# Eclectic-Sheep/sheeprl

Hardware: NVIDIA H100
Metric: Dreamer-V3 train-steps/sec (S, bs16 seq64 horizon15, 64x64x3 obs) (higher is better)
Workload: dtype f32

## Files before the change

include/b200rl.h:

```cpp
#ifndef B200RL_H_
#define B200RL_H_

#include <cuda_runtime_api.h>

#ifdef __cplusplus
extern "C" {
#endif

const char* b200rl_last_error(void);
int b200rl_abi_version(void);
const char* b200rl_build_arch(void);
int b200rl_device_check(void);

int b200rl_gemm_f32(const float* A, const float* B, float* C, const float* bias, int M, int N, int K, int lda, int ldb,
                    int ldc, int transA, int transB, int accumulate, cudaStream_t stream);
int b200rl_set_matmul_precision(int tf32_passes);
int b200rl_get_matmul_precision(void);
int b200rl_gemm_tc_supported(const float* A, const float* B, int M, int N, int K, int lda, int ldb, int transA,
                             int transB);
int b200rl_gemm_tc(const float* A, const float* B, float* C, const float* bias, int M, int N, int K, int lda, int ldb,
                   int ldc, int transA, int transB, int accumulate, cudaStream_t stream);
int b200rl_tf32_split(const float* X, float* Xhi, float* Xlo, long long n, cudaStream_t stream);
int b200rl_tf32_split_t(const float* W, float* Thi, float* Tlo, int rows, int cols, long long ldw, long long ldt,
                        cudaStream_t stream);
int b200rl_gemm_tc_presplit_supported(const float* A, const float* Bhi, const float* Blo, int M, int N, int K, int lda,
                                      int ldb);
int b200rl_gemm_tc_presplit(const float* A, const float* Bhi, const float* Blo, float* C, const float* bias, int M, int N,
                            int K, int lda, int ldb, int ldc, int accumulate, cudaStream_t stream);
int b200rl_gemm_ln_supported(const float* A, const float* W, int M, int N, int K, int lda, int ldw, int mode);
int b200rl_gemm_ln(const float* A, const float* W, int M, int N, int K, int lda, int ldw, const float* gamma,
                   const float* beta, float eps, int act, float* pre, long long ldpre, float* out, long long ldout,
                   int mode, const float* h_prev, long long ldh, float* h_out, long long ldho, float* h_out2,
                   long long ldho2, cudaStream_t stream);
int b200rl_gemm_ln_presplit_supported(const float* A, const float* Whi, const float* Wlo, int M, int N, int K, int lda,
                                      int ldw, int mode);
int b200rl_gemm_ln_presplit(const float* A, const float* Whi, const float* Wlo, int M, int N, int K, int lda, int ldw,
                            const float* gamma, const float* beta, float eps, int act, float* pre, long long ldpre,
                            float* out, long long ldout, int mode, const float* h_prev, long long ldh, float* h_out,
                            long long ldho, float* h_out2, long long ldho2, cudaStream_t stream);
int b200rl_ln_act_route(int C, long long ld0, long long ld1, long long ld2, const float* p0, const float* p1,
                        const float* p2, const float* gamma, const float* beta);
int b200rl_ln_act_fwd(const float* X, const float* gamma, const float* beta, float* Y, long long M, int C,
                      long long ldx, long long ldy, float eps, int act, cudaStream_t stream);
int b200rl_ln_act_bwd(const float* X, const float* gamma, const float* beta, const float* dY, float* dX, float* dgamma,
                      float* dbeta, long long M, int C, long long ldx, long long lddy, long long lddx, float eps,
                      int act, int accumulate, cudaStream_t stream);
int b200rl_col_sum(const float* X, float* out, long long M, int C, long long ldx, int accumulate, cudaStream_t stream);

int b200rl_obs_prep(const void* obs_nchw, int is_uint8, float* out_nhwc, long long NB, int C, int HW,
                    cudaStream_t stream);
int b200rl_transpose_batched(const float* X, float* Y, int NB, int a, int b, cudaStream_t stream);
int b200rl_transpose2d(const float* X, float* Y, int rows, int cols, long long ldx, long long ldy, cudaStream_t stream);
int b200rl_conv_down(const float* big, const float* W, float* small_, int NB, int h, int w, int Cs, int Cb,
                     cudaStream_t stream);
int b200rl_conv_up(const float* small_, const float* W, float* big, const float* bias, int NB, int h, int w, int Cs,
                   int Cb, cudaStream_t stream);
int b200rl_conv_wgrad(const float* small_, const float* big, float* dW, int NB, int h, int w, int Cs, int Cb,
                      int accumulate, cudaStream_t stream);
int b200rl_thin_down_supported(int w, int Cs, int Cb);
int b200rl_thin_up_supported(int Cs, int Cb);
int b200rl_thin_wgrad_supported(int Cs, int Cb);
int b200rl_conv_wgrad_tc_supported(int NB, int h, int w, int Cs, int Cb);
long long b200rl_conv_wgrad_tc_workspace(int NB, int h, int w, int Cs, int Cb);
int b200rl_conv_wgrad_tc(const float* small_, const float* big, float* dW, float* workspace, int NB, int h, int w,
                         int Cs, int Cb, int accumulate, cudaStream_t stream);
int b200rl_conv_tc_supported(int mode_up, int NB, int h, int w, int Cs, int Cb);
long long b200rl_conv_pack_floats(int mode_up, int Cs, int Cb);
int b200rl_conv_pack(const float* W, float* Wpacked, int mode_up, int Cs, int Cb, cudaStream_t stream);
int b200rl_conv_down_tc(const float* big, const float* Wpacked, float* small_, int NB, int h, int w, int Cs, int Cb,
                        cudaStream_t stream);
int b200rl_conv_up_tc(const float* small_, const float* Wpacked, float* big, const float* bias, int NB, int h, int w,
                      int Cs, int Cb, cudaStream_t stream);
int b200rl_conv_pack_split(const float* W, float* Whi, float* Wlo, int mode_up, int Cs, int Cb, cudaStream_t stream);
int b200rl_conv_down_tc_presplit(const float* big, const float* Whi, const float* Wlo, float* small_, int NB, int h, int w,
                                 int Cs, int Cb, cudaStream_t stream);
int b200rl_conv_up_tc_presplit(const float* small_, const float* Whi, const float* Wlo, float* big, const float* bias,
                               int NB, int h, int w, int Cs, int Cb, cudaStream_t stream);

int b200rl_gru_gate_fwd(const float* G, const float* Hin, float* Hout, long long M, int R, long long ldg,
                        long long ldhi, long long ldho, cudaStream_t stream);
int b200rl_gru_gate_bwd(const float* G, const float* Hin, const float* dH, float* dG, float* dHin, long long M, int R,
                        long long ldg, long long ldhi, long long lddh, long long lddg, long long lddhi,
                        cudaStream_t stream);
int b200rl_mask_mix(const float* prev, const float* init_row, const float* first, float* out, long long M, int C,
                    long long ldp, long long ldo, cudaStream_t stream);
int b200rl_mask_bwd(const float* dIn, const float* first, float* dPrev, float* dInit, int M, int C, long long ldi,
                    long long ldp, cudaStream_t stream);
int b200rl_cat_sample(const float* raw, const float* noise, float* onehot, float* mix_out, long long M, int groups,
                      int classes, long long ldr, long long ldn, long long ldo, long long ldm, float unimix,
                      cudaStream_t stream);
int b200rl_head_sample_supported(const float* X, const float* W, int Kin, int A, long long ldx, long long ldw);
int b200rl_head_sample(const float* X, const float* W, const float* bias, const float* noise, float* raw, float* onehot,
                       long long M, int Kin, int A, long long ldx, long long ldw, long long ldr, long long ldn,
                       long long ldo, float unimix, cudaStream_t stream);
int b200rl_cat_sample_bwd(const float* raw, const float* dz, const float* dmix, float* draw, long long M, int groups,
                          int classes, long long ldr, long long lddz, long long lddm, long long lddr, float unimix,
                          cudaStream_t stream);
int b200rl_kl_loss_grad(const float* post_mix, const float* prior_mix, float* d_post, float* d_prior, float* rows,
                        long long M, int groups, int classes, long long ldp, long long ldq, long long lddp,
                        long long lddq, float kl_dyn, float kl_rep, float free_nats, float regularizer, float scale,
                        cudaStream_t stream);
typedef struct b200rl_rssm_scan_args {
  int T, B, S, D, R, A, Dx, Dt, Dr, ld_lat, ld_wr1;
  float eps, unimix;
  const float *W_in, *lnx_g, *lnx_b, *W_g, *lng_g, *lng_b, *W_t1, *lnt_g, *lnt_b, *W_t2, *b_t2;
  const float *W_r1, *lnr_g, *lnr_b, *W_r2, *b_r2;
  const float *h0, *z0;
  const float *pe, *actions, *first, *noise;
  float* latent;
  float *z_in, *h_in, *a_in, *x_pre, *x_act, *g_pre, *g_ln, *tr_pre, *tr_act, *rp_pre, *rp_act;
  float *post_raw, *prior_raw, *post_mix, *prior_mix;
  void* workspace;
  long long workspace_bytes;
} b200rl_rssm_scan_args;
typedef struct b200rl_rssm_scan_grads {
  const float *d_latent, *d_post_mix, *d_prior_mix;
  float *d_post_raw, *d_prior_raw, *d_rp_act, *d_rp_pre, *d_tr_act, *d_tr_pre, *d_g_ln, *d_g_pre, *d_x_act, *d_x_pre;
  float* d_h0;
  const float *q_r, *q_g, *q_x;
} b200rl_rssm_scan_grads;
long long b200rl_rssm_scan_workspace_bytes(int T, int B, int S, int D, int Dx, int R, int Dr);
int b200rl_rssm_scan_fwd(const b200rl_rssm_scan_args* args, cudaStream_t stream);
int b200rl_rssm_scan_bwd(const b200rl_rssm_scan_args* args, const b200rl_rssm_scan_grads* grads, cudaStream_t stream);
int b200rl_rssm_scan_check(const b200rl_rssm_scan_args* args, int backward);
int b200rl_rssm_scan_error(const void* workspace, cudaStream_t stream);
int b200rl_rssm_scan_profile(const void* workspace, long long* out64, cudaStream_t stream);
typedef struct b200rl_gru_scan_args {
  int T, B, R, ld_wg, ld_lat, lat_off;
  float eps;
  const float *W_g, *lng_g, *lng_b;
  const float *h0, *first;
  float* g_pre;
  float *g_ln, *h_in, *latent;
  void* workspace;
  long long workspace_bytes;
} b200rl_gru_scan_args;
typedef struct b200rl_gru_scan_grads {
  const float *d_latent, *q_g;
  float *d_g_ln, *d_h0;
} b200rl_gru_scan_grads;
long long b200rl_gru_scan_workspace_bytes(int T, int B, int R);
int b200rl_gru_scan_fwd(const b200rl_gru_scan_args* args, cudaStream_t stream);
int b200rl_gru_scan_bwd(const b200rl_gru_scan_args* args, const b200rl_gru_scan_grads* grads, cudaStream_t stream);
int b200rl_gru_scan_check(const b200rl_gru_scan_args* args, int backward);

int b200rl_mse_loss_grad(const float* pred, const float* target, float* loss_row, float* grad, long long M, int P,
                         float scale, cudaStream_t stream);
int b200rl_twohot_loss_grad(const float* logits, const float* x, const float* weight, float* loss_row, float* dlogits,
                            long long M, int nbins, long long ldl, long long ldd, float low, float high, float scale,
                            int accumulate, cudaStream_t stream);
int b200rl_bce_loss_grad(const float* logit, const float* target, float* loss_row, float* dlogit, long long M,
                         float loss_scale, float scale, cudaStream_t stream);
int b200rl_twohot_mean(const float* logits, float* out, long long M, int nbins, long long ldl, float low, float high,
                       cudaStream_t stream);
int b200rl_lambda_returns(const float* rew, const float* val, const float* cont_logit, const float* true_cont,
                          float* lam, float* discount, int H, int N, float gamma, float lmbda, cudaStream_t stream);
int b200rl_moments_update(const float* x, long long n, float* state_low_high, float* out_offset_invscale, float decay,
                          float max_, float p_low, float p_high, cudaStream_t stream);
int b200rl_actor_loss_grad(const float* raw, const float* actions, const float* lam, const float* val,
                           const float* discount, const float* moments, float* rows, float* draw, long long M,
                           const int* head_dims_host, int n_heads, float unimix, float ent_coef, float scale,
                           cudaStream_t stream);
int b200rl_sum_rows(const float* X, float* out, long long M, int C, long long ldx, float scale, cudaStream_t stream);
int b200rl_weighted_mean(const float* x, const float* w, float* out, long long n, float scale, cudaStream_t stream);

int b200rl_sumsq(const float* x, long long n, double* out, cudaStream_t stream);
int b200rl_adam_step(float* p, const float* g, float* m, float* v, const double* normsq, const int* step_dev,
                     float* norm_out, long long n, float max_norm, float lr, float b1, float b2, float eps,
                     cudaStream_t stream);
int b200rl_adam_step_wd(float* p, const float* g, float* m, float* v, const double* normsq, const int* step_dev,
                        float* norm_out, long long n, float max_norm, float lr, float b1, float b2, float eps,
                        float weight_decay, cudaStream_t stream);
int b200rl_rmsprop_step(float* p, const float* g, float* square_avg, float* momentum_buf, float* grad_avg,
                        const double* normsq, float* norm_out, long long n, float max_norm, float lr, float alpha,
                        float eps, float weight_decay, float momentum, cudaStream_t stream);
int b200rl_ema(float* target, const float* src, long long n, float tau, cudaStream_t stream);
int b200rl_fill_exponential(float* out, long long n, unsigned long long seed, unsigned int stream_id,
                            const int* counter_dev, cudaStream_t stream);
int b200rl_zero(float* x, long long n, cudaStream_t stream);
int b200rl_copy2d(const float* src, float* dst, long long M, int C, long long lds, long long ldd, cudaStream_t stream);
int b200rl_axpy(const float* x, float* y, long long n, float alpha, cudaStream_t stream);
int b200rl_affine(const float* x, float* y, long long n, float alpha, float beta, cudaStream_t stream);
int b200rl_symlog(const float* x, float* y, long long M, int C, long long ldx, long long ldy, cudaStream_t stream);
int b200rl_tanh_fwd(const float* x, float* y, long long n, cudaStream_t stream);
int b200rl_tanh_bwd(const float* y, const float* dy, float* dx, long long n, int accumulate, cudaStream_t stream);
int b200rl_increment(int* p, cudaStream_t stream);

int b200rl_replay_gather(const void* storage, const long long* idx, void* out, int n_samples, int batch, int seq_len,
                         long long row_bytes, cudaStream_t stream);
int b200rl_replay_scatter(const void* src, const long long* dst_rows, void* storage, long long n_rows,
                          long long row_bytes, cudaStream_t stream);
int b200rl_gae(const float* rewards, const float* values, const float* dones, const float* next_value, float* returns,
// ... 89 lines not shown
```

sheeprl_b200/algos/p2e_dv3/engine.py:

```python
from __future__ import annotations

from collections import OrderedDict
from typing import Dict, Optional, Sequence

import torch

from sheeprl_b200.engine import TWOHOT_HIGH, TWOHOT_LOW, DV3Engine, _MLP, dv3_param_shapes
from sheeprl_b200.params import FlatGroup


def ensemble_param_shapes(cfg, actions_dim: Sequence[int], members: Sequence[int]) -> "OrderedDict[str, tuple]":
    a, w = cfg.algo, cfg.algo.world_model
    Z = w.stochastic_size * w.discrete_size
    d_in = Z + w.recurrent_model.recurrent_state_size + int(sum(actions_dim))
    hid, nh = a.ensembles.dense_units, a.ensembles.mlp_layers
    out = OrderedDict()
    for i in members:
        for k in range(nh):
            out[f"{i}._model.{3 * k}.weight"] = (hid, d_in if k == 0 else hid)
            out[f"{i}._model.{3 * k + 1}.weight"] = (hid,)
            out[f"{i}._model.{3 * k + 1}.bias"] = (hid,)
        out[f"{i}._model.{3 * nh}.weight"] = (Z, hid)
        out[f"{i}._model.{3 * nh}.bias"] = (Z,)
    return out


class P2EDV3Engine(DV3Engine):
    METRIC_NAMES_P2E = ("Loss/ensemble_loss", "Loss/policy_loss_exploration")

    def __init__(self, cfg, actions_dim: Sequence[int], in_channels: int = 3, device="cuda", ops=None,
                 is_continuous: bool = False, mlp_dims=None, cnn_dims=None):
        if cfg.algo.world_model.decoupled_rssm:
            raise NotImplementedError(
                "Plan2Explore cannot run with decoupled_rssm: the reference's exploration train() calls the five-argument "
                "RSSM.dynamic (p2e_dv3_exploration.py:136), which DecoupledRSSM does not have")
        super().__init__(cfg, actions_dim, in_channels, device, ops, is_continuous=is_continuous, mlp_dims=mlp_dims,
                         cnn_dims=cnn_dims)
        a = cfg.algo
        N, H, L, A, Z = self.N, self.H, self.L, self.A, self.Z
        M1, M0 = (H + 1) * N, H * N
        b = self._buf
        _, ac_s, cr_s, _ = dv3_param_shapes(cfg, self.actions_dim, in_channels, self.is_continuous,
                                            dict(zip(self.vec_keys, self.vec_dims)), self.cnn_dims)
        self.actor_expl = FlatGroup(ac_s, device)
        self.actor_expl_mlp = _MLP(self, self.actor_expl, "model._model.", L, self.du, self.nh, None, M1, self.eps,
                                   "actor_expl", True)
        self.critics_expl: "OrderedDict[str, dict]" = OrderedDict()
        for k, v in a.critics_exploration.items():
            if v.weight > 0:
                grp, tgt = FlatGroup(cr_s, device), FlatGroup(cr_s, device, with_optimizer=False)
                self.critics_expl[k] = dict(
                    weight=float(v.weight), reward_type=str(v.reward_type), group=grp, target=tgt,
                    mlp=_MLP(self, grp, "_model.", L, self.du, self.nh, self.bins_c, M1, self.eps, f"critic_expl_{k}", True),
                    target_mlp=_MLP(self, tgt, "_model.", L, self.du, self.nh, self.bins_c, M0, self.eps, f"target_expl_{k}", False),
                    moments_state=b(f"moments_state_{k}", 2), moments_out=b(f"moments_out_{k}", 2),
                    values=b(f"values_{k}", H + 1, N), lam=b(f"lam_{k}", H, N), reward_mean=b(f"reward_mean_{k}", 1),
                    values_mean=b(f"values_mean_{k}", 1), lam_mean=b(f"lam_mean_{k}", 1), value_loss=b(f"value_loss_{k}", 1),
                    policy_rows=b(f"policy_rows_{k}", M0) if self.is_continuous else None)
        if not any(c["reward_type"] == "intrinsic" for c in self.critics_expl.values()):
            raise RuntimeError("You must specify at least one intrinsic critic (`reward_type='intrinsic'`)")
        self.n_ens = int(a.ensembles.n)
        rest = list(range(self.n_ens - 1))
        self.ens_rest = FlatGroup(ensemble_param_shapes(cfg, self.actions_dim, rest), device) if rest else None
        self.ens_last = FlatGroup(ensemble_param_shapes(cfg, self.actions_dim, [self.n_ens - 1]), device)
        eh, el = a.ensembles.dense_units, a.ensembles.mlp_layers
        self.ens_mlps = [_MLP(self, self.ens_last if i == self.n_ens - 1 else self.ens_rest, f"{i}._model.", L + A, eh, el, Z,
                              M1, self.eps, f"ens{i}", True) for i in range(self.n_ens)]
        self.ens_in = b("ens_in", M1, L + A)
        self.z_next = b("z_next", N, Z)
        self.ens_rows = b("ens_rows", M1)
        self.d_ens_out = b("d_ens_out", N, Z)
        self.ens_mean = b("ens_mean", M1, Z)
        self.ens_scratch = b("ens_scratch", M1, Z)
        self.intr_reward = b("intr_reward", H + 1, N)
        self.d_actor_raw_k = b("d_actor_raw_k", M0, self.AW)
        self.policy_rows_k = b("policy_rows_k", M0)
        self.p2e_metrics = b("p2e_metrics", 4)
        self.unit_moments = b("unit_moments", 2)
        self.unit_moments[1] = 1.0
        self.norms = b("norms_p2e", 6 + len(self.critics_expl))
        for name in ["ens_rest", "ens_last", "actor_expl"] + [f"critic_expl_{k}" for k in self.critics_expl]:
            self.normsq[name] = self._buf(f"normsq_{name}", (), dtype=torch.float64)
        self.noise_img_state_expl = b("noise_img_state_expl", H, N, Z)
        self.noise_img_action_expl = b("noise_img_action_expl", H + 1, N, A)

    def extra_groups(self):
        d = {"actor_expl": self.actor_expl, "ens_last": self.ens_last}
        if self.ens_rest is not None:
            d["ens_rest"] = self.ens_rest
        for k, c in self.critics_expl.items():
            d[f"critic_expl_{k}"] = c["group"]
        return d

    def optimizer_groups(self):
        return super().optimizer_groups() + list(self.extra_groups().values())

    def groups(self) -> "OrderedDict[str, FlatGroup]":
        out = OrderedDict(wm=self.wm, actor_task=self.actor, critic_task=self.critic, target_task=self.target,
                          actor_expl=self.actor_expl)
        for k, c in self.critics_expl.items():
            out[f"critic_expl_{k}"], out[f"target_expl_{k}"] = c["group"], c["target"]
        return out

    def load_ensembles(self, state: Dict[str, torch.Tensor]):
        last = f"{self.n_ens - 1}."
        if self.ens_rest is not None:
            self.ens_rest.load({k: v for k, v in state.items() if not k.startswith(last)})
        self.ens_last.load({k: v for k, v in state.items() if k.startswith(last)})

    def ensembles_state_dict(self) -> "OrderedDict[str, torch.Tensor]":
        out = OrderedDict()
        if self.ens_rest is not None:
            out.update(self.ens_rest.state_dict())
        out.update(self.ens_last.state_dict())
        return out

    def train_step(self, data: Dict[str, torch.Tensor], noise: Optional[Dict[str, torch.Tensor]] = None):
        ops = self.ops
        N, H, Z = self.N, self.H, self.Z
        if noise is None:
            self._draw_noise(None)
            ops.fill_exponential(self.noise_img_state_expl.view(-1), self.rng_seed, 3, self.rng_t)
            fill = ops.fill_normal if self.is_continuous else ops.fill_exponential
            fill(self.noise_img_action_expl.view(-1), self.rng_seed, 4, self.rng_t)
        else:
            self._draw_noise({"post": noise["post"], "img_state": noise["img_state_task"], "img_action": noise["img_action_task"]})
            self.noise_img_state_expl.copy_(noise["img_state_expl"].reshape(H, N, Z))
            self.noise_img_action_expl.copy_(torch.cat([x for x in noise["img_action_expl"]], -1))
        self._world_model_phase(data, heads_detached=True)
        self._ensemble_learning(data)
        task_noise = (self.noise_img_state, self.noise_img_action)
        self.noise_img_state, self.noise_img_action = self.noise_img_state_expl, self.noise_img_action_expl
        try:
            self._imagine(self.actor_expl, self.actor_expl_mlp)
            self._exploration_losses()
        finally:
            self.noise_img_state, self.noise_img_action = task_noise
        self._imagine()
        self._behaviour_losses()
        return self.metrics

    def _ensemble_learning(self, data: Dict[str, torch.Tensor]):
        ops, N, B, L, A, Z = self.ops, self.N, self.B, self.L, self.A, self.Z
        a = self.cfg.algo
        M = N - B
        x = self.ens_in[:N]
        ops.copy(self.latent, x[:, :L])
        ops.copy(data["actions"].reshape(N, A), x[:, L:])
        ops.copy(self.latent[B:, :Z], self.z_next[:M])
        ops.zero(self.ens_last.grad)
        if self.ens_rest is not None:
            ops.zero(self.ens_rest.grad)
        ops.zero(self.p2e_metrics[0:1])
        x = x[:M]
        for m in self.ens_mlps:
            out = m.forward(x, M=M)
            ops.mse_loss_grad(out, self.z_next[:M], 1.0 / M, self.ens_rows[:M], self.d_ens_out[:M])
            ops.sum_rows(self.ens_rows[:M].view(M, 1), self.p2e_metrics[2:3], 1.0 / M)
            ops.axpy(self.p2e_metrics[2:3], self.p2e_metrics[0:1])
            m.backward(x, self.d_ens_out[:M], None, False, M=M)
        o = a.ensembles.optimizer
        if self.ens_rest is not None:
            self._optimizer_step("ens_rest", self.ens_rest, 0.0, o, self.norms.numel() - 1)
        self._optimizer_step("ens_last", self.ens_last, float(a.ensembles.clip_gradients or 0.0), o, 3)

    def _intrinsic_reward(self):
        ops, N, H, L, Z = self.ops, self.N, self.H, self.L, self.Z
        M1 = (H + 1) * N
        n = self.n_ens
        x = self.ens_in
        ops.copy(self.traj.view(M1, L), x[:, :L])
        ops.copy(self.actions.view(M1, self.A), x[:, L:])
        outs = [m.forward(x) for m in self.ens_mlps]
        ops.zero(self.ens_mean)
        for o in outs:
            ops.axpy(o, self.ens_mean, 1.0 / n)
        ops.zero(self.intr_reward)
        scale = float(self.cfg.algo.intrinsic_reward_multiplier) / (Z * max(n - 1, 1))
        for o in outs:
            ops.mse_loss_grad(o, self.ens_mean, 0.0, self.ens_rows, self.ens_scratch)
            ops.axpy(self.ens_rows, self.intr_reward.view(-1), scale)

    def _exploration_losses(self):
        ops, N, H, L = self.ops, self.N, self.H, self.L
        a = self.cfg.algo
        M1, M0 = (H + 1) * N, H * N
        traj2 = self.traj.view(M1, L)
        c_logit = self.cont_img.forward(traj2)
        mo = a.actor.moments
        weights_sum = sum(c["weight"] for c in self.critics_expl.values())
        v_logits, r_logits = {}, None
        for k, c in self.critics_expl.items():
            v_logits[k] = c["mlp"].forward(traj2)
            ops.twohot_mean(v_logits[k], TWOHOT_LOW, TWOHOT_HIGH, c["values"].view(-1))
            if c["reward_type"] == "intrinsic":
                self._intrinsic_reward()
                rew = self.intr_reward
            else:
                r_logits = self.rew_img.forward(traj2)
                ops.twohot_mean(r_logits, TWOHOT_LOW, TWOHOT_HIGH, self.rew_pred.view(-1))
                rew = self.rew_pred
            ops.sum_rows(rew.view(M1, 1), c["reward_mean"], 1.0 / M1)
            ops.lambda_returns(rew, c["values"], c_logit.view(H + 1, N), self.true_cont, float(a.gamma), float(a.lmbda),
                               c["lam"], self.discount)
            lam_all = c["lam"] if self.allgather is None else self.allgather(c["lam"])
            ops.moments_update(lam_all.view(-1), c["moments_state"], float(mo.decay), float(mo.max),
                               float(mo.percentile.low), float(mo.percentile.high), c["moments_out"])
            ops.sum_rows(c["values"].view(M1, 1), c["values_mean"], 1.0 / M1)
            ops.sum_rows(c["lam"].view(M0, 1), c["lam_mean"], 1.0 / M0)
        ops.zero(self.p2e_metrics[1:2])
        if self.is_continuous:
            self._continuous_policy_gradient(c_logit, [
                (c["mlp"], v_logits[k], c["values"], c["lam"], c["moments_out"], c["weight"] / weights_sum,
                 None if c["reward_type"] == "intrinsic" else r_logits, c["policy_rows"])
                for k, c in self.critics_expl.items()])
            for c in self.critics_expl.values():
                ops.sum_rows(c["policy_rows"].view(M0, 1), self.p2e_metrics[2:3], -c["weight"] / weights_sum / M0)
                ops.axpy(self.p2e_metrics[2:3], self.p2e_metrics[1:2])
        else:
            for j, (k, c) in enumerate(self.critics_expl.items()):
                share = c["weight"] / weights_sum
                rows, draw = (self.policy_rows, self.d_actor_raw) if j == 0 else (self.policy_rows_k, self.d_actor_raw_k)
                ops.actor_loss_grad(self.actor_raw[:M0], self.actions.view(M1, self.A)[:M0], c["lam"].view(-1),
                                    c["values"].view(-1)[:M0], self.discount.view(-1)[:M0], c["moments_out"],
                                    self.actions_dim, self.unimix, float(a.actor.ent_coef) / share if j == 0 else 0.0,
                                    share / M0, rows, draw)
                ops.sum_rows(rows.view(M0, 1), self.p2e_metrics[2:3], -share / M0)
                ops.axpy(self.p2e_metrics[2:3], self.p2e_metrics[1:2])
                if j > 0:
                    ops.axpy(self.d_actor_raw_k, self.d_actor_raw)
        self._actor_update(self.actor_expl, self.actor_expl_mlp, "actor_expl", 4)
        for j, (k, c) in enumerate(self.critics_expl.items()):
            self._critic_update(c["group"], c["mlp"], c["target_mlp"], v_logits[k], c["lam"], c["value_loss"],
                                f"critic_expl_{k}", 5 + j)

    def metrics_dict(self) -> Dict[str, torch.Tensor]:
        d = {n: self.metrics[i] for i, n in enumerate(self.METRIC_NAMES[:8])}
        d["Loss/policy_loss_task"], d["Loss/value_loss_task"] = self.metrics[8], self.metrics[9]
        d["Loss/ensemble_loss"], d["Loss/policy_loss_exploration"] = self.p2e_metrics[0], self.p2e_metrics[1]
        d["Grads/world_model"], d["Grads/actor_task"], d["Grads/critic_task"] = self.norms[0], self.norms[1], self.norms[2]
        d["Grads/ensemble"], d["Grads/actor_exploration"] = self.norms[3], self.norms[4]
        for j, (k, c) in enumerate(self.critics_expl.items()):
            d[f"Loss/value_loss_exploration_{k}"] = c["value_loss"][0]
            d[f"Grads/critic_exploration_{k}"] = self.norms[5 + j]
            d[f"Values_exploration/predicted_values_{k}"] = c["values_mean"][0]
            d[f"Values_exploration/lambda_values_{k}"] = c["lam_mean"][0]
            if c["reward_type"] == "intrinsic":
                d[f"Rewards/intrinsic_{k}"] = c["reward_mean"][0]
        return d

    def update_targets(self, tau: float):
        self.update_target(tau)
        for c in self.critics_expl.values():
            if tau >= 1.0:
                self.ops.copy(c["group"].flat, c["target"].flat)
            else:
                self.ops.ema(c["target"].flat, c["group"].flat, float(tau))
```

sheeprl_b200/csrc/gemm_tc.cu:

```cuda
#include <cuda.h>
#include <cudaTypedefs.h>

#include <mutex>
#include <unordered_map>

#include "common.cuh"

namespace {

constexpr int BM = 128, BK = 32;
constexpr int NTHREADS = 384;
constexpr int NSPLIT_THREADS = 96;
constexpr int NCONS_WARPS = 8;
constexpr int PRODUCER_REGS = 56, CONSUMER_REGS = 224;
template <int PASSES, bool PRESPLIT> __host__ __device__ constexpr int b_buffers() { return PRESPLIT ? (PASSES == 3 ? 2 : 1) : 3; }
template <int BN, int PASSES, bool PRESPLIT> constexpr int stages_for() {
  return (227 * 1024 - 1024 - 256) / ((BM + b_buffers<PASSES, PRESPLIT>() * BN) * BK * (int)sizeof(float));
}

__device__ __forceinline__ uint32_t smem_u32(const void* p) { return (uint32_t)__cvta_generic_to_shared(p); }

__device__ __forceinline__ void mbar_init(uint64_t* bar, uint32_t count) {
  asm volatile("mbarrier.init.shared::cta.b64 [%0], %1;" ::"r"(smem_u32(bar)), "r"(count) : "memory");
}
__device__ __forceinline__ void mbar_expect_tx(uint64_t* bar, uint32_t bytes) {
  asm volatile("mbarrier.arrive.expect_tx.shared::cta.b64 _, [%0], %1;" ::"r"(smem_u32(bar)), "r"(bytes) : "memory");
}
__device__ __forceinline__ void mbar_arrive(uint64_t* bar) {
  asm volatile("mbarrier.arrive.shared::cta.b64 _, [%0];" ::"r"(smem_u32(bar)) : "memory");
}
__device__ __forceinline__ bool mbar_try_wait(uint64_t* bar, uint32_t parity) {
  uint32_t ok;
  asm volatile(
      "{\n\t"
      ".reg .pred p;\n\t"
      "mbarrier.try_wait.parity.shared::cta.b64 p, [%1], %2;\n\t"
      "selp.u32 %0, 1, 0, p;\n\t"
      "}"
      : "=r"(ok)
      : "r"(smem_u32(bar)), "r"(parity)
      : "memory");
  return ok != 0;
}
__device__ __forceinline__ void mbar_wait(uint64_t* bar, uint32_t parity) {
  if (mbar_try_wait(bar, parity)) return;
  const long long t0 = clock64();
  while (!mbar_try_wait(bar, parity)) {
    if (clock64() - t0 > 2000000000LL) asm volatile("trap;");
  }
}
__device__ __forceinline__ bool elect_one() {
  uint32_t pred;
  asm volatile(
      "{\n\t"
      ".reg .pred p;\n\t"
      "elect.sync _|p, 0xffffffff;\n\t"
      "selp.u32 %0, 1, 0, p;\n\t"
      "}"
      : "=r"(pred));
  return pred != 0;
}
__device__ __forceinline__ void tma_load_2d(void* smem_dst, const CUtensorMap* map, uint64_t* bar, int c0, int c1) {
  asm volatile(
      "cp.async.bulk.tensor.2d.shared::cluster.global.mbarrier::complete_tx::bytes [%0], [%1, {%3, %4}], [%2];" ::"r"(
          smem_u32(smem_dst)),
      "l"(map), "r"(smem_u32(bar)), "r"(c0), "r"(c1)
      : "memory");
}
__device__ __forceinline__ void tma_load_4d(void* smem_dst, const CUtensorMap* map, uint64_t* bar, int c0, int c1, int c2,
                                            int c3) {
  asm volatile(
      "cp.async.bulk.tensor.4d.shared::cluster.global.mbarrier::complete_tx::bytes [%0], [%1, {%3, %4, %5, %6}], [%2];" ::"r"(
          smem_u32(smem_dst)),
      "l"(map), "r"(smem_u32(bar)), "r"(c0), "r"(c1), "r"(c2), "r"(c3)
      : "memory");
}

__device__ __forceinline__ void wgmma_tf32(float (&d)[32], const uint32_t (&a)[4], uint64_t desc_b, int scale_d) {
  asm volatile(
      "{\n\t.reg .pred p;\n\tsetp.ne.b32 p, %37, 0;\n\twgmma.mma_async.sync.aligned.m64n64k8.f32.tf32.tf32 {%0, %1, %2, %3, %4, %5, %6, %7, %8, %9, %10, %11, %12, %13, %14, %15, %16, %17, %18, %19, %20, %21, %22, %23, %24, %25, %26, %27, %28, %29, %30, %31}, {%32, %33, %34, %35}, %36, p, 1, 1;\n\t}"
      : "+f"(d[0]), "+f"(d[1]), "+f"(d[2]), "+f"(d[3]), "+f"(d[4]), "+f"(d[5]), "+f"(d[6]), "+f"(d[7]), "+f"(d[8]), "+f"(d[9]), "+f"(d[10]), "+f"(d[11]), "+f"(d[12]), "+f"(d[13]), "+f"(d[14]), "+f"(d[15]), "+f"(d[16]), "+f"(d[17]), "+f"(d[18]), "+f"(d[19]), "+f"(d[20]), "+f"(d[21]), "+f"(d[22]), "+f"(d[23]), "+f"(d[24]), "+f"(d[25]), "+f"(d[26]), "+f"(d[27]), "+f"(d[28]), "+f"(d[29]), "+f"(d[30]), "+f"(d[31])
      : "r"(a[0]), "r"(a[1]), "r"(a[2]), "r"(a[3]), "l"(desc_b), "r"(scale_d));
}
__device__ __forceinline__ void wgmma_tf32(float (&d)[64], const uint32_t (&a)[4], uint64_t desc_b, int scale_d) {
  asm volatile(
      "{\n\t.reg .pred p;\n\tsetp.ne.b32 p, %69, 0;\n\twgmma.mma_async.sync.aligned.m64n128k8.f32.tf32.tf32 {%0, %1, %2, %3, %4, %5, %6, %7, %8, %9, %10, %11, %12, %13, %14, %15, %16, %17, %18, %19, %20, %21, %22, %23, %24, %25, %26, %27, %28, %29, %30, %31, %32, %33, %34, %35, %36, %37, %38, %39, %40, %41, %42, %43, %44, %45, %46, %47, %48, %49, %50, %51, %52, %53, %54, %55, %56, %57, %58, %59, %60, %61, %62, %63}, {%64, %65, %66, %67}, %68, p, 1, 1;\n\t}"
      : "+f"(d[0]), "+f"(d[1]), "+f"(d[2]), "+f"(d[3]), "+f"(d[4]), "+f"(d[5]), "+f"(d[6]), "+f"(d[7]), "+f"(d[8]), "+f"(d[9]), "+f"(d[10]), "+f"(d[11]), "+f"(d[12]), "+f"(d[13]), "+f"(d[14]), "+f"(d[15]), "+f"(d[16]), "+f"(d[17]), "+f"(d[18]), "+f"(d[19]), "+f"(d[20]), "+f"(d[21]), "+f"(d[22]), "+f"(d[23]), "+f"(d[24]), "+f"(d[25]), "+f"(d[26]), "+f"(d[27]), "+f"(d[28]), "+f"(d[29]), "+f"(d[30]), "+f"(d[31]), "+f"(d[32]), "+f"(d[33]), "+f"(d[34]), "+f"(d[35]), "+f"(d[36]), "+f"(d[37]), "+f"(d[38]), "+f"(d[39]), "+f"(d[40]), "+f"(d[41]), "+f"(d[42]), "+f"(d[43]), "+f"(d[44]), "+f"(d[45]), "+f"(d[46]), "+f"(d[47]), "+f"(d[48]), "+f"(d[49]), "+f"(d[50]), "+f"(d[51]), "+f"(d[52]), "+f"(d[53]), "+f"(d[54]), "+f"(d[55]), "+f"(d[56]), "+f"(d[57]), "+f"(d[58]), "+f"(d[59]), "+f"(d[60]), "+f"(d[61]), "+f"(d[62]), "+f"(d[63])
      : "r"(a[0]), "r"(a[1]), "r"(a[2]), "r"(a[3]), "l"(desc_b), "r"(scale_d));
}
__device__ __forceinline__ void wgmma_fence() { asm volatile("wgmma.fence.sync.aligned;" ::: "memory"); }
__device__ __forceinline__ void wgmma_commit() { asm volatile("wgmma.commit_group.sync.aligned;" ::: "memory"); }
__device__ __forceinline__ void wgmma_wait_all() { asm volatile("wgmma.wait_group.sync.aligned 0;" ::: "memory"); }
template <int N>
__device__ __forceinline__ void fence_regs(float (&r)[N]) {
#pragma unroll
  for (int i = 0; i < N; ++i) asm volatile("" : "+f"(r[i])::"memory");
}
template <int N, int W>
__device__ __forceinline__ void fence_regs(uint32_t (&r)[N][W]) {
#pragma unroll
  for (int i = 0; i < N; ++i)
#pragma unroll
    for (int j = 0; j < W; ++j) asm volatile("" : "+r"(r[i][j])::"memory");
}

__device__ __forceinline__ uint64_t make_desc(uint32_t smem_addr) {
  uint64_t d = 0;
  d |= (uint64_t)((smem_addr & 0x3FFFF) >> 4);
  d |= (uint64_t)1 << 16;
  d |= (uint64_t)(1024 >> 4) << 32;
  d |= (uint64_t)1 << 62;
  return d;
}

__device__ __forceinline__ uint32_t kmajor_off(int r, int k) {
  return (uint32_t)(r * 128 + ((((k >> 2) ^ r) & 7) << 4) + (k & 3) * 4);
}
__device__ __forceinline__ uint32_t mnmajor_off(int r, int k) {
  return (uint32_t)((r >> 5) * 4096 + k * 128 + (((((r & 31) >> 2) ^ k) & 7) << 4) + (r & 3) * 4);
}

template <int BN, int PASSES, bool PRESPLIT>
struct Smem;
template <int BN, int PASSES>
struct Smem<BN, PASSES, false> {
  static constexpr int STAGES = stages_for<BN, PASSES, false>();
  float a[STAGES][BM * BK];
  float b[STAGES][BN * BK];
  float b_hi[STAGES][BN * BK];
  float b_lo[STAGES][BN * BK];
  uint64_t full[STAGES], split[STAGES], empty[STAGES];
};
template <int BN, int PASSES>
struct Smem<BN, PASSES, true> {
  static constexpr int STAGES = stages_for<BN, PASSES, true>();
  float a[STAGES][BM * BK];
  float b_hi[STAGES][BN * BK];
  float b_lo[PASSES == 3 ? STAGES : 1][PASSES == 3 ? BN * BK : 256];
  uint64_t full[STAGES], empty[STAGES];
};

constexpr int CH = 4;

constexpr int MODE_GEMM = 0, MODE_DOWN = 1, MODE_UP = 2;
constexpr int MODE_UP4 = 3;
constexpr int GROUP_M = 16;
struct TileGeo {
  int mode;
  int h, w, NB;
  int bw, bh, bn;
  int tiles_x, tiles_y;
  int chunks;
  int Cout;
  int ksplits;
  float* part;
  int mpad, ldw;
  int force_part;
  int passes;
  int a_mn, b_mn;
// ... 630 lines not shown
extern "C" int b200rl_tf32_split_t(const float* W, float* Thi, float* Tlo, int rows, int cols, long long ldw, long long ldt,
                                   cudaStream_t st) {
  RL_CHECK_ARG(W && Thi && Tlo, "null pointer");
  RL_CHECK_ARG(rows > 0 && cols > 0 && ldw >= cols && ldt >= rows, "bad transposed-split geometry");
  dim3 grid(ceil_div(cols, 32), ceil_div(ldt, 32));
  tf32_split_t_kernel<<<grid, dim3(32, 8), 0, st>>>(W, Thi, Tlo, rows, cols, ldw, ldt);
  RL_CHECK_LAUNCH();
  return B200RL_OK;
}

extern "C" int b200rl_gemm_tc_supported(const float* A, const float* B, int M, int N, int K, int lda, int ldb,
                                        int transA, int transB) {
  (void)transA; (void)transB;
  if (M < 32 || N < 48 || K < 32) return 0;
  if ((lda & 3) || (ldb & 3)) return 0;
  if ((reinterpret_cast<uintptr_t>(A) & 15) || (reinterpret_cast<uintptr_t>(B) & 15)) return 0;
  return 1;
}

namespace {
struct FusedTail { float* part; int ks, mpad, ldw; };

int gemm_tc_impl(const float* A, const float* B, const float* Blo, float* C, const float* bias, int M, int N, int K,
                 int lda, int ldb, int ldc, int transA, int transB, int accumulate, cudaStream_t st, FusedTail* fused) {
  RL_CHECK_ARG(A && B && (C || fused), "null pointer");
  RL_CHECK_ARG(b200rl_gemm_tc_supported(A, B, M, N, K, lda, ldb, transA, transB), "shape not eligible for the tensor-core path");
  RL_CHECK_ARG(!Blo || (transB && !(reinterpret_cast<uintptr_t>(Blo) & 15)), "pre-split B must be 16-byte aligned [N][K] planes");
  const int BN = (N <= 64) ? 64 : 128;
  CUtensorMap ma, mb, mb2;
  if (!transA) { if (int rc = get_map(A, M, K, lda, BM, &ma)) return rc; }
  else         { if (int rc = get_map(A, K, M, lda, 32, &ma)) return rc; }
  if (transB)  { if (int rc = get_map(B, N, K, ldb, BN, &mb)) return rc; }
  else         { if (int rc = get_map(B, K, N, ldb, 32, &mb)) return rc; }
  mb2 = mb;
  if (Blo && g_passes == 3) { if (int rc = get_map(Blo, N, K, ldb, BN, &mb2)) return rc; }
  dim3 grid((N + BN - 1) / BN, (M + BM - 1) / BM);
  TileGeo g = {};
  g.mode = MODE_GEMM;
  g.a_mn = transA ? 1 : 0;
  g.b_mn = transB ? 0 : 1;
  g.ksplits = 1;
  g.passes = g_passes;
  const int tiles = grid.x * grid.y, nkb = (K + BK - 1) / BK;
  if (tiles < 2 * kNumSMs && nkb >= 8) {
    int best = 1;
    float best_t = 1e30f;
    const int max_sp = nkb / 4 < 32 ? nkb / 4 : 32;
    for (int sp = 1; sp <= (max_sp < 1 ? 1 : max_sp); ++sp) {
      const int per = (nkb + sp - 1) / sp, real = (nkb + per - 1) / per;
      const int waves = (tiles * real + kNumSMs - 1) / kNumSMs;
      const float t = waves * (per * 0.8f + 4.0f) + (real > 1 ? 3.0f + 0.3f * real : 0.0f);
      if (t < best_t - 1e-3f) { best_t = t; best = real; }
    }
    g.ksplits = best;
  }
  if (g.ksplits > 1 || fused) {
    grid.z = g.ksplits;
    g.mpad = (int)grid.y * BM;
    g.ldw = (int)grid.x * BN;
    if (int rc = split_workspace((size_t)g.ksplits * g.mpad * g.ldw, st, &g.part)) return rc;
    if (fused) { g.force_part = 1; *fused = FusedTail{g.part, g.ksplits, g.mpad, g.ldw}; }
  }
  g.mtiles = (int)grid.y;
  g.ntiles = (int)grid.x;
  grid.x = 1;
  grid.y = persistent_grid_y(g.mtiles * g.ntiles, grid.z);
  DISPATCH_GEMM_TC(BN, g.passes, Blo != nullptr, grid, st, ma, mb, mb2, C, bias, M, N, K, ldc, accumulate, g);
  RL_CHECK_LAUNCH();
  if (g.ksplits > 1 && !fused) {
    splitk_reduce_kernel<<<ceil_div((long long)M * ((N + 3) / 4), 256), 256, 0, st>>>(g.part, C, bias, M, N, ldc, g.ksplits, g.mpad,
                                                                                      g.ldw, accumulate);
    RL_CHECK_LAUNCH();
  }
  return B200RL_OK;
}

template <int NV>
__global__ void __launch_bounds__(256)
splitk_ln_kernel(const float* __restrict__ part, int ks, int mpad, int ldw, int M, int N, const float* __restrict__ gamma,
                 const float* __restrict__ beta, float eps, int act, float* __restrict__ pre, long long ldpre,
                 float* __restrict__ ln_out, long long ldln, int mode, const float* __restrict__ h_prev, long long ldh,
                 float* __restrict__ h_out, long long ldho, float* __restrict__ h_out2, long long ldho2) {
  const int lane = threadIdx.x & 31;
  const long long row = ((long long)blockIdx.x * blockDim.x + threadIdx.x) >> 5;
  if (row >= M) return;
  const int n4 = N >> 2;
  float4 v[NV];
#pragma unroll
  for (int i = 0; i < NV; ++i) v[i] = make_float4(0.f, 0.f, 0.f, 0.f);
#pragma unroll 4
  for (int z = 0; z < ks; ++z) {
    const float4* p = reinterpret_cast<const float4*>(part + ((size_t)z * mpad + row) * ldw);
#pragma unroll
    for (int i = 0; i < NV; ++i) {
      const int c = lane + 32 * i;
      if (c < n4) { const float4 t = __ldcg(p + c); v[i].x += t.x; v[i].y += t.y; v[i].z += t.z; v[i].w += t.w; }
    }
  }
  float s = 0.f;
#pragma unroll
  for (int i = 0; i < NV; ++i) {
    const int c = lane + 32 * i;
    if (c < n4) {
      if (pre) reinterpret_cast<float4*>(pre + row * ldpre)[c] = v[i];
      s += (v[i].x + v[i].y) + (v[i].z + v[i].w);
    }
  }
  const float mu = warp_sum(s) / (float)N;
  float q = 0.f;
#pragma unroll
  for (int i = 0; i < NV; ++i) {
    const int c = lane + 32 * i;
    if (c < n4) {
      const float dx = v[i].x - mu, dy = v[i].y - mu, dz = v[i].z - mu, dw = v[i].w - mu;
      q += (dx * dx + dy * dy) + (dz * dz + dw * dw);
    }
  }
  const float rstd = rsqrtf(warp_sum(q) / (float)N + eps);
#pragma unroll
  for (int i = 0; i < NV; ++i) {
    const int c = lane + 32 * i;
    if (c < n4) {
      const float4 g = reinterpret_cast<const float4*>(gamma)[c], b = reinterpret_cast<const float4*>(beta)[c];
      v[i].x = (v[i].x - mu) * rstd * g.x + b.x; v[i].y = (v[i].y - mu) * rstd * g.y + b.y;
      v[i].z = (v[i].z - mu) * rstd * g.z + b.z; v[i].w = (v[i].w - mu) * rstd * g.w + b.w;
      if (mode == 0 && act == 1) {
        v[i].x = v[i].x / (1.f + expf(-v[i].x)); v[i].y = v[i].y / (1.f + expf(-v[i].y));
        v[i].z = v[i].z / (1.f + expf(-v[i].z)); v[i].w = v[i].w / (1.f + expf(-v[i].w));
      }
      if (ln_out) reinterpret_cast<float4*>(ln_out + row * ldln)[c] = v[i];
    }
  }
  if (mode == 1) {
    constexpr int NR = NV / 3;
#pragma unroll
    for (int i = 0; i < NR; ++i) {
      const int c = lane + 32 * i;
      const float4 hp = reinterpret_cast<const float4*>(h_prev + row * ldh)[c];
      const float4 gr = v[i], gc = v[i + NR], gu = v[i + 2 * NR];
      float4 h;
      auto gate = [](float r_, float c_, float u_, float hprev) {
        const float r = 1.f / (1.f + expf(-r_));
        const float cand = tanhf(r * c_);
        const float u = 1.f / (1.f + expf(-(u_ - 1.f)));
        return u * cand + (1.f - u) * hprev;
      };
      h.x = gate(gr.x, gc.x, gu.x, hp.x); h.y = gate(gr.y, gc.y, gu.y, hp.y);
      h.z = gate(gr.z, gc.z, gu.z, hp.z); h.w = gate(gr.w, gc.w, gu.w, hp.w);
      reinterpret_cast<float4*>(h_out + row * ldho)[c] = h;
      if (h_out2) reinterpret_cast<float4*>(h_out2 + row * ldho2)[c] = h;
    }
  }
}
}

extern "C" int b200rl_gemm_tc(const float* A, const float* B, float* C, const float* bias, int M, int N, int K, int lda,
                              int ldb, int ldc, int transA, int transB, int accumulate, cudaStream_t st) {
  return gemm_tc_impl(A, B, nullptr, C, bias, M, N, K, lda, ldb, ldc, transA, transB, accumulate, st, nullptr);
}

extern "C" int b200rl_gemm_tc_presplit_supported(const float* A, const float* Bhi, const float* Blo, int M, int N, int K,
                                                 int lda, int ldb) {
  return b200rl_gemm_tc_supported(A, Bhi, M, N, K, lda, ldb, 0, 1) && !(reinterpret_cast<uintptr_t>(Blo) & 15);
}
extern "C" int b200rl_gemm_tc_presplit(const float* A, const float* Bhi, const float* Blo, float* C, const float* bias, int M,
                                       int N, int K, int lda, int ldb, int ldc, int accumulate, cudaStream_t st) {
  RL_CHECK_ARG(Blo, "null pointer");
  return gemm_tc_impl(A, Bhi, Blo, C, bias, M, N, K, lda, ldb, ldc, 0, 1, accumulate, st, nullptr);
}

extern "C" int b200rl_gemm_ln_supported(const float* A, const float* B, int M, int N, int K, int lda, int ldb, int mode) {
  if (!b200rl_gemm_tc_supported(A, B, M, N, K, lda, ldb, 0, 1)) return 0;
  if (N % 4 || N > 1536) return 0;
  if (mode == 1 && (N % 384 != 0)) return 0;
  return 1;
}

namespace {
int gemm_ln_impl(const float* A, const float* W, const float* Wlo, int M, int N, int K, int lda, int ldw_, const float* gamma,
                 const float* beta, float eps, int act, float* pre, long long ldpre, float* out, long long ldout, int mode,
                 const float* h_prev, long long ldh, float* h_out, long long ldho, float* h_out2, long long ldho2,
                 cudaStream_t st) {
  RL_CHECK_ARG(A && W && gamma && beta, "null pointer");
  RL_CHECK_ARG(b200rl_gemm_ln_supported(A, W, M, N, K, lda, ldw_, mode), "shape not eligible for the fused product + LayerNorm");
  RL_CHECK_ARG(mode == 0 ? out != nullptr : (h_prev && h_out), "missing output");
  RL_CHECK_ARG(((reinterpret_cast<uintptr_t>(gamma) | reinterpret_cast<uintptr_t>(beta) | reinterpret_cast<uintptr_t>(pre) |
                 reinterpret_cast<uintptr_t>(out) | reinterpret_cast<uintptr_t>(h_prev) | reinterpret_cast<uintptr_t>(h_out) |
                 reinterpret_cast<uintptr_t>(h_out2)) & 15) == 0 &&
                   ((ldpre | ldout | ldh | ldho | ldho2) & 3) == 0,
               "fused product + LayerNorm needs 16-byte aligned rows");
  FusedTail ft;
  if (int rc = gemm_tc_impl(A, W, Wlo, nullptr, nullptr, M, N, K, lda, ldw_, N, 0, 1, 0, st, &ft)) return rc;
  const int blocks = ceil_div((long long)M * 32, 256);
#define LAUNCH_SPLITK_LN(NV_)                                                                                              \
  splitk_ln_kernel<NV_><<<blocks, 256, 0, st>>>(ft.part, ft.ks, ft.mpad, ft.ldw, M, N, gamma, beta, eps, act, pre, ldpre, out, \
                                                ldout, mode, h_prev, ldh, h_out, ldho, h_out2, ldho2)
  if (mode == 1) {
    if (N == 384) LAUNCH_SPLITK_LN(3); else if (N == 768) LAUNCH_SPLITK_LN(6); else if (N == 1152) LAUNCH_SPLITK_LN(9);
    else LAUNCH_SPLITK_LN(12);
  } else if (N <= 128) LAUNCH_SPLITK_LN(1);
  else if (N <= 256) LAUNCH_SPLITK_LN(2);
  else if (N <= 512) LAUNCH_SPLITK_LN(4);
  else if (N <= 1024) LAUNCH_SPLITK_LN(8);
  else LAUNCH_SPLITK_LN(12);
#undef LAUNCH_SPLITK_LN
  RL_CHECK_LAUNCH();
  return B200RL_OK;
}
}

extern "C" int b200rl_gemm_ln(const float* A, const float* W, int M, int N, int K, int lda, int ldw_, const float* gamma,
                              const float* beta, float eps, int act, float* pre, long long ldpre, float* out, long long ldout,
                              int mode, const float* h_prev, long long ldh, float* h_out, long long ldho, float* h_out2,
                              long long ldho2, cudaStream_t st) {
  return gemm_ln_impl(A, W, nullptr, M, N, K, lda, ldw_, gamma, beta, eps, act, pre, ldpre, out, ldout, mode, h_prev, ldh,
                      h_out, ldho, h_out2, ldho2, st);
}
extern "C" int b200rl_gemm_ln_presplit_supported(const float* A, const float* Whi, const float* Wlo, int M, int N, int K,
                                                 int lda, int ldw, int mode) {
  return b200rl_gemm_ln_supported(A, Whi, M, N, K, lda, ldw, mode) && !(reinterpret_cast<uintptr_t>(Wlo) & 15);
}
extern "C" int b200rl_gemm_ln_presplit(const float* A, const float* Whi, const float* Wlo, int M, int N, int K, int lda,
                                       int ldw, const float* gamma, const float* beta, float eps, int act, float* pre,
                                       long long ldpre, float* out, long long ldout, int mode, const float* h_prev,
                                       long long ldh, float* h_out, long long ldho, float* h_out2, long long ldho2,
                                       cudaStream_t st) {
  RL_CHECK_ARG(Wlo, "null pointer");
  return gemm_ln_impl(A, Whi, Wlo, M, N, K, lda, ldw, gamma, beta, eps, act, pre, ldpre, out, ldout, mode, h_prev, ldh,
                      h_out, ldho, h_out2, ldho2, st);
}

extern "C" int b200rl_conv_wgrad_mn_supported(int NB, int h, int w, int Cs, int Cb) {
  if (w <= 0 || h <= 0 || (w & (w - 1)) || (h & (h - 1))) return 0;
  const long long P = (long long)NB * h * w;
  if (Cb % 32 || Cs < 48 || Cs % 4 || P % 32 || P < 1024 || P > 2000000000LL) return 0;
  const int bw = w < 32 ? w : 32, bh = (32 / bw) < h ? (32 / bw) : h, bn = 32 / (bw * bh);
  return (bw * bh * bn == 32) && (NB % bn == 0);
}

extern "C" int b200rl_conv_wgrad_mn(const float* small_, const float* big, float* G, int NB, int h, int w, int Cs, int Cb,
                                    cudaStream_t st) {
  RL_CHECK_ARG(small_ && big && G, "null pointer");
  RL_CHECK_ARG(b200rl_conv_wgrad_mn_supported(NB, h, w, Cs, Cb), "shape not eligible for the in-place wgrad path");
  const int P = NB * h * w, M = 16 * Cb, N = Cs;
  TileGeo g = {};
  g.mode = MODE_GEMM; g.a_mn = 1; g.b_mn = 1; g.wg = 1; g.passes = g_passes;
  g.h = h; g.w = w; g.NB = NB; g.Cout = Cb;
  g.bw = w < 32 ? w : 32; g.bh = (32 / g.bw) < h ? (32 / g.bw) : h; g.bn = 32 / (g.bw * g.bh);
  CUtensorMap ma, mb;
  if (int rc = get_map4(big, Cb, 2 * w, 2 * h, NB, g.bw, g.bh, g.bn, 2, &ma)) return rc;
  if (int rc = get_map(small_, P, Cs, Cs, 32, &mb)) return rc;
  const int BN = (N <= 64) ? 64 : 128;
  dim3 grid((N + BN - 1) / BN, M / BM);
  const int tiles = grid.x * grid.y, nkb = P / BK;
  int sp = (2 * kNumSMs + tiles - 1) / tiles;
  if (sp > nkb / 8) sp = nkb / 8;
  if (sp < 1) sp = 1;
  const int per = (nkb + sp - 1) / sp;
  g.ksplits = (nkb + per - 1) / per;
  grid.z = g.ksplits;
  g.mtiles = (int)grid.y;
  g.ntiles = (int)grid.x;
  if (g.ksplits > 1) {
    g.mpad = (int)grid.y * BM;
    g.ldw = (int)grid.x * BN;
    if (int rc = split_workspace((size_t)g.ksplits * g.mpad * g.ldw, st, &g.part)) return rc;
  }
  grid.x = 1;
  grid.y = (unsigned)(g.mtiles * g.ntiles);
  DISPATCH_GEMM_TC(BN, g.passes, false, grid, st, ma, mb, mb, G, nullptr, M, N, P, N, 0, g);
  RL_CHECK_LAUNCH();
  if (g.ksplits > 1) {
    splitk_reduce_kernel<<<ceil_div((long long)M * ((N + 3) / 4), 256), 256, 0, st>>>(g.part, G, nullptr, M, N, N, g.ksplits, g.mpad,
                                                                                      g.ldw, 0);
    RL_CHECK_LAUNCH();
  }
  return B200RL_OK;
}
```

sheeprl_b200/csrc/rssm.cu:

```cuda
#include "common.cuh"

namespace {

__global__ void gru_gate_fwd_kernel(const float* __restrict__ G, const float* __restrict__ Hin, float* __restrict__ Hout,
                                    long long M, int R, long long ldg, long long ldhi, long long ldho) {
  const long long idx = (long long)blockIdx.x * blockDim.x + threadIdx.x;
  if (idx >= M * R) return;
  const long long m = idx / R;
  const int j = (int)(idx - m * R);
  const float* g = G + m * ldg;
  const float r = sigmoidf_(g[j]);
  const float c = tanhf(r * g[R + j]);
  const float u = sigmoidf_(g[2 * R + j] - 1.f);
  const float h = Hin[m * ldhi + j];
  Hout[m * ldho + j] = u * c + (1.f - u) * h;
}

__global__ void gru_gate_bwd_kernel(const float* __restrict__ G, const float* __restrict__ Hin,
                                    const float* __restrict__ dH, float* __restrict__ dG, float* __restrict__ dHin,
                                    long long M, int R, long long ldg, long long ldhi, long long lddh,
                                    long long lddg, long long lddhi) {
  const long long idx = (long long)blockIdx.x * blockDim.x + threadIdx.x;
  if (idx >= M * R) return;
  const long long m = idx / R;
  const int j = (int)(idx - m * R);
  const float* g = G + m * ldg;
  const float gc = g[R + j];
  const float r = sigmoidf_(g[j]);
  const float c = tanhf(r * gc);
  const float u = sigmoidf_(g[2 * R + j] - 1.f);
  const float h = Hin[m * ldhi + j];
  const float dh = dH[m * lddh + j];
  const float du = dh * (c - h);
  const float drc = dh * u * (1.f - c * c);
  float* dg = dG + m * lddg;
  dg[j] = drc * gc * r * (1.f - r);
  dg[R + j] = drc * r;
  dg[2 * R + j] = du * u * (1.f - u);
  dHin[m * lddhi + j] = dh * (1.f - u);
}

__global__ void mask_mix_kernel(const float* __restrict__ prev, const float* __restrict__ init,
                                const float* __restrict__ first, float* __restrict__ out, long long M, int C,
                                long long ldp, long long ldo) {
  const long long idx = (long long)blockIdx.x * blockDim.x + threadIdx.x;
  if (idx >= M * C) return;
  const long long m = idx / C;
  const int c = (int)(idx - m * C);
  const float f = first[m];
  float v = (1.f - f) * prev[m * ldp + c];
  if (init) v += f * init[c];
  out[m * ldo + c] = v;
}

__global__ void mask_bwd_kernel(const float* __restrict__ dIn, const float* __restrict__ first,
                                float* __restrict__ dPrev, float* __restrict__ dInit, int M, int C, long long ldi,
                                long long ldp) {
  const int c = blockIdx.x * blockDim.x + threadIdx.x;
  if (c >= C) return;
  float s = 0.f;
  for (int m = 0; m < M; ++m) {
    const float f = first[m];
    const float d = dIn[m * ldi + c];
    dPrev[m * ldp + c] = (1.f - f) * d;
    s = fmaf(f, d, s);
  }
  if (dInit) dInit[c] += s;
}

struct GroupStats {
  float raw_max, raw_sum;
  float lse;
};

__device__ __forceinline__ float unimix_logprob(float s, float unimix, float invK, float& pm) {
  pm = (1.f - unimix) * s + unimix * invK;
  return logf(fminf(fmaxf(pm, kFp32Eps), 1.f - kFp32Eps));
}

__device__ __forceinline__ GroupStats group_stats(const float* x, int K, float unimix, int lane) {
  GroupStats st;
  float mx = -INFINITY;
  for (int c = lane; c < K; c += 32) mx = fmaxf(mx, x[c]);
  mx = warp_max(mx);
  float sm = 0.f;
  for (int c = lane; c < K; c += 32) sm += expf(x[c] - mx);
  sm = warp_sum(sm);
  st.raw_max = mx;
  st.raw_sum = sm;
  const float invK = 1.f / (float)K;
  float lmx = -INFINITY;
  for (int c = lane; c < K; c += 32) {
    float l = x[c];
    if (unimix > 0.f) { float pm; l = unimix_logprob(expf(x[c] - mx) / sm, unimix, invK, pm); }
    lmx = fmaxf(lmx, l);
  }
  lmx = warp_max(lmx);
  float ls = 0.f;
  for (int c = lane; c < K; c += 32) {
    float l = x[c];
    if (unimix > 0.f) { float pm; l = unimix_logprob(expf(x[c] - mx) / sm, unimix, invK, pm); }
    ls += expf(l - lmx);
  }
  ls = warp_sum(ls);
  st.lse = lmx + logf(ls);
  return st;
}

__global__ void __launch_bounds__(256)
cat_sample_kernel(const float* __restrict__ raw, const float* __restrict__ noise, float* __restrict__ onehot,
                  float* __restrict__ mix_out, long long M, int groups, int K, long long ldr, long long ldn,
                  long long ldo, long long ldm, float unimix) {
  const int lane = threadIdx.x & 31;
  const long long warp = ((long long)blockIdx.x * blockDim.x + threadIdx.x) >> 5;
  if (warp >= M * groups) return;
  const long long m = warp / groups;
  const int g = (int)(warp - m * groups);
  const float* x = raw + m * ldr + (long long)g * K;
  const GroupStats st = group_stats(x, K, unimix, lane);
  const float invK = 1.f / (float)K;
  float lgmax = -INFINITY;
  for (int c = lane; c < K; c += 32) {
    float l = x[c];
    if (unimix > 0.f) { float pm; l = unimix_logprob(expf(x[c] - st.raw_max) / st.raw_sum, unimix, invK, pm); }
    if (mix_out) mix_out[m * ldm + (long long)g * K + c] = l;
    lgmax = fmaxf(lgmax, l - st.lse);
  }
  lgmax = warp_max(lgmax);
  float psum = 0.f;
  for (int c = lane; c < K; c += 32) {
    float l = x[c];
    if (unimix > 0.f) { float pm; l = unimix_logprob(expf(x[c] - st.raw_max) / st.raw_sum, unimix, invK, pm); }
    psum += expf(l - st.lse - lgmax);
  }
  psum = warp_sum(psum);
  if (!onehot) return;
  float best = -INFINITY;
  int besti = 0x7fffffff;
  for (int c = lane; c < K; c += 32) {
    float l = x[c];
    if (unimix > 0.f) { float pm; l = unimix_logprob(expf(x[c] - st.raw_max) / st.raw_sum, unimix, invK, pm); }
    float p = expf(l - st.lse - lgmax) / psum;
    if (noise) p = p / noise[m * ldn + (long long)g * K + c];
    if (p > best) { best = p; besti = c; }
  }
#pragma unroll
  for (int o = 16; o > 0; o >>= 1) {
    const float ob = __shfl_xor_sync(0xffffffffu, best, o);
    const int oi = __shfl_xor_sync(0xffffffffu, besti, o);
    if (ob > best || (ob == best && oi < besti)) { best = ob; besti = oi; }
  }
  for (int c = lane; c < K; c += 32) onehot[m * ldo + (long long)g * K + c] = (c == besti) ? 1.f : 0.f;
}

__device__ __forceinline__ void cat_sample_lane(float xv, bool on, int K, int lane, float unimix,
                                                const float* __restrict__ noise_row, float* __restrict__ onehot_row,
                                                float* __restrict__ mix_row) {
  const float mx = warp_max(xv);
  const float sm = warp_sum(on ? expf(xv - mx) : 0.f);
  const float invK = 1.f / (float)K;
  float l = xv;
  if (unimix > 0.f && on) { float pm; l = unimix_logprob(expf(xv - mx) / sm, unimix, invK, pm); }
  const float lmx = warp_max(on ? l : -INFINITY);
  const float ls = warp_sum(on ? expf(l - lmx) : 0.f);
  const float lse = lmx + logf(ls);
  if (mix_row && on) mix_row[lane] = l;
  const float lgmax = warp_max(on ? l - lse : -INFINITY);
  const float e = on ? expf(l - lse - lgmax) : 0.f;
  const float psum = warp_sum(e);
  if (!onehot_row) return;
  float best = -INFINITY;
  int besti = 0x7fffffff;
  if (on) {
    float p = e / psum;
    if (noise_row) p = p / noise_row[lane];
    if (p > best) { best = p; besti = lane; }
  }
#pragma unroll
  for (int o = 16; o > 0; o >>= 1) {
    const float ob = __shfl_xor_sync(0xffffffffu, best, o);
    const int oi = __shfl_xor_sync(0xffffffffu, besti, o);
    if (ob > best || (ob == best && oi < besti)) { best = ob; besti = oi; }
  }
  if (on) onehot_row[lane] = (lane == besti) ? 1.f : 0.f;
}

__global__ void __launch_bounds__(256)
cat_sample_small_kernel(const float* __restrict__ raw, const float* __restrict__ noise, float* __restrict__ onehot,
                        float* __restrict__ mix_out, long long M, int groups, int K, long long ldr, long long ldn,
                        long long ldo, long long ldm, float unimix) {
  const int lane = threadIdx.x & 31;
  const long long warp = ((long long)blockIdx.x * blockDim.x + threadIdx.x) >> 5;
  if (warp >= M * groups) return;
  const long long m = warp / groups;
  const int g = (int)(warp - m * groups);
  const bool on = lane < K;
  const float xv = on ? raw[m * ldr + (long long)g * K + lane] : -INFINITY;
  cat_sample_lane(xv, on, K, lane, unimix, noise ? noise + m * ldn + (long long)g * K : nullptr,
                  onehot ? onehot + m * ldo + (long long)g * K : nullptr, mix_out ? mix_out + m * ldm + (long long)g * K : nullptr);
}

__global__ void __launch_bounds__(256)
head_sample_kernel(const float* __restrict__ X, const float* __restrict__ W, const float* __restrict__ bias,
                   const float* __restrict__ noise, float* __restrict__ raw, float* __restrict__ onehot, long long M, int Kin,
                   int A, long long ldx, long long ldw, long long ldr, long long ldn, long long ldo, float unimix) {
  const int lane = threadIdx.x & 31;
  const long long m = ((long long)blockIdx.x * blockDim.x + threadIdx.x) >> 5;
  if (m >= M) return;
  const int k4 = Kin >> 2;
  float4 x[8];
#pragma unroll
  for (int i = 0; i < 8; ++i) {
    const int c = lane + 32 * i;
    x[i] = c < k4 ? reinterpret_cast<const float4*>(X + m * ldx)[c] : make_float4(0.f, 0.f, 0.f, 0.f);
  }
  float mine = -INFINITY;
  for (int a = 0; a < A; ++a) {
    const float4* w = reinterpret_cast<const float4*>(W + (long long)a * ldw);
    float acc = 0.f;
#pragma unroll
    for (int i = 0; i < 8; ++i) {
      const int c = lane + 32 * i;
      if (c < k4) {
        const float4 t = __ldg(w + c);
        acc = fmaf(x[i].x, t.x, acc); acc = fmaf(x[i].y, t.y, acc); acc = fmaf(x[i].z, t.z, acc); acc = fmaf(x[i].w, t.w, acc);
      }
    }
    acc = warp_sum(acc);
    if (lane == a) mine = acc + (bias ? bias[a] : 0.f);
  }
  const bool on = lane < A;
  if (on) raw[m * ldr + lane] = mine;
  cat_sample_lane(mine, on, A, lane, unimix, noise ? noise + m * ldn : nullptr, onehot + m * ldo, nullptr);
}

__global__ void __launch_bounds__(256)
cat_sample_bwd_kernel(const float* __restrict__ raw, const float* __restrict__ dz, const float* __restrict__ dmix,
                      float* __restrict__ draw, long long M, int groups, int K, long long ldr, long long lddz,
                      long long lddm, long long lddr, float unimix) {
  const int lane = threadIdx.x & 31;
  const long long warp = ((long long)blockIdx.x * blockDim.x + threadIdx.x) >> 5;
  if (warp >= M * groups) return;
  const long long m = warp / groups;
  const int g = (int)(warp - m * groups);
  const long long go = (long long)g * K;
  const float* x = raw + m * ldr + go;
  const GroupStats st = group_stats(x, K, unimix, lane);
  const float invK = 1.f / (float)K;
  float pdz = 0.f;
  if (dz) {
    for (int c = lane; c < K; c += 32) {
      float l = x[c];
      if (unimix > 0.f) { float pm; l = unimix_logprob(expf(x[c] - st.raw_max) / st.raw_sum, unimix, invK, pm); }
      pdz = fmaf(expf(l - st.lse), dz[m * lddz + go + c], pdz);
    }
    pdz = warp_sum(pdz);
  }
  float sds = 0.f;
  for (int c = lane; c < K; c += 32) {
    const float s = expf(x[c] - st.raw_max) / st.raw_sum;
    float pm = 0.f, l = x[c];
    if (unimix > 0.f) l = unimix_logprob(s, unimix, invK, pm);
    float gg = dmix ? dmix[m * lddm + go + c] : 0.f;
    if (dz) gg += expf(l - st.lse) * (dz[m * lddz + go + c] - pdz);
    if (unimix > 0.f) {
      const bool inside = pm >= kFp32Eps && pm <= 1.f - kFp32Eps;
      const float ds = inside ? gg * (1.f - unimix) / pm : 0.f;
      sds = fmaf(s, ds, sds);
    }
  }
  sds = warp_sum(sds);
  for (int c = lane; c < K; c += 32) {
    const float s = expf(x[c] - st.raw_max) / st.raw_sum;
    float pm = 0.f, l = x[c];
    if (unimix > 0.f) l = unimix_logprob(s, unimix, invK, pm);
    float gg = dmix ? dmix[m * lddm + go + c] : 0.f;
    if (dz) gg += expf(l - st.lse) * (dz[m * lddz + go + c] - pdz);
    if (unimix > 0.f) {
      const bool inside = pm >= kFp32Eps && pm <= 1.f - kFp32Eps;
      const float ds = inside ? gg * (1.f - unimix) / pm : 0.f;
      gg = s * (ds - sds);
    }
    draw[m * lddr + go + c] = gg;
  }
}

__global__ void __launch_bounds__(256)
kl_loss_grad_kernel(const float* __restrict__ post, const float* __restrict__ prior, float* __restrict__ d_post,
                    float* __restrict__ d_prior, float* __restrict__ rows, int groups, int K, long long ldp,
                    long long ldq, long long lddp, long long lddq, float kl_dyn, float kl_rep, float free_nats,
                    float coef ) {
  __shared__ float red[32];
  const long long m = blockIdx.x;
  const int lane = threadIdx.x & 31, wid = threadIdx.x >> 5, nw = blockDim.x >> 5;
  const float* lp0 = post + m * ldp;
  const float* lq0 = prior + m * ldq;
  float kl = 0.f, hp = 0.f, hq = 0.f;
  for (int g = wid; g < groups; g += nw) {
    const float* a = lp0 + (long long)g * K;
    const float* b = lq0 + (long long)g * K;
    float ma = -INFINITY, mb = -INFINITY;
    for (int c = lane; c < K; c += 32) { ma = fmaxf(ma, a[c]); mb = fmaxf(mb, b[c]); }
    ma = warp_max(ma); mb = warp_max(mb);
    float sa = 0.f, sb = 0.f;
    for (int c = lane; c < K; c += 32) { sa += expf(a[c] - ma); sb += expf(b[c] - mb); }
    const float lsea = ma + logf(warp_sum(sa)), lseb = mb + logf(warp_sum(sb));
    float t = 0.f, ea = 0.f, eb = 0.f;
    for (int c = lane; c < K; c += 32) {
      const float lpa = a[c] - lsea, lqb = b[c] - lseb;
      const float pa = expf(lpa), pb = expf(lqb);
      t = fmaf(pa, lpa - lqb, t);
      ea = fmaf(-pa, lpa, ea);
      eb = fmaf(-pb, lqb, eb);
    }
    kl += t; hp += ea; hq += eb;
  }
  kl = block_sum(kl, red);
  hp = block_sum(hp, red);
  hq = block_sum(hq, red);
  if (threadIdx.x == 0) {
    rows[m * 4 + 0] = kl;
    rows[m * 4 + 1] = (kl_dyn + kl_rep) * fmaxf(kl, free_nats);
    rows[m * 4 + 2] = hp;
    rows[m * 4 + 3] = hq;
  }
  const float live = (kl > free_nats) ? coef : 0.f;
  for (int g = wid; g < groups; g += nw) {
    const float* a = lp0 + (long long)g * K;
    const float* b = lq0 + (long long)g * K;
    float ma = -INFINITY, mb = -INFINITY;
    for (int c = lane; c < K; c += 32) { ma = fmaxf(ma, a[c]); mb = fmaxf(mb, b[c]); }
    ma = warp_max(ma); mb = warp_max(mb);
    float sa = 0.f, sb = 0.f;
    for (int c = lane; c < K; c += 32) { sa += expf(a[c] - ma); sb += expf(b[c] - mb); }
    const float lsea = ma + logf(warp_sum(sa)), lseb = mb + logf(warp_sum(sb));
    float t = 0.f;
    for (int c = lane; c < K; c += 32) {
// ... 212 lines not shown
```

sheeprl_b200/engine.py:

```python
from __future__ import annotations

import math
from typing import Dict, Mapping, Optional, Sequence

import torch

from sheeprl_b200.params import FlatGroup

ACT_NONE, ACT_SILU = 0, 1
TWOHOT_LOW, TWOHOT_HIGH = -20.0, 20.0


def decoder_channels(cfg, in_channels: int, cnn_dims: Optional[Mapping[str, int]] = None) -> int:
    a = cfg.algo
    dec = list(a.cnn_keys.decoder or [])
    if dec == list(a.cnn_keys.encoder or []):
        return in_channels
    missing = [k for k in dec if k not in (cnn_dims or {})]
    if missing:
        raise ValueError(f"the channel count of the decoded image key(s) {missing} is not known (pass cnn_dims)")
    return sum(int(cnn_dims[k]) for k in dec)


def check_decoder_keys(cfg) -> None:
    a = cfg.algo
    for kind in ("cnn_keys", "mlp_keys"):
        enc, dec = list(a[kind].encoder or []), list(a[kind].decoder or [])
        for k in dec:
            if k not in enc:
                raise ValueError(f"{kind}.decoder: key '{k}' is not in {kind}.encoder {enc}: the decoder can only "
                                 f"reconstruct encoded keys")
        if len(set(dec)) != len(dec):
            raise ValueError(f"{kind}.decoder names a key twice: {dec}")
    if not a.cnn_keys.decoder and not a.mlp_keys.decoder:
        raise ValueError("There must be at least one decoder: cnn_keys.decoder and mlp_keys.decoder are both empty")


def dv3_param_shapes(cfg, actions_dim: Sequence[int], in_channels: int, is_continuous: bool = False,
                     mlp_dims: Optional[Mapping[str, int]] = None, cnn_dims: Optional[Mapping[str, int]] = None):
    a, w = cfg.algo, cfg.algo.world_model
    S, D = w.stochastic_size, w.discrete_size
    Z, R = S * D, w.recurrent_model.recurrent_state_size
    L = Z + R
    du, nh = a.dense_units, a.mlp_layers
    mult = w.encoder.cnn_channels_multiplier
    stages = int(round(math.log2(cfg.env.screen_size) - 2))
    A = int(sum(actions_dim))
    wm, actor, critic = {}, {}, {}

    def mlp(d, prefix, i, hidden, n_hidden, o):
        for k in range(n_hidden):
            d[f"{prefix}{3 * k}.weight"] = (hidden, i if k == 0 else hidden)
            d[f"{prefix}{3 * k + 1}.weight"] = (hidden,)
            d[f"{prefix}{3 * k + 1}.bias"] = (hidden,)
        if o is not None:
            d[f"{prefix}{3 * n_hidden}.weight"] = (o, hidden)
            d[f"{prefix}{3 * n_hidden}.bias"] = (o,)

    has_cnn = len(a.cnn_keys.encoder) > 0
    vkeys, vdims = list(a.mlp_keys.encoder), dict(mlp_dims or {})
    chans = [in_channels] + [mult * 2 ** i for i in range(stages)]
    for i in range(stages if has_cnn else 0):
        p = f"encoder.cnn_encoder.model.0._model.{3 * i}"
        wm[p + ".weight"] = (chans[i + 1], chans[i], 4, 4)
        wm[f"encoder.cnn_encoder.model.0._model.{3 * i + 1}.weight"] = (chans[i + 1],)
        wm[f"encoder.cnn_encoder.model.0._model.{3 * i + 1}.bias"] = (chans[i + 1],)
    E = chans[-1] * 16 if has_cnn else 0
    Ev = w.encoder.dense_units if vkeys else 0
    if vkeys:
        mlp(wm, "encoder.mlp_encoder.model._model.", sum(vdims[k] for k in vkeys), w.encoder.dense_units,
            w.encoder.mlp_layers, None)
    dx = w.recurrent_model.dense_units
    wm["rssm.initial_recurrent_state"] = (R,)
    wm["rssm.recurrent_model.mlp._model.0.weight"] = (dx, Z + A)
    wm["rssm.recurrent_model.mlp._model.1.weight"] = (dx,)
    wm["rssm.recurrent_model.mlp._model.1.bias"] = (dx,)
    wm["rssm.recurrent_model.rnn.linear.weight"] = (3 * R, R + dx)
    wm["rssm.recurrent_model.rnn.layer_norm.weight"] = (3 * R,)
    wm["rssm.recurrent_model.rnn.layer_norm.bias"] = (3 * R,)
    mlp(wm, "rssm.representation_model._model.", (0 if w.decoupled_rssm else R) + E + Ev,
        w.representation_model.hidden_size, 1, Z)
    mlp(wm, "rssm.transition_model._model.", R, w.transition_model.hidden_size, 1, Z)
    has_cnn_dec = len(a.cnn_keys.decoder or []) > 0
    if has_cnn_dec:
        wm["observation_model.cnn_decoder.model.0.weight"] = (E, L)
        wm["observation_model.cnn_decoder.model.0.bias"] = (E,)
    dch = [chans[-1]] + [mult * 2 ** i for i in reversed(range(stages - 1))] + [
        decoder_channels(cfg, in_channels, cnn_dims) if has_cnn_dec else in_channels]
    for i in range(stages if has_cnn_dec else 0):
        p = f"observation_model.cnn_decoder.model.2._model.{3 * i}"
        wm[p + ".weight"] = (dch[i], dch[i + 1], 4, 4)
        if i == stages - 1:
            wm[p + ".bias"] = (dch[i + 1],)
        else:
            wm[f"observation_model.cnn_decoder.model.2._model.{3 * i + 1}.weight"] = (dch[i + 1],)
            wm[f"observation_model.cnn_decoder.model.2._model.{3 * i + 1}.bias"] = (dch[i + 1],)
    if a.mlp_keys.decoder:
        om = w.observation_model
        mlp(wm, "observation_model.mlp_decoder.model._model.", L, om.dense_units, om.mlp_layers, None)
        for i, k in enumerate(a.mlp_keys.decoder):
            wm[f"observation_model.mlp_decoder.heads.{i}.weight"] = (vdims[k], om.dense_units)
            wm[f"observation_model.mlp_decoder.heads.{i}.bias"] = (vdims[k],)
    mlp(wm, "reward_model._model.", L, du, nh, w.reward_model.bins)
    mlp(wm, "continue_model._model.", L, du, nh, 1)
    mlp(actor, "model._model.", L, du, nh, None)
    if is_continuous:
        actor["mlp_heads.0.weight"] = (2 * A, du)
        actor["mlp_heads.0.bias"] = (2 * A,)
    else:
        for i, ad in enumerate(actions_dim):
            actor[f"mlp_heads.{i}.weight"] = (ad, du)
            actor[f"mlp_heads.{i}.bias"] = (ad,)
    mlp(critic, "_model.", L, du, nh, a.critic.bins)
    return wm, actor, critic, dict(chans=chans, dch=dch, E=E, Ev=Ev, stages=stages)


def _check_supported_modules(cfg) -> None:
    a, w = cfg.algo, cfg.algo.world_model
    blocks = {"algo": a, "encoder": w.encoder, "observation_model": w.observation_model, "reward_model": w.reward_model,
              "discount_model": w.discount_model, "transition_model": w.transition_model,
              "representation_model": w.representation_model, "recurrent_model": w.recurrent_model, "actor": a.actor,
              "critic": a.critic}
    for name, blk in blocks.items():
        for key in ("dense_act", "cnn_act"):
            v = blk.get(key, None)
            if v is not None and not str(v).endswith("SiLU"):
                raise NotImplementedError(f"{name}.{key} = {v}: only torch.nn.SiLU is built")
        for key in ("layer_norm", "mlp_layer_norm", "cnn_layer_norm"):
            v = blk.get(key, None)
            if v is not None and "LayerNorm" not in str(v.get("cls", "LayerNorm")):
                raise NotImplementedError(f"{name}.{key}.cls = {v.get('cls')}: only the LayerNorm variants are built")
    for name in ("reward_model", "discount_model"):
        blk = blocks[name]
        if int(blk.get("dense_units", a.dense_units)) != int(a.dense_units) or int(blk.get("mlp_layers", a.mlp_layers)) != int(a.mlp_layers):
            raise NotImplementedError(f"world_model.{name}: dense_units / mlp_layers must equal algo.dense_units / algo.mlp_layers")
    if int(w.observation_model.get("cnn_channels_multiplier", w.encoder.cnn_channels_multiplier)) != int(w.encoder.cnn_channels_multiplier):
        raise NotImplementedError("observation_model.cnn_channels_multiplier must equal encoder.cnn_channels_multiplier")
    for name in ("actor", "critic"):
        blk = blocks[name]
        if int(blk.get("dense_units", a.dense_units)) != int(a.dense_units) or int(blk.get("mlp_layers", a.mlp_layers)) != int(a.mlp_layers):
            raise NotImplementedError(f"algo.{name}: dense_units / mlp_layers must equal algo.dense_units / algo.mlp_layers")


FUSED_DENSE_MAX_ROWS = 4096


def dense_ln_act(ops, x, W, gamma, beta, eps, act, out, pre=None, scratch=None):
    if x.shape[0] <= FUSED_DENSE_MAX_ROWS and ops.gemm_ln_supported(x, W):
        ops.gemm_ln_act(x, W, gamma, beta, eps, act, out, pre)
        return
    tmp = pre if pre is not None else scratch
    ops.gemm(x, W, tmp, False, True)
    ops.ln_act_fwd(tmp, gamma, beta, eps, act, out)


class _MLP:

    def __init__(self, eng, group: FlatGroup, prefix: str, in_dim: int, hidden: int, n_hidden: int,
                 out_dim: Optional[int], rows: int, eps: float, tag: str, train: bool):
        self.eng, self.g, self.prefix = eng, group, prefix
        self.in_dim, self.hidden, self.n_hidden, self.out_dim, self.eps = in_dim, hidden, n_hidden, out_dim, eps
        self.rows = rows
        new = eng._buf
        self.pre = [new(f"{tag}.pre{i}", rows, hidden) for i in range(n_hidden)]
        self.act = [new(f"{tag}.act{i}", rows, hidden) for i in range(n_hidden)]
        self.out = new(f"{tag}.out", rows, out_dim) if out_dim is not None else None
        if train:
            self.dact = new(f"{tag}.dact", rows, hidden)
            self.dpre = new(f"{tag}.dpre", rows, hidden)

    def W(self, i):
        return self.g.views[f"{self.prefix}{3 * i}.weight"]

    def forward(self, x: torch.Tensor, group: Optional[FlatGroup] = None, M: Optional[int] = None):
        ops = self.eng.ops
        g = group or self.g
        M = x.shape[0] if M is None else M
        cur = x
        for i in range(self.n_hidden):
            dense_ln_act(ops, cur, g.views[f"{self.prefix}{3 * i}.weight"], g.views[f"{self.prefix}{3 * i + 1}.weight"],
                         g.views[f"{self.prefix}{3 * i + 1}.bias"], self.eps, ACT_SILU, self.act[i][:M], self.pre[i][:M])
            cur = self.act[i][:M]
        if self.out_dim is None:
            return cur
        j = 3 * self.n_hidden
        ops.gemm(cur, g.views[f"{self.prefix}{j}.weight"], self.out[:M], False, True,
                 bias=g.views[f"{self.prefix}{j}.bias"])
        return self.out[:M]

    def backward(self, x: torch.Tensor, dout: torch.Tensor, dx: Optional[torch.Tensor], accumulate_dx: bool,
                 M: Optional[int] = None, data_only: bool = False, group: Optional[FlatGroup] = None):
        ops, g = self.eng.ops, group or self.g
        M = x.shape[0] if M is None else M
        if self.out_dim is not None:
            j = 3 * self.n_hidden
            last = self.act[-1][:M]
            if not data_only:
                ops.gemm(dout, last, g.gviews[f"{self.prefix}{j}.weight"], True, False)
                ops.col_sum(dout, g.gviews[f"{self.prefix}{j}.bias"])
            ops.gemm(dout, g.views[f"{self.prefix}{j}.weight"], self.dact[:M], False, False)
            d = self.dact[:M]
        else:
            d = dout
        for i in reversed(range(self.n_hidden)):
            ops.ln_act_bwd(self.pre[i][:M], g.views[f"{self.prefix}{3 * i + 1}.weight"],
                           g.views[f"{self.prefix}{3 * i + 1}.bias"], self.eps, ACT_SILU, d, self.dpre[:M],
                           None if data_only else g.gviews[f"{self.prefix}{3 * i + 1}.weight"],
                           None if data_only else g.gviews[f"{self.prefix}{3 * i + 1}.bias"])
            inp = x if i == 0 else self.act[i - 1][:M]
            if not data_only:
                ops.gemm(self.dpre[:M], inp, g.gviews[f"{self.prefix}{3 * i}.weight"], True, False)
            if i > 0:
                ops.gemm(self.dpre[:M], g.views[f"{self.prefix}{3 * i}.weight"], self.dact[:M], False, False)
                d = self.dact[:M]
            elif dx is not None:
                ops.gemm(self.dpre[:M], g.views[f"{self.prefix}0.weight"], dx, False, False, accumulate=accumulate_dx)


class DV3Engine:
    def __init__(self, cfg, actions_dim: Sequence[int], in_channels: int = 3, device="cuda", ops=None,
                 is_continuous: bool = False, groups=None, mlp_dims: Optional[Mapping[str, int]] = None,
                 cnn_dims: Optional[Mapping[str, int]] = None):
        a, w = cfg.algo, cfg.algo.world_model
        self.is_continuous = bool(is_continuous)
        if self.is_continuous and str(cfg.distribution.get("type", "auto")).lower() not in ("auto", "scaled_normal"):
            raise NotImplementedError(
                "continuous actions: distribution.type must be auto / scaled_normal — the reference's own train() fails "
                "with tanh_normal (entropy fallback shape, dreamer_v3.py:294-297) and normal (negative scale)")
        self.decoupled = bool(w.decoupled_rssm)
        _check_supported_modules(cfg)
        if not a.cnn_keys.encoder and not a.mlp_keys.encoder:
            raise ValueError("There must be at least one encoder, both cnn and mlp encoders are None")
        check_decoder_keys(cfg)
        actor_cls = str(a.actor.get("cls", "Actor"))
        if actor_cls.endswith("MinedojoActor"):
            raise NotImplementedError(f"algo.actor.cls = {actor_cls}: the action masks of the MineDojo actor are not built")
        self.cnn_keys = list(a.cnn_keys.encoder)
        self.has_cnn = len(self.cnn_keys) > 0
        self.vec_keys = list(a.mlp_keys.encoder)
        vd = dict(mlp_dims if mlp_dims is not None else (cfg.env.get("mlp_dims", None) or {}))
        self.vec_dims = [int(vd[k]) for k in self.vec_keys]
        self.Dv = sum(self.vec_dims)
        self.dec_cnn_keys = list(a.cnn_keys.decoder or [])
        self.has_cnn_dec = len(self.dec_cnn_keys) > 0
        self.cnn_dec_same = self.dec_cnn_keys == self.cnn_keys
        self.dec_vec_keys = list(a.mlp_keys.decoder or [])
        self.dec_vec_dims = [int(vd[k]) for k in self.dec_vec_keys]
        self.has_vec_dec = len(self.dec_vec_keys) > 0
        self.vec_dec_same = self.dec_vec_keys == self.vec_keys
        self.Dvd = sum(self.dec_vec_dims)
        self.cnn_dims = dict(cnn_dims if cnn_dims is not None else (cfg.env.get("cnn_channels", None) or {}))
        if ops is None:
            from sheeprl_b200.lib import CudaOps

            ops = CudaOps(device)
        self.ops = ops
        self.cfg = cfg
        self.device = torch.device(device)
        self.actions_dim = tuple(int(x) for x in actions_dim)
        self.Cin = in_channels
        self.T, self.B = a.per_rank_sequence_length, a.per_rank_batch_size
        self.N = self.T * self.B
        self.H = a.horizon
        self.S, self.D = w.stochastic_size, w.discrete_size
        self.Z, self.R = self.S * self.D, w.recurrent_model.recurrent_state_size
        self.L = self.Z + self.R
        self.Rh = 0 if self.decoupled else self.R
        self.A = int(sum(self.actions_dim))
        self.du, self.nh = a.dense_units, a.mlp_layers
        self.Dx = w.recurrent_model.dense_units
        self.Dt, self.Dr = w.transition_model.hidden_size, w.representation_model.hidden_size
        self.eps = float(a.mlp_layer_norm.kw.eps)
        self.ceps = float(a.cnn_layer_norm.kw.eps)
        self.unimix = float(a.unimix)
        self.img = cfg.env.screen_size
        self.key = a.cnn_keys.encoder[0] if self.has_cnn else None
        self.bins_r, self.bins_c = w.reward_model.bins, a.critic.bins
        self.Cdec = decoder_channels(cfg, in_channels, self.cnn_dims) if self.has_cnn_dec else 0
        wm_s, ac_s, cr_s, meta = dv3_param_shapes(cfg, self.actions_dim, in_channels, self.is_continuous,
                                                  dict(zip(self.vec_keys, self.vec_dims)), self.cnn_dims)
        self.Ev = meta["Ev"]
        self.AW = 2 * self.A if self.is_continuous else self.A
        self.chans, self.dch, self.E, self.stages = meta["chans"], meta["dch"], meta["E"], meta["stages"]
        if groups is not None:
            self.wm, self.actor, self.critic, self.target = groups
        else:
            self.wm = FlatGroup(wm_s, device)
            self.actor = FlatGroup(ac_s, device)
            self.critic = FlatGroup(cr_s, device)
            self.target = FlatGroup(cr_s, device, with_optimizer=False)
        self.moments_state = torch.zeros(2, dtype=torch.float32, device=device)
        self.world_size = 1
        self.allreduce = None
        self.allgather = None
        self.allreduce_async = None
        self.allreduce_join = None
        self._bufs: Dict[str, torch.Tensor] = {}
        self._alloc()

    def _buf(self, name: str, *shape, dtype=torch.float32) -> torch.Tensor:
        assert name not in self._bufs, name
        t = torch.zeros(*shape, dtype=dtype, device=self.device)
        self._bufs[name] = t
        return t

    def _buf_ld4(self, name: str, rows: int, cols: int) -> torch.Tensor:
        return self._buf(name, rows, (cols + 3) // 4 * 4)[:, :cols]

    def _alloc(self):
        N, T, B, H, Z, R, L, A, E = self.N, self.T, self.B, self.H, self.Z, self.R, self.L, self.A, self.E
        b = self._buf
        img = self.img
        n_st = self.stages if self.has_cnn else 0
        self.x0 = b("x0", N, img, img, self.Cin) if self.has_cnn else None
        self.enc_y, self.enc_a = [], []
        s = img
        for i in range(n_st):
            s //= 2
            self.enc_y.append(b(f"enc_y{i}", N, s, s, self.chans[i + 1]))
            self.enc_a.append(b(f"enc_a{i}", N, s, s, self.chans[i + 1]))
        self.emb = b("emb", N, E) if self.has_cnn else None
        self.pe = b("pe", N, self.Dr)
        we, wo = self.cfg.algo.world_model.encoder, self.cfg.algo.world_model.observation_model
        if self.vec_keys:
            self.vx = b("vx", N, self.Dv)
            self.venc = _MLP(self, self.wm, "encoder.mlp_encoder.model._model.", self.Dv, we.dense_units, we.mlp_layers, None,
                             N, float(we.mlp_layer_norm.kw.eps), "venc", True)
            self.d_emb_vec = b("d_emb_vec", N, self.Ev)
        if self.has_vec_dec:
            self.vdec = _MLP(self, self.wm, "observation_model.mlp_decoder.model._model.", L, wo.dense_units, wo.mlp_layers,
                             None, N, float(wo.mlp_layer_norm.kw.eps), "vdec", True)
            self.vrecon, self.vec_rows = b("vrecon", N, self.Dvd), b("vec_rows", N)
            self.d_vdec_hidden = b("d_vdec_hidden", N, wo.dense_units)
            self.vtgt = self.vx if self.vec_dec_same else b("vtgt", N, self.Dvd)
        self.traj = b("traj", H + 1, N, L)
        self.latent = self.traj[0]
        self.z_in, self.h_in, self.a_in = b("z_in", N, Z), b("h_in", N, R), b("a_in", N, A)
        self.x_pre, self.x_act = b("x_pre", N, self.Dx), b("x_act", N, self.Dx)
        self.g_pre, self.g_ln = b("g_pre", N, 3 * R), b("g_ln", N, 3 * R)
        self.tr_pre, self.tr_act = b("tr_pre", N, self.Dt), b("tr_act", N, self.Dt)
        self.rp_pre, self.rp_act = b("rp_pre", N, self.Dr), b("rp_act", N, self.Dr)
        self.post_raw, self.prior_raw = b("post_raw", N, Z), b("prior_raw", N, Z)
        self.post_mix, self.prior_mix = b("post_mix", N, Z), b("prior_mix", N, Z)
        self.h0, self.z0 = b("h0", 1, R), b("z0", 1, Z)
        self.init_tr_pre, self.init_tr_act = b("init_tr_pre", 1, self.Dt), b("init_tr_act", 1, self.Dt)
        self.init_raw = b("init_raw", 1, Z)
        self.zero_h, self.zero_z = b("zero_h", B, R), b("zero_z", B, Z)
        self.shift_actions = b("shift_actions", N, A)
        self.d_latent = b("d_latent", N, L)
        self.d_post_mix, self.d_prior_mix = b("d_post_mix", N, Z), b("d_prior_mix", N, Z)
        self.d_post_raw, self.d_prior_raw = b("d_post_raw", N, Z), b("d_prior_raw", N, Z)
        self.d_rp_act, self.d_rp_pre = b("d_rp_act", N, self.Dr), b("d_rp_pre", N, self.Dr)
        self.d_tr_act, self.d_tr_pre = b("d_tr_act", N, self.Dt), b("d_tr_pre", N, self.Dt)
        self.d_g_ln, self.d_g_pre = b("d_g_ln", N, 3 * R), b("d_g_pre", N, 3 * R)
        self.d_x_act, self.d_x_pre = b("d_x_act", N, self.Dx), b("d_x_pre", N, self.Dx)
        self.dz_carry, self.dh_carry = b("dz_carry", B, Z), b("dh_carry", B, R)
        self.dz_tot, self.dh_tot = b("dz_tot", B, Z), b("dh_tot", B, R)
        self.dh_in, self.dz_in = b("dh_in", B, R), b("dz_in", B, Z)
        self.d_h0 = b("d_h0", R)
        self.kl_rows = b("kl_rows", N, 4)
        self.dec_y, self.dec_a, self.d_dec_a, self.d_enc_a = [], [], [], []
        if self.has_cnn:
            self.d_emb = b("d_emb", N, E)
        if self.has_cnn_dec:
            self.dec_lin = b("dec_lin", N, E)
            C0 = self.dch[0]
            self.dec_in = b("dec_in", N, 4, 4, C0)
            s = 4
            for i in range(self.stages - 1):
                s *= 2
                self.dec_y.append(b(f"dec_y{i}", N, s, s, self.dch[i + 1]))
                self.dec_a.append(b(f"dec_a{i}", N, s, s, self.dch[i + 1]))
            self.recon = b("recon", N, img, img, self.Cdec)
            self.d_dec_in = b("d_dec_in", N, 4, 4, C0)
            self.d_dec_lin = b("d_dec_lin", N, E)
            self.d_dec_a = [b(f"d_dec_a{i}", *self.dec_a[i].shape) for i in range(self.stages - 1)]
            self.x_dec = self.x0 if self.cnn_dec_same else b("x_dec", N, img, img, self.Cdec)
        if self.has_cnn:
            self.d_enc_a = [b(f"d_enc_a{i}", *self.enc_a[i].shape) for i in range(self.stages)]
        self.obs_rows, self.rew_rows, self.cont_rows = b("obs_rows", N), b("rew_rows", N), b("cont_rows", N)
        self.metrics = b("metrics", 16)
        self.normsq = {k: self._buf(f"normsq_{k}", (), dtype=torch.float64) for k in ("wm", "actor", "critic")}
        self.norms = b("norms", 3)
        self.reward_wm = _MLP(self, self.wm, "reward_model._model.", L, self.du, self.nh, self.bins_r, N, self.eps,
                              "rew", True)
        self.cont_wm = _MLP(self, self.wm, "continue_model._model.", L, self.du, self.nh, 1, N, self.eps, "cont", True)
        self.d_rew_logits, self.d_cont_logit = self._buf_ld4("d_rew_logits", N, self.bins_r), b("d_cont_logit", N, 1)
        M1 = (H + 1) * N
        self.actions = b("img_actions", H + 1, N, A)
        self.actor_mlp = _MLP(self, self.actor, "model._model.", L, self.du, self.nh, None, M1, self.eps, "actor", True)
        self.actor_raw = b("actor_raw", M1, self.AW)
        self.d_actor_raw = b("d_actor_raw", H * N, self.AW)
        self.d_actor_hidden = b("d_actor_hidden", H * N, self.du)
        self.critic_mlp = _MLP(self, self.critic, "_model.", L, self.du, self.nh, self.bins_c, M1, self.eps,
                               "critic", True)
        self.target_mlp = _MLP(self, self.target, "_model.", L, self.du, self.nh, self.bins_c, H * N, self.eps,
                               "target", False)
        self.rew_img = _MLP(self, self.wm, "reward_model._model.", L, self.du, self.nh, self.bins_r, M1, self.eps,
                            "rew_img", self.is_continuous)
        self.cont_img = _MLP(self, self.wm, "continue_model._model.", L, self.du, self.nh, 1, M1, self.eps,
                             "cont_img", False)
        self.values, self.rew_pred = b("values", H + 1, N), b("rew_pred", H + 1, N)
        self.target_values = b("target_values", H * N)
        self.true_cont = b("true_cont", N)
        self.lam, self.discount = b("lam", H, N), b("discount", H + 1, N)
        self.moments_out = b("moments_out", 2)
        self.policy_rows = b("policy_rows", H * N)
        self.value_rows = b("value_rows", H * N)
        self.d_critic_logits = self._buf_ld4("d_critic_logits", H * N, self.bins_c)
        self.i_x_pre = b("i_x_pre", N, self.Dx)
        self.i_hx = b("i_hx", N, self.R + self.Dx)
        self.i_x_act = self.i_hx[:, self.R:]
        self.i_g_pre, self.i_g_ln = b("i_g_pre", N, 3 * R), b("i_g_ln", N, 3 * R)
        self.i_tr_pre, self.i_tr_act = b("i_tr_pre", N, self.Dt), b("i_tr_act", N, self.Dt)
        self.i_raw = b("i_raw", N, Z)
        if self.is_continuous:
            self.c_x_pre, self.c_hx = b("c_x_pre", H, N, self.Dx), b("c_hx", H, N, self.R + self.Dx)
            self.c_g_pre, self.c_g_ln = b("c_g_pre", H, N, 3 * R), b("c_g_ln", H, N, 3 * R)
            self.c_tr_pre, self.c_tr_act = b("c_tr_pre", H, N, self.Dt), b("c_tr_act", H, N, self.Dt)
            self.c_raw = b("c_raw", H, N, Z)
            self.act_ent = b("act_ent", M1)
            self.d_values, self.d_rew = b("d_values", H + 1, N), b("d_rew", H + 1, N)
            self.d_v_logits = self._buf_ld4("d_v_logits", M1, self.bins_c)
            self.d_r_logits = self._buf_ld4("d_r_logits", M1, self.bins_r)
            self.d_traj = b("d_traj", H + 1, N, L)
            self.cd_raw = b("cd_raw", N, Z)
            self.cd_tr_act, self.cd_tr_pre = b("cd_tr_act", N, self.Dt), b("cd_tr_pre", N, self.Dt)
            self.cd_g_ln, self.cd_g_pre = b("cd_g_ln", N, 3 * R), b("cd_g_pre", N, 3 * R)
            self.cd_x_act, self.cd_x_pre = b("cd_x_act", N, self.Dx), b("cd_x_pre", N, self.Dx)
            self.cd_dz, self.cd_dh = b("cd_dz", N, Z), b("cd_dh", N, R)
            self.cd_dz_carry, self.cd_dh_carry = b("cd_dz_carry", N, Z), b("cd_dh_carry", N, R)
            self.cd_a = b("cd_a", N, A)
        self.noise_post = b("noise_post", T, B, Z)
        self.noise_img_state = b("noise_img_state", H, N, Z)
        self.noise_img_action = b("noise_img_action", H + 1, N, A)
        self.rng_seed = int(self.cfg.get("seed", 0) or 0)
        self.rng_t = torch.zeros(1, dtype=torch.int32, device=self.device)
        self.cuda_graph = bool(self.cfg.algo.get("cuda_graph", True))
        prec = self.cfg.get("float32_matmul_precision", None)
        if prec is not None and hasattr(self.ops, "set_matmul_precision"):
            self.ops.set_matmul_precision(str(prec))
        self._graph = None
        if self.decoupled:
            has_scan, dims = hasattr(self.ops, "gru_scan_fwd"), self._gru_scan_dims()
            self.fused_scan = has_scan and self.ops.gru_scan_supported(dims, backward=False)
            self.fused_scan_bwd = has_scan and self.ops.gru_scan_supported(dims, backward=True)
        else:
            has_scan, dims = hasattr(self.ops, "rssm_scan_fwd"), self._scan_dims()
            self.fused_scan = has_scan and self.ops.rssm_scan_supported(dims, backward=False)
            self.fused_scan_bwd = has_scan and self.ops.rssm_scan_supported(dims, backward=True)
        self._scan_ws = None
        self._scan_q = None

    def optimizer_groups(self):
        return [self.wm, self.actor, self.critic]

    def use_cuda_graph(self) -> bool:
        return self.cuda_graph and self.device.type == "cuda" and type(self.ops).__name__ == "CudaOps"

    def graph_key(self) -> tuple:
        prec = self.ops.matmul_precision() if hasattr(self.ops, "matmul_precision") else "highest"
        return tuple((float(g.optimizer.lr), g.adam_kwargs().get("weight_decay", 0.0))
                     if getattr(g, "optimizer", None) is not None else -1.0 for g in self.optimizer_groups()) + (prec,)

    def step_graph(self):
        if self._graph is None:
            from sheeprl_b200.graph import StepGraph

            groups = self.optimizer_groups()

            def bump():
                for g in groups:
                    g.step += 1

            self._graph = StepGraph(self.device, warmup=2, on_replay=bump,
                                    host_state=(lambda: [g.step for g in groups],
                                                lambda s: [setattr(g, "step", v) for g, v in zip(groups, s)]))
        return self._graph

    def rng_state(self) -> Dict[str, torch.Tensor]:
        return {"rng_t": self.rng_t.detach().clone().cpu(), "rng_seed": torch.tensor(self.rng_seed)}

    def load_rng_state(self, st) -> None:
        self.rng_t.copy_(st["rng_t"].to(self.rng_t.device))
        self.rng_seed = int(st["rng_seed"])

    def bytes_allocated(self) -> int:
        tot = sum(t.numel() * t.element_size() for t in self._bufs.values())
        for g in (self.wm, self.actor, self.critic):
            tot += 4 * g.numel * 4
        return tot + self.target.numel * 4

    def _w(self, name):
        return self.wm.views[name]

    def _gw(self, name):
        return self.wm.gviews[name]

    def train_step(self, data: Dict[str, torch.Tensor], noise: Optional[Dict[str, torch.Tensor]] = None):
        self._draw_noise(noise)
        self._world_model_phase(data)
        self._imagine()
        self._behaviour_losses()
        return self.metrics

    def _draw_noise(self, noise: Optional[Dict[str, torch.Tensor]]):
        ops = self.ops
        T, B, N, H, Z = self.T, self.B, self.N, self.H, self.Z
        if noise is None:
            ops.increment(self.rng_t)
            ops.fill_exponential(self.noise_post.view(-1), self.rng_seed, 0, self.rng_t)
            ops.fill_exponential(self.noise_img_state.view(-1), self.rng_seed, 1, self.rng_t)
            if self.is_continuous:
                ops.fill_normal(self.noise_img_action.view(-1), self.rng_seed, 2, self.rng_t)
            else:
                ops.fill_exponential(self.noise_img_action.view(-1), self.rng_seed, 2, self.rng_t)
        else:
            self.noise_post.copy_(noise["post"].reshape(T, B, Z))
            self.noise_img_state.copy_(noise["img_state"].reshape(H, N, Z))
            self.noise_img_action.copy_(torch.cat([x for x in noise["img_action"]], -1))

    def _world_model_phase(self, data: Dict[str, torch.Tensor], heads_detached: bool = False):
        ops = self.ops
        B, N, R, A = self.B, self.N, self.R, self.A
        w = self.cfg.algo.world_model
        if self.has_cnn:
            ops.obs_prep(self.image_batch(data, N), self.x0)
        off = 0
        for k, d in zip(self.vec_keys, self.vec_dims):
            ops.symlog(data[k].reshape(N, d), self.vx[:, off:off + d])
            off += d
        if self.has_cnn_dec and not self.cnn_dec_same:
            ops.obs_prep(self.image_batch(data, N, self.dec_cnn_keys), self.x_dec)
        if self.has_vec_dec and not self.vec_dec_same:
            off = 0
            for k, d in zip(self.dec_vec_keys, self.dec_vec_dims):
                ops.symlog(data[k].reshape(N, d), self.vtgt[:, off:off + d])
                off += d
        data["is_first"][0].fill_(1.0)
        first = data["is_first"].reshape(N)
        ops.zero(self.shift_actions[:B])
        ops.copy(data["actions"].reshape(N, A)[: N - B], self.shift_actions[B:])
        rewards = data["rewards"].reshape(N)
        ops.affine(data["terminated"].reshape(N), self.true_cont, -1.0, 1.0)

        self._encoder_forward()
        self._project_embedding(self.rp_pre if self.decoupled else self.pe)
        self._scan_forward(first)
        self._decoder_forward()
        rew_logits = self.reward_wm.forward(self.latent)
        cont_logit = self.cont_wm.forward(self.latent)

        inv = 1.0 / N
        if self.has_cnn_dec:
            P = self.img * self.img * self.Cdec
            ops.mse_loss_grad(self.recon.view(N, P), self.x_dec.view(N, P), inv, self.obs_rows, self.recon.view(N, P))
        if self.has_vec_dec:
            rows = self.vec_rows if self.has_cnn_dec else self.obs_rows
            ops.mse_loss_grad(self.vrecon, self.vtgt, inv, rows, self.vrecon)
            if self.has_cnn_dec:
                ops.axpy(self.vec_rows, self.obs_rows)
        ops.twohot_loss_grad(rew_logits, rewards, None, inv, TWOHOT_LOW, TWOHOT_HIGH, self.rew_rows, self.d_rew_logits)
        ops.bce_loss_grad(cont_logit, self.true_cont, float(w.continue_scale_factor), inv, self.cont_rows,
                          self.d_cont_logit)
        ops.kl_loss_grad(self.post_mix, self.prior_mix, self.S, self.D, float(w.kl_dynamic),
                         float(w.kl_representation), float(w.kl_free_nats), float(w.kl_regularizer), inv,
                         self.d_post_mix, self.d_prior_mix, self.kl_rows)
        ops.sum_rows(self.obs_rows.view(N, 1), self.metrics[1:2], inv)
        ops.sum_rows(self.rew_rows.view(N, 1), self.metrics[2:3], inv)
        ops.sum_rows(self.cont_rows.view(N, 1), self.metrics[4:5], inv)
        ops.sum_rows(self.kl_rows[:, 1:2], self.metrics[3:4], inv)
        ops.sum_rows(self.kl_rows[:, 0:1], self.metrics[5:6], inv)
        ops.sum_rows(self.kl_rows[:, 2:4], self.metrics[6:8], inv)
        ops.zero(self.metrics[0:1])
        ops.axpy(self.metrics[1:2], self.metrics[0:1])
        ops.axpy(self.metrics[2:3], self.metrics[0:1])
        ops.axpy(self.metrics[3:4], self.metrics[0:1], float(w.kl_regularizer))
        ops.axpy(self.metrics[4:5], self.metrics[0:1])

        ops.zero(self.wm.grad)
        self._decoder_backward()
        self.reward_wm.backward(self.latent, self.d_rew_logits, None if heads_detached else self.d_latent, True)
        self.cont_wm.backward(self.latent, self.d_cont_logit, None if heads_detached else self.d_latent, True)
        b_enc, b_tail = self._wm_buckets()
        overlap = self.allreduce_async is not None and bool(self.cfg.algo.get("overlap_allreduce", not self.fused_scan))
        if overlap:
            self.allreduce_async(self.wm.grad[b_tail:])
        self._scan_backward(first)
        if overlap:
            self.allreduce_async(self.wm.grad[b_enc:b_tail])
        self._encoder_backward()
        if overlap:
            self.allreduce_async(self.wm.grad[:b_enc])
            self.allreduce_join()
        self._optimizer_step("wm", self.wm, float(w.clip_gradients or 0.0), w.optimizer, 0, reduced=overlap)

    def _enc_names(self, i):
        p = "encoder.cnn_encoder.model.0._model."
        return f"{p}{3 * i}.weight", f"{p}{3 * i + 1}.weight", f"{p}{3 * i + 1}.bias"

    def _dec_names(self, i):
        p = "observation_model.cnn_decoder.model.2._model."
        return f"{p}{3 * i}.weight", f"{p}{3 * i + 1}.weight", f"{p}{3 * i + 1}.bias"

    def image_batch(self, obs: Dict[str, torch.Tensor], rows: int, keys: Optional[Sequence[str]] = None) -> torch.Tensor:
        keys = self.cnn_keys if keys is None else keys
        C = self.Cin if keys is self.cnn_keys else self.Cdec
        imgs = [obs[k].reshape(rows, -1, self.img, self.img) for k in keys]
        if len(imgs) == 1:
            return imgs[0]
        if any(t.dtype != imgs[0].dtype for t in imgs):
            imgs = [t.float() for t in imgs]
        out = torch.cat(imgs, 1)
        assert out.shape[1] == C, f"image keys {keys} carry {out.shape[1]} channels, the network was built for {C}"
        return out

    def _project_embedding(self, out: torch.Tensor):
        ops, R, E = self.ops, self.Rh, self.E
        Wr1 = self._w("rssm.representation_model._model.0.weight")
        if self.has_cnn:
            ops.gemm(self.emb, Wr1[:, R:R + E], out, False, True)
        if self.vec_keys:
            ops.gemm(self.venc.act[-1], Wr1[:, R + E:], out, False, True, accumulate=self.has_cnn)

    def _encoder_forward(self):
        ops = self.ops
        if self.vec_keys:
            self.venc.forward(self.vx)
        if not self.has_cnn:
            return
        cur = self.x0
        for i in range(self.stages):
            wn, gn, bn = self._enc_names(i)
            ops.conv_down(cur, self._w(wn), self.enc_y[i])
            C = self.chans[i + 1]
            ops.ln_act_fwd(self.enc_y[i].view(-1, C), self._w(gn), self._w(bn), self.ceps, ACT_SILU,
                           self.enc_a[i].view(-1, C))
            cur = self.enc_a[i]
        C = self.chans[-1]
        ops.transpose_batched(cur.view(self.N, 16, C), self.emb.view(self.N, C, 16))

    def _encoder_backward(self):
        ops = self.ops
        if self.vec_keys:
            self.venc.backward(self.vx, self.d_emb_vec, None, False)
        if not self.has_cnn:
            return
        C = self.chans[-1]
        ops.transpose_batched(self.d_emb.view(self.N, C, 16), self.d_enc_a[-1].view(self.N, 16, C))
        for i in reversed(range(self.stages)):
            wn, gn, bn = self._enc_names(i)
            C = self.chans[i + 1]
            d = self.d_enc_a[i].view(-1, C)
            ops.ln_act_bwd(self.enc_y[i].view(-1, C), self._w(gn), self._w(bn), self.ceps, ACT_SILU, d, d,
                           self._gw(gn), self._gw(bn))
            inp = self.x0 if i == 0 else self.enc_a[i - 1]
            ops.conv_wgrad(self.d_enc_a[i], inp, self._gw(wn))
            if i > 0:
                ops.conv_up(self.d_enc_a[i], self._w(wn), self.d_enc_a[i - 1])

    def _vec_heads(self):
        out, off = [], 0
        for i, d in enumerate(self.dec_vec_dims):
            out.append((f"observation_model.mlp_decoder.heads.{i}", off, d))
            off += d
        return out

    def _decoder_forward(self):
        ops = self.ops
        if self.has_vec_dec:
            hid = self.vdec.forward(self.latent)
            for name, off, d in self._vec_heads():
                ops.gemm(hid, self._w(name + ".weight"), self.vrecon[:, off:off + d], False, True, bias=self._w(name + ".bias"))
        if not self.has_cnn_dec:
            return
        p = "observation_model.cnn_decoder.model."
        ops.gemm(self.latent, self._w(p + "0.weight"), self.dec_lin, False, True, bias=self._w(p + "0.bias"))
        C0 = self.dch[0]
        ops.transpose_batched(self.dec_lin.view(self.N, C0, 16), self.dec_in.view(self.N, 16, C0))
        cur = self.dec_in
        for i in range(self.stages - 1):
            wn, gn, bn = self._dec_names(i)
            C = self.dch[i + 1]
            ops.conv_up(cur, self._w(wn), self.dec_y[i])
            ops.ln_act_fwd(self.dec_y[i].view(-1, C), self._w(gn), self._w(bn), self.ceps, ACT_SILU,
                           self.dec_a[i].view(-1, C))
            cur = self.dec_a[i]
        wn = self._dec_names(self.stages - 1)[0]
        ops.conv_up(cur, self._w(wn), self.recon, bias=self._w(wn.replace(".weight", ".bias")))

    def _decoder_backward(self):
        ops = self.ops
        if self.has_cnn_dec:
            self._cnn_decoder_backward()
        if self.has_vec_dec:
            hid = self.vdec.act[-1]
            ops.zero(self.d_vdec_hidden)
            for name, off, d in self._vec_heads():
                dv = self.vrecon[:, off:off + d]
                ops.gemm(dv, hid, self._gw(name + ".weight"), True, False)
                ops.col_sum(dv, self._gw(name + ".bias"))
                ops.gemm(dv, self._w(name + ".weight"), self.d_vdec_hidden, False, False, accumulate=True)
            self.vdec.backward(self.latent, self.d_vdec_hidden, self.d_latent, self.has_cnn_dec)

    def _cnn_decoder_backward(self):
        ops = self.ops
        st = self.stages
        wn = self._dec_names(st - 1)[0]
        d_big = self.recon
        ops.col_sum(d_big.view(-1, self.Cdec), self._gw(wn.replace(".weight", ".bias")))
        for i in reversed(range(st)):
            wn, gn, bn = self._dec_names(i)
            inp = self.dec_in if i == 0 else self.dec_a[i - 1]
            d_inp = self.d_dec_in if i == 0 else self.d_dec_a[i - 1]
            ops.conv_wgrad(inp, d_big, self._gw(wn))
            ops.conv_down(d_big, self._w(wn), d_inp)
            if i > 0:
                gn_p, bn_p = self._dec_names(i - 1)[1:]
                C = self.dch[i]
                d = d_inp.view(-1, C)
                ops.ln_act_bwd(self.dec_y[i - 1].view(-1, C), self._w(gn_p), self._w(bn_p), self.ceps, ACT_SILU, d, d,
                               self._gw(gn_p), self._gw(bn_p))
            d_big = d_inp
        C0 = self.dch[0]
        ops.transpose_batched(self.d_dec_in.view(self.N, 16, C0), self.d_dec_lin.view(self.N, C0, 16))
        p = "observation_model.cnn_decoder.model."
        ops.gemm(self.d_dec_lin, self.latent, self._gw(p + "0.weight"), True, False)
        ops.col_sum(self.d_dec_lin, self._gw(p + "0.bias"))
        ops.gemm(self.d_dec_lin, self._w(p + "0.weight"), self.d_latent, False, False)

    def _recurrent_forward(self, z, act, h_prev, x_pre, x_act, g_pre, g_ln, h_out, win_t=None, hx=None, h_next=None,
                           keep: bool = True):
        self._recurrent_input(z, act, x_pre, x_act, win_t, keep)
        return self._gru_forward(h_prev, x_act, g_pre, g_ln, h_out, hx, h_next, keep)

    def _recurrent_input(self, z, act, x_pre, x_act, win_t=None, keep: bool = True):
        ops, Z = self.ops, self.Z
        p = "rssm.recurrent_model."
        Win = self._w(p + "mlp._model.0.weight")
        fused_x = win_t is not None and ops.onehot_linear_ln_supported(win_t, x_act, x_pre if keep else None)
        if fused_x:
            ops.onehot_linear_ln(z, act, win_t, self._w(p + "mlp._model.1.weight"), self._w(p + "mlp._model.1.bias"),
                                 self.eps, x_act, self.S, self.D, pre=x_pre if keep else None)
        elif win_t is not None:
            ops.onehot_linear(z, act, win_t, x_pre, self.S, self.D)
        else:
            ops.gemm(z, Win[:, :Z], x_pre, False, True)
            ops.gemm(act, Win[:, Z:], x_pre, False, True, accumulate=True)
        if not fused_x:
            ops.ln_act_fwd(x_pre, self._w(p + "mlp._model.1.weight"), self._w(p + "mlp._model.1.bias"), self.eps,
                           ACT_SILU, x_act)

    def _gru_forward(self, h_prev, x_act, g_pre, g_ln, h_out, hx=None, h_next=None, keep: bool = True):
        ops, R = self.ops, self.R
        p = "rssm.recurrent_model."
        Wg = self._w(p + "rnn.linear.weight")
        if hx is not None and hx.shape[0] <= FUSED_DENSE_MAX_ROWS and ops.gemm_ln_supported(hx, Wg, 1):
            ops.gemm_ln_gru(hx, Wg, self._w(p + "rnn.layer_norm.weight"), self._w(p + "rnn.layer_norm.bias"), self.eps,
                            h_prev, h_out, h_next, g_pre if keep else None, g_ln if keep else None)
            return True
        if hx is not None:
            ops.gemm(hx, Wg, g_pre, False, True)
        else:
            ops.gemm(h_prev, Wg[:, :R], g_pre, False, True, accumulate=x_act is None)
            if x_act is not None:
                ops.gemm(x_act, Wg[:, R:], g_pre, False, True, accumulate=True)
        ops.ln_act_fwd(g_pre, self._w(p + "rnn.layer_norm.weight"), self._w(p + "rnn.layer_norm.bias"), self.eps,
                       ACT_NONE, g_ln)
        ops.gru_gate_fwd(g_ln, h_prev, h_out)
        return False

    def _recurrent_backward(self, g_ln, h_prev, g_pre, x_pre, dh, d_g_ln, d_g_pre, d_x_act, d_x_pre, dh_prev, dz,
                            da=None):
        ops, Z, R = self.ops, self.Z, self.R
        p = "rssm.recurrent_model."
        Win, Wg = self._w(p + "mlp._model.0.weight"), self._w(p + "rnn.linear.weight")
        self._gru_backward(g_ln, h_prev, g_pre, dh, d_g_ln, d_g_pre, dh_prev)
        ops.gemm(d_g_pre, Wg[:, R:], d_x_act, False, False)
        ops.ln_act_bwd(x_pre, self._w(p + "mlp._model.1.weight"), self._w(p + "mlp._model.1.bias"), self.eps, ACT_SILU,
                       d_x_act, d_x_pre, None, None)
        ops.gemm(d_x_pre, Win[:, :Z], dz, False, False)
        if da is not None:
            ops.gemm(d_x_pre, Win[:, Z:], da, False, False)

    def _gru_backward(self, g_ln, h_prev, g_pre, dh, d_g_ln, d_g_pre, dh_prev):
        ops = self.ops
        p = "rssm.recurrent_model.rnn."
        ops.gru_gate_bwd(g_ln, h_prev, dh, d_g_ln, dh_prev)
        ops.ln_act_bwd(g_pre, self._w(p + "layer_norm.weight"), self._w(p + "layer_norm.bias"), self.eps, ACT_NONE,
                       d_g_ln, d_g_pre, None, None)
        ops.gemm(d_g_pre, self._w(p + "linear.weight")[:, :self.R], dh_prev, False, False, accumulate=True)

    def _transition_forward(self, h, tr_pre, tr_act, raw, keep: bool = True):
        ops = self.ops
        p = "rssm.transition_model._model."
        dense_ln_act(ops, h, self._w(p + "0.weight"), self._w(p + "1.weight"), self._w(p + "1.bias"), self.eps, ACT_SILU,
                     tr_act, tr_pre if keep else None, scratch=tr_pre)
        ops.gemm(tr_act, self._w(p + "3.weight"), raw, False, True, bias=self._w(p + "3.bias"))

    def _transition_backward(self, raw, tr_pre, dz, dmix, d_raw, d_tr_act, d_tr_pre, dh, ln_grads: bool = False):
        ops = self.ops
        p = "rssm.transition_model._model."
        ops.cat_sample_bwd(raw, dz, dmix, self.unimix, self.S, self.D, d_raw)
        ops.gemm(d_raw, self._w(p + "3.weight"), d_tr_act, False, False)
        ops.ln_act_bwd(tr_pre, self._w(p + "1.weight"), self._w(p + "1.bias"), self.eps, ACT_SILU, d_tr_act, d_tr_pre,
                       self._gw(p + "1.weight") if ln_grads else None, self._gw(p + "1.bias") if ln_grads else None)
        ops.gemm(d_tr_pre, self._w(p + "0.weight"), dh, False, False, accumulate=True)

    def _posterior_forward(self, h, rp_pre, rp_act, raw, noise, z_out, mix_out=None):
        ops, R = self.ops, self.R
        pr = "rssm.representation_model._model."
        if h is not None:
            ops.gemm(h, self._w(pr + "0.weight")[:, :R], rp_pre, False, True, accumulate=True)
        ops.ln_act_fwd(rp_pre, self._w(pr + "1.weight"), self._w(pr + "1.bias"), self.eps, ACT_SILU, rp_act)
        ops.gemm(rp_act, self._w(pr + "3.weight"), raw, False, True, bias=self._w(pr + "3.bias"))
        ops.cat_sample(raw, noise, self.unimix, self.S, self.D, z_out, mix_out)

    def _scan_forward(self, first: torch.Tensor):
        ops, B, Z, R = self.ops, self.B, self.Z, self.R
        ops.tanh_fwd(self._w("rssm.initial_recurrent_state").view(1, R), self.h0)
        self._transition_forward(self.h0, self.init_tr_pre, self.init_tr_act, self.init_raw)
        ops.cat_sample(self.init_raw, None, self.unimix, self.S, self.D, self.z0)
        if self.decoupled:
            self._scan_forward_decoupled(first)
        elif self.fused_scan:
            self._scan_forward_fused(first)
        for t in (() if self.fused_scan or self.decoupled else range(self.T)):
            s = slice(t * B, (t + 1) * B)
            f = first[s]
            if t == 0:
                zp, hp = self.zero_z, self.zero_h
            else:
                sp = slice((t - 1) * B, t * B)
                zp, hp = self.latent[sp, :Z], self.latent[sp, Z:]
            ops.mask_rows(self.shift_actions[s], f, self.a_in[s])
            ops.mask_mix(hp, self.h0, f, self.h_in[s])
            ops.mask_mix(zp, self.z0, f, self.z_in[s])
            h = self.latent[s, Z:]
            self._recurrent_forward(self.z_in[s], self.a_in[s], self.h_in[s], self.x_pre[s], self.x_act[s],
                                    self.g_pre[s], self.g_ln[s], h)
            ops.copy(self.pe[s], self.rp_pre[s])
            self._posterior_forward(h, self.rp_pre[s], self.rp_act[s], self.post_raw[s], self.noise_post[t],
                                    self.latent[s, :Z], self.post_mix[s])
        self._prior_forward()

    def _scan_forward_decoupled(self, first: torch.Tensor):
        ops, B, N, Z, R = self.ops, self.B, self.N, self.Z, self.R
        self._posterior_forward(None, self.rp_pre, self.rp_act, self.post_raw, self.noise_post.view(N, Z),
                                self.latent[:, :Z], self.post_mix)
        ops.mask_mix(self.zero_z, self.z0, first[:B], self.z_in[:B])
        if N > B:
            ops.mask_mix(self.latent[:N - B, :Z], self.z0, first[B:], self.z_in[B:])
        ops.mask_rows(self.shift_actions, first, self.a_in)
        self._recurrent_input(self.z_in, self.a_in, self.x_pre, self.x_act)
        ops.gemm(self.x_act, self._w("rssm.recurrent_model.rnn.linear.weight")[:, R:], self.g_pre, False, True)
        if self.fused_scan:
            if self._scan_ws is None:
                self._scan_ws = ops.gru_scan_workspace(self.T, B, R)
            ops.gru_scan_fwd(self._gru_scan_dims(), self.eps, self._gru_scan_tensors(first), self._scan_ws)
            return
        for t in range(self.T):
            s = slice(t * B, (t + 1) * B)
            hp = self.zero_h if t == 0 else self.latent[(t - 1) * B:t * B, Z:]
            ops.mask_mix(hp, self.h0, first[s], self.h_in[s])
            self._gru_forward(self.h_in[s], None, self.g_pre[s], self.g_ln[s], self.latent[s, Z:])

    def _gru_scan_dims(self):
        return dict(T=self.T, B=self.B, R=self.R, ld_wg=self.R + self.Dx, ld_lat=self.L, lat_off=self.Z)

    def _gru_scan_tensors(self, first: torch.Tensor):
        p = "rssm.recurrent_model.rnn."
        return dict(W_g=self._w(p + "linear.weight"), lng_g=self._w(p + "layer_norm.weight"),
                    lng_b=self._w(p + "layer_norm.bias"), h0=self.h0, first=first, g_pre=self.g_pre, g_ln=self.g_ln,
                    h_in=self.h_in, latent=self.latent)

    def _prior_forward(self):
        Z = self.Z
        self._transition_forward(self.latent[:, Z:], self.tr_pre, self.tr_act, self.prior_raw)
        self.ops.cat_sample(self.prior_raw, None, self.unimix, self.S, self.D, None, self.prior_mix)

    def _scan_forward_fused(self, first: torch.Tensor):
        if self._scan_ws is None:
            self._scan_ws = self.ops.rssm_scan_workspace(self.T, self.B, self.S, self.D, self.Dx, self.R, self.Dr)
        self.ops.rssm_scan_fwd(self._scan_dims(), self.eps, self.unimix, self._scan_tensors(first), self._scan_ws)

    def _scan_dims(self):
        return dict(T=self.T, B=self.B, S=self.S, D=self.D, R=self.R, A=self.A, Dx=self.Dx, Dt=self.Dt, Dr=self.Dr,
                    ld_lat=self.L, ld_wr1=self.Rh + self.E + self.Ev)

    def _scan_tensors(self, first: torch.Tensor):
        p = "rssm.recurrent_model."
        pt, pr = "rssm.transition_model._model.", "rssm.representation_model._model."
        w = self._w
        return dict(
            W_in=w(p + "mlp._model.0.weight"), lnx_g=w(p + "mlp._model.1.weight"), lnx_b=w(p + "mlp._model.1.bias"),
            W_g=w(p + "rnn.linear.weight"), lng_g=w(p + "rnn.layer_norm.weight"), lng_b=w(p + "rnn.layer_norm.bias"),
            W_t1=w(pt + "0.weight"), lnt_g=w(pt + "1.weight"), lnt_b=w(pt + "1.bias"), W_t2=w(pt + "3.weight"),
            b_t2=w(pt + "3.bias"), W_r1=w(pr + "0.weight"), lnr_g=w(pr + "1.weight"), lnr_b=w(pr + "1.bias"),
            W_r2=w(pr + "3.weight"), b_r2=w(pr + "3.bias"), h0=self.h0, z0=self.z0, pe=self.pe,
            actions=self.shift_actions, first=first, noise=self.noise_post, latent=self.latent, z_in=self.z_in,
            h_in=self.h_in, a_in=self.a_in, x_pre=self.x_pre, x_act=self.x_act, g_pre=self.g_pre, g_ln=self.g_ln,
            tr_pre=self.tr_pre, tr_act=self.tr_act, rp_pre=self.rp_pre, rp_act=self.rp_act, post_raw=self.post_raw,
            prior_raw=self.prior_raw, post_mix=self.post_mix, prior_mix=self.prior_mix)

    def _prior_backward(self):
        self._transition_backward(self.prior_raw, self.tr_pre, None, self.d_prior_mix, self.d_prior_raw, self.d_tr_act,
                                  self.d_tr_pre, self.d_latent[:, self.Z:], ln_grads=True)

    def _scan_backward_fused(self, first: torch.Tensor):
        ops, Z, R = self.ops, self.Z, self.R
        if self._scan_q is None:
            new = lambda *shape: torch.zeros(*shape, dtype=torch.float32, device=self.device)
            self._scan_q = (new(self.N, R), new(self.N, R + self.Dx), new(self.N, Z))
        q_r, q_g, q_x = self._scan_q
        grads = dict(d_latent=self.d_latent, d_post_mix=self.d_post_mix, d_prior_mix=self.d_prior_mix,
                     d_post_raw=self.d_post_raw, d_prior_raw=self.d_prior_raw, d_rp_act=self.d_rp_act,
                     d_rp_pre=self.d_rp_pre, d_tr_act=self.d_tr_act, d_tr_pre=self.d_tr_pre, d_g_ln=self.d_g_ln,
                     d_g_pre=self.d_g_pre, d_x_act=self.d_x_act, d_x_pre=self.d_x_pre, d_h0=self.d_h0,
                     q_r=q_r, q_g=q_g, q_x=q_x)
        p, pr = "rssm.recurrent_model.", "rssm.representation_model._model."
        ops.gemm(self.rp_pre, self._w(pr + "0.weight")[:, :R], q_r, False, False)
        ops.gemm(self.g_pre, self._w(p + "rnn.linear.weight"), q_g, False, False)
        ops.gemm(self.x_pre, self._w(p + "mlp._model.0.weight")[:, :Z], q_x, False, False)
        ops.rssm_scan_bwd(self._scan_dims(), self.eps, self.unimix, self._scan_tensors(first), grads, self._scan_ws)

    def _scan_backward(self, first: torch.Tensor):
        ops, B, Z, R = self.ops, self.B, self.Z, self.R
        pt, pr = "rssm.transition_model._model.", "rssm.representation_model._model."
        Wr1 = self._w(pr + "0.weight")
        ops.zero(self.dz_carry)
        ops.zero(self.dh_carry)
        ops.zero(self.d_h0)
        self._prior_backward()
        fused = self.fused_scan and self.fused_scan_bwd
        if self.decoupled:
            self._scan_backward_decoupled(first, fused)
        elif fused:
            self._scan_backward_fused(first)
        for t in (() if fused or self.decoupled else reversed(range(self.T))):
            s = slice(t * B, (t + 1) * B)
            f = first[s]
            ops.copy(self.d_latent[s, :Z], self.dz_tot)
            ops.axpy(self.dz_carry, self.dz_tot)
            ops.copy(self.d_latent[s, Z:], self.dh_tot)
            ops.axpy(self.dh_carry, self.dh_tot)
            ops.cat_sample_bwd(self.post_raw[s], self.dz_tot, self.d_post_mix[s], self.unimix, self.S, self.D,
                               self.d_post_raw[s])
            ops.gemm(self.d_post_raw[s], self._w(pr + "3.weight"), self.d_rp_act[s], False, False)
            ops.ln_act_bwd(self.rp_pre[s], self._w(pr + "1.weight"), self._w(pr + "1.bias"), self.eps, ACT_SILU,
                           self.d_rp_act[s], self.d_rp_pre[s], None, None)
            ops.gemm(self.d_rp_pre[s], Wr1[:, :R], self.dh_tot, False, False, accumulate=True)
            self._recurrent_backward(self.g_ln[s], self.h_in[s], self.g_pre[s], self.x_pre[s], self.dh_tot,
                                     self.d_g_ln[s], self.d_g_pre[s], self.d_x_act[s], self.d_x_pre[s], self.dh_in,
                                     self.dz_in)
            ops.mask_bwd(self.dz_in, f, self.dz_carry, None)
            ops.mask_bwd(self.dh_in, f, self.dh_carry, self.d_h0)
        self._representation_param_grads()
        gW, h_all = self._gw, self.latent[:, Z:]
        ops.gemm(self.d_prior_raw, self.tr_act, gW(pt + "3.weight"), True, False)
        ops.col_sum(self.d_prior_raw, gW(pt + "3.bias"))
        ops.gemm(self.d_tr_pre, h_all, gW(pt + "0.weight"), True, False)
        if not self.decoupled:
            self._recurrent_param_grads()
        if self.cfg.algo.world_model.get("learnable_initial_recurrent_state", True):
            ops.tanh_bwd(self.h0.view(R), self.d_h0, gW("rssm.initial_recurrent_state"))

    def _representation_param_grads(self):
        ops, R, E, Z, gW = self.ops, self.Rh, self.E, self.Z, self._gw
        pr = "rssm.representation_model._model."
        Wr1 = self._w(pr + "0.weight")
        ops.gemm(self.d_post_raw, self.rp_act, gW(pr + "3.weight"), True, False)
        ops.col_sum(self.d_post_raw, gW(pr + "3.bias"))
        ops.ln_act_bwd(self.rp_pre, self._w(pr + "1.weight"), self._w(pr + "1.bias"), self.eps, ACT_SILU,
                       self.d_rp_act, self.d_rp_pre, gW(pr + "1.weight"), gW(pr + "1.bias"))
        gWr1 = gW(pr + "0.weight")
        if R:
            ops.gemm(self.d_rp_pre, self.latent[:, Z:], gWr1[:, :R], True, False)
        if self.has_cnn:
            ops.gemm(self.d_rp_pre, self.emb, gWr1[:, R:R + E], True, False)
            ops.gemm(self.d_rp_pre, Wr1[:, R:R + E], self.d_emb, False, False)
        if self.vec_keys:
            ops.gemm(self.d_rp_pre, self.venc.act[-1], gWr1[:, R + E:], True, False)
            ops.gemm(self.d_rp_pre, Wr1[:, R + E:], self.d_emb_vec, False, False)

    def _recurrent_param_grads(self, x_data_grad: bool = False):
        ops, Z, R, gW = self.ops, self.Z, self.R, self._gw
        p = "rssm.recurrent_model."
        ops.ln_act_bwd(self.g_pre, self._w(p + "rnn.layer_norm.weight"), self._w(p + "rnn.layer_norm.bias"),
                       self.eps, ACT_NONE, self.d_g_ln, self.d_g_pre, gW(p + "rnn.layer_norm.weight"),
                       gW(p + "rnn.layer_norm.bias"))
        gWg = gW(p + "rnn.linear.weight")
        ops.gemm(self.d_g_pre, self.h_in, gWg[:, :R], True, False)
        ops.gemm(self.d_g_pre, self.x_act, gWg[:, R:], True, False)
        if x_data_grad:
            ops.gemm(self.d_g_pre, self._w(p + "rnn.linear.weight")[:, R:], self.d_x_act, False, False)
        ops.ln_act_bwd(self.x_pre, self._w(p + "mlp._model.1.weight"), self._w(p + "mlp._model.1.bias"), self.eps,
                       ACT_SILU, self.d_x_act, self.d_x_pre, gW(p + "mlp._model.1.weight"),
                       gW(p + "mlp._model.1.bias"))
        gWin = gW(p + "mlp._model.0.weight")
        ops.gemm(self.d_x_pre, self.z_in, gWin[:, :Z], True, False)
        ops.gemm(self.d_x_pre, self.a_in, gWin[:, Z:], True, False)

    def _scan_backward_decoupled(self, first: torch.Tensor, fused: bool):
        ops, B, N, Z, R = self.ops, self.B, self.N, self.Z, self.R
        p, pr = "rssm.recurrent_model.", "rssm.representation_model._model."
        if fused:
            if self._scan_q is None:
                self._scan_q = torch.zeros(N, R, dtype=torch.float32, device=self.device)
            ops.gemm(self.g_pre, self._w(p + "rnn.linear.weight")[:, :R], self._scan_q, False, False)
            ops.gru_scan_bwd(self._gru_scan_dims(), self.eps, self._gru_scan_tensors(first),
                             dict(d_latent=self.d_latent, d_g_ln=self.d_g_ln, d_h0=self.d_h0, q_g=self._scan_q),
                             self._scan_ws)
        for t in (() if fused else reversed(range(self.T))):
            s = slice(t * B, (t + 1) * B)
            ops.copy(self.d_latent[s, Z:], self.dh_tot)
            ops.axpy(self.dh_carry, self.dh_tot)
            self._gru_backward(self.g_ln[s], self.h_in[s], self.g_pre[s], self.dh_tot, self.d_g_ln[s], self.d_g_pre[s],
                               self.dh_in)
            ops.mask_bwd(self.dh_in, first[s], self.dh_carry, self.d_h0)
        self._recurrent_param_grads(x_data_grad=True)
        if N > B:
            ops.mask_rows(self.d_x_pre, first, self.d_x_act)
            ops.gemm(self.d_x_act[B:], self._w(p + "mlp._model.0.weight")[:, :Z], self.d_latent[:N - B, :Z], False, False,
                     accumulate=True)
        ops.cat_sample_bwd(self.post_raw, self.d_latent[:, :Z], self.d_post_mix, self.unimix, self.S, self.D,
                           self.d_post_raw)
        ops.gemm(self.d_post_raw, self._w(pr + "3.weight"), self.d_rp_act, False, False)

    def _wm_buckets(self):
        off = self.wm.offsets
        b_enc = off["rssm.initial_recurrent_state"]
        tail = [v for k, v in off.items() if not (k.startswith("encoder.") or k.startswith("rssm."))]
        return b_enc, min(tail)

    def _optimizer_step(self, name: str, g: FlatGroup, max_norm: float, ocfg, slot: int, reduced: bool = False):
        ops = self.ops
        if self.allreduce is not None and not reduced:
            self.allreduce(g.grad, name)
        ops.sumsq(g.grad, self.normsq[name])
        g.step += 1
        ops.increment(g.step_t)
        b1, b2 = ocfg.betas
        opt = getattr(g, "optimizer", None)
        lr = opt.lr if opt is not None else float(ocfg.lr)
        ops.adam_step(g.flat, g.grad, g.exp_avg, g.exp_avg_sq, self.normsq[name], max_norm, lr,
                      float(b1), float(b2), float(ocfg.eps), g.step_t, self.norms[slot: slot + 1],
                      **g.adam_kwargs(ocfg.get("weight_decay", 0.0)))

    def _actor_heads(self, hidden: torch.Tensor, raw_out: torch.Tensor, actor: Optional[FlatGroup] = None):
        actor = actor or self.actor
        if self.is_continuous:
            self.ops.gemm(hidden, actor.views["mlp_heads.0.weight"], raw_out, False, True,
                          bias=actor.views["mlp_heads.0.bias"])
            return
        off = 0
        for i, ad in enumerate(self.actions_dim):
            self.ops.gemm(hidden, actor.views[f"mlp_heads.{i}.weight"], raw_out[:, off:off + ad], False, True,
                          bias=actor.views[f"mlp_heads.{i}.bias"])
            off += ad

    def _imagine(self, actor: Optional[FlatGroup] = None, actor_mlp: Optional["_MLP"] = None):
        ops, N, Z, R, H = self.ops, self.N, self.Z, self.R, self.H
        actor = actor or self.actor
        am = actor_mlp or self.actor_mlp
        Win = self._w("rssm.recurrent_model.mlp._model.0.weight")
        gather = ops.onehot_linear_supported(self.S, self.D, self.A, Win.shape[0])
        if gather:
            if getattr(self, "_win_t", None) is None:
                self._win_t = torch.empty(Win.shape[1], Win.shape[0], dtype=torch.float32, device=self.device)
            ops.transpose2d(Win, self._win_t)
        h_staged = False
        for i in range(H + 1):
            rows = slice(i * N, (i + 1) * N)
            if i > 0:
                prev, cur = self.traj[i - 1], self.traj[i]
                if self.is_continuous:
                    j = i - 1
                    x_pre, hx, g_pre, g_ln = self.c_x_pre[j], self.c_hx[j], self.c_g_pre[j], self.c_g_ln[j]
                    tr_pre, tr_act, raw = self.c_tr_pre[j], self.c_tr_act[j], self.c_raw[j]
                else:
                    x_pre, hx, g_pre, g_ln = self.i_x_pre, self.i_hx, self.i_g_pre, self.i_g_ln
                    tr_pre, tr_act, raw = self.i_tr_pre, self.i_tr_act, self.i_raw
                if not h_staged:
                    ops.copy(prev[:, Z:], hx[:, :R])
                keep = self.is_continuous
                h_next = None
                if i < H:
                    h_next = (self.c_hx[i] if self.is_continuous else hx)[:, :R]
                h_staged = self._recurrent_forward(prev[:, :Z], self.actions[i - 1], prev[:, Z:], x_pre, hx[:, R:], g_pre,
                                                   g_ln, cur[:, Z:], win_t=self._win_t if gather else None, hx=hx,
                                                   h_next=h_next, keep=keep) and h_next is not None
                self._transition_forward(cur[:, Z:], tr_pre, tr_act, raw, keep=keep)
                ops.cat_sample(raw, self.noise_img_state[i - 1], self.unimix, self.S, self.D, cur[:, :Z])
            x = self.traj[i]
            cur_in = x
            for l in range(am.n_hidden):
                dense_ln_act(ops, cur_in, am.W(l), actor.views[f"model._model.{3 * l + 1}.weight"],
                             actor.views[f"model._model.{3 * l + 1}.bias"], self.eps, ACT_SILU, am.act[l][rows],
                             am.pre[l][rows])
                cur_in = am.act[l][rows]
            if not self.is_continuous:
                off, done = 0, True
                for k, ad in enumerate(self.actions_dim):
                    Wh = actor.views[f"mlp_heads.{k}.weight"]
                    done = done and ops.head_sample_supported(cur_in, Wh)
                if done:
                    for k, ad in enumerate(self.actions_dim):
                        ops.head_sample(cur_in, actor.views[f"mlp_heads.{k}.weight"], actor.views[f"mlp_heads.{k}.bias"],
                                        self.noise_img_action[i, :, off:off + ad], self.unimix,
                                        self.actor_raw[rows, off:off + ad], self.actions[i, :, off:off + ad])
                        off += ad
                    continue
            self._actor_heads(cur_in, self.actor_raw[rows], actor)
            if self.is_continuous:
                ac = self.cfg.algo.actor
                ops.cont_action_fwd(self.actor_raw[rows], self.noise_img_action[i], self.actions[i], self.act_ent[rows],
                                    float(ac.min_std), float(ac.max_std), float(ac.init_std), float(ac.action_clip))
                continue
            off = 0
            for k, ad in enumerate(self.actions_dim):
                ops.cat_sample(self.actor_raw[rows, off:off + ad], self.noise_img_action[i, :, off:off + ad],
                               self.unimix, 1, ad, self.actions[i, :, off:off + ad])
                off += ad


    def _continuous_policy_gradient(self, c_logit, critics):
        ops, N, H, Z, R, L = self.ops, self.N, self.H, self.Z, self.R, self.L
        a = self.cfg.algo
        ac = a.actor
        M1, M0 = (H + 1) * N, H * N
        traj2, d_traj2 = self.traj.view(M1, L), self.d_traj.view(M1, L)
        for j, (mlp, v_logits, values, lam, moments, share, r_logits, rows) in enumerate(critics):
            ops.lambda_returns_bwd(c_logit.view(H + 1, N), self.discount, moments, lam, values, self.act_ent,
                                   float(a.gamma), float(a.lmbda), float(ac.ent_coef) / share if j == 0 else 0.0,
                                   share / M0, self.d_values, self.d_rew, rows.view(H, N))
            ops.twohot_mean_bwd(v_logits, self.d_values.view(-1), TWOHOT_LOW, TWOHOT_HIGH, self.d_v_logits)
            if r_logits is not None:
                ops.twohot_mean_bwd(r_logits, self.d_rew.view(-1), TWOHOT_LOW, TWOHOT_HIGH, self.d_r_logits)
            mlp.backward(traj2, self.d_v_logits, d_traj2, j > 0, data_only=True)
            if r_logits is not None:
                self.rew_img.backward(traj2, self.d_r_logits, d_traj2, True, data_only=True)
        args = (float(ac.min_std), float(ac.max_std), float(ac.init_std), float(ac.action_clip))
        ops.zero(self.cd_dz_carry)
        ops.zero(self.cd_dh_carry)
        for i in range(H, 0, -1):
            j = i - 1
            ops.copy(self.d_traj[i][:, :Z], self.cd_dz)
            ops.axpy(self.cd_dz_carry, self.cd_dz)
            ops.copy(self.d_traj[i][:, Z:], self.cd_dh)
            ops.axpy(self.cd_dh_carry, self.cd_dh)
            self._transition_backward(self.c_raw[j], self.c_tr_pre[j], self.cd_dz, None, self.cd_raw, self.cd_tr_act,
                                      self.cd_tr_pre, self.cd_dh)
            self._recurrent_backward(self.c_g_ln[j], self.c_hx[j][:, :R], self.c_g_pre[j], self.c_x_pre[j], self.cd_dh,
                                     self.cd_g_ln, self.cd_g_pre, self.cd_x_act, self.cd_x_pre, self.cd_dh_carry,
                                     self.cd_dz_carry, da=self.cd_a)
            rows = slice(j * N, (j + 1) * N)
            ops.cont_action_bwd(self.actor_raw[rows], self.noise_img_action[j], self.cd_a, self.discount[j],
                                self.d_actor_raw[rows], *args, -float(ac.ent_coef) / M0)

    def _behaviour_losses(self):
        ops, N, H, L = self.ops, self.N, self.H, self.L
        a = self.cfg.algo
        M1, M0 = (H + 1) * N, H * N
        traj2 = self.traj.view(M1, L)
        v_logits = self.critic_mlp.forward(traj2)
        ops.twohot_mean(v_logits, TWOHOT_LOW, TWOHOT_HIGH, self.values.view(-1))
        r_logits = self.rew_img.forward(traj2)
        ops.twohot_mean(r_logits, TWOHOT_LOW, TWOHOT_HIGH, self.rew_pred.view(-1))
        c_logit = self.cont_img.forward(traj2)
        ops.lambda_returns(self.rew_pred, self.values, c_logit.view(H + 1, N), self.true_cont, float(a.gamma),
                           float(a.lmbda), self.lam, self.discount)
        mo = a.actor.moments
        lam_all = self.lam if self.allgather is None else self.allgather(self.lam)
        ops.moments_update(lam_all.view(-1), self.moments_state, float(mo.decay), float(mo.max),
                           float(mo.percentile.low), float(mo.percentile.high), self.moments_out)
        if self.is_continuous:
            self._continuous_policy_gradient(c_logit, [(self.critic_mlp, v_logits, self.values, self.lam, self.moments_out,
                                                        1.0, r_logits, self.policy_rows)])
        else:
            ops.actor_loss_grad(self.actor_raw[:M0], self.actions.view(M1, self.A)[:M0], self.lam.view(-1),
                                self.values.view(-1)[:M0], self.discount.view(-1)[:M0], self.moments_out,
                                self.actions_dim, self.unimix, float(a.actor.ent_coef), 1.0 / M0, self.policy_rows,
                                self.d_actor_raw)
        ops.sum_rows(self.policy_rows.view(M0, 1), self.metrics[8:9], -1.0 / M0)
        self._actor_update(self.actor, self.actor_mlp, "actor", 1)
        self._critic_update(self.critic, self.critic_mlp, self.target_mlp, v_logits, self.lam, self.metrics[9:10],
                            "critic", 2)

    def _actor_update(self, actor: FlatGroup, am: "_MLP", name: str, slot: int):
        ops, N, H, L = self.ops, self.N, self.H, self.L
        a = self.cfg.algo
        M1, M0 = (H + 1) * N, H * N
        traj2 = self.traj.view(M1, L)
        ops.zero(actor.grad)
        last = am.act[-1][:M0]
        ops.zero(self.d_actor_hidden)
        off = 0
        for i, ad in enumerate((self.AW,) if self.is_continuous else self.actions_dim):
            d = self.d_actor_raw[:, off:off + ad]
            ops.gemm(d, last, actor.gviews[f"mlp_heads.{i}.weight"], True, False)
            ops.col_sum(d, actor.gviews[f"mlp_heads.{i}.bias"])
            ops.gemm(d, actor.views[f"mlp_heads.{i}.weight"], self.d_actor_hidden, False, False, accumulate=True)
            off += ad
        am.backward(traj2[:M0], self.d_actor_hidden, None, False, M=M0)
        self._optimizer_step(name, actor, float(a.actor.clip_gradients or 0.0), a.actor.optimizer, slot)

    def _critic_update(self, critic: FlatGroup, cm: "_MLP", tm: "_MLP", v_logits: torch.Tensor, lam: torch.Tensor,
                       metric: torch.Tensor, name: str, slot: int):
        ops, N, H, L = self.ops, self.N, self.H, self.L
        a = self.cfg.algo
        M1, M0 = (H + 1) * N, H * N
        traj2 = self.traj.view(M1, L)
        t_logits = tm.forward(traj2[:M0])
        ops.twohot_mean(t_logits, TWOHOT_LOW, TWOHOT_HIGH, self.target_values)
        disc = self.discount.view(-1)[:M0]
        ops.twohot_loss_grad(v_logits[:M0], lam.view(-1), disc, 1.0 / M0, TWOHOT_LOW, TWOHOT_HIGH,
                             self.value_rows, self.d_critic_logits)
        ops.twohot_loss_grad(v_logits[:M0], self.target_values, disc, 1.0 / M0, TWOHOT_LOW, TWOHOT_HIGH,
                             self.value_rows, self.d_critic_logits, accumulate=True)
        ops.weighted_mean(self.value_rows, disc, 1.0 / M0, metric)
        ops.zero(critic.grad)
        cm.backward(traj2[:M0], self.d_critic_logits, None, False, M=M0)
        self._optimizer_step(name, critic, float(a.critic.clip_gradients or 0.0), a.critic.optimizer, slot)

    METRIC_NAMES = (
        "Loss/world_model_loss", "Loss/observation_loss", "Loss/reward_loss", "Loss/state_loss",
        "Loss/continue_loss", "State/kl", "State/post_entropy", "State/prior_entropy", "Loss/policy_loss",
        "Loss/value_loss",
    )

    def metrics_dict(self) -> Dict[str, torch.Tensor]:
        d = {n: self.metrics[i] for i, n in enumerate(self.METRIC_NAMES)}
        d["Grads/world_model"], d["Grads/actor"], d["Grads/critic"] = self.norms[0], self.norms[1], self.norms[2]
        return d

    def update_target(self, tau: float):
        if tau >= 1.0:
            self.ops.copy(self.critic.flat, self.target.flat)
        else:
            self.ops.ema(self.target.flat, self.critic.flat, float(tau))
```

sheeprl_b200/lib.py:

```python
from __future__ import annotations

import ctypes
import os
import re
from typing import Optional, Sequence

import torch

_HERE = os.path.dirname(os.path.abspath(__file__))
LIB_PATH = os.path.join(_HERE, "libb200rl.so")
HEADER_PATH = os.path.join(os.path.dirname(_HERE), "include", "b200rl.h")

_lib = None

PRESPLIT_MIN_ROWS = 4096


class B200RLError(RuntimeError):
    pass


_SCALARS = {"int": ctypes.c_int, "long long": ctypes.c_longlong, "unsigned int": ctypes.c_uint,
            "unsigned long long": ctypes.c_ulonglong, "float": ctypes.c_float}


def _decl(text: str, where: Optional[str] = None, result: bool = False):
    m = re.fullmatch(r"\s*(.+?)\s*\b(\w+)\s*", text, re.S)
    if m is None:
        raise B200RLError(f"{where}: cannot parse the declaration {text.strip()!r}")
    words = m.group(1).replace("*", " * ").split()
    base = " ".join(w for w in words if w not in ("const", "*"))
    if "*" in words or base == "cudaStream_t":
        return m.group(2), ctypes.c_char_p if result and base == "char" else ctypes.c_void_p
    if base not in _SCALARS:
        raise B200RLError(f"{where or m.group(2)}: C type {m.group(1)!r} has no ctypes binding")
    return m.group(2), _SCALARS[base]


def parse_header(text: str):
    text = re.sub(r"/\*.*?\*/|^\s*#[^\n]*", " ", text, flags=re.S | re.M)
    structs, typedef = {}, r"typedef\s+struct\s+\w+\s*\{(.*?)\}\s*(\w+)\s*;"
    for body, name in re.findall(typedef, text, re.S):
        structs[name] = []
        for stmt in filter(str.strip, body.split(";")):
            first, *more = stmt.split(",")
            base = re.match(r"\s*(.*?)[\s*]*\w+\s*$", first, re.S).group(1)
            structs[name] += [_decl(d, name) for d in [first] + [base + " " + d for d in more]]
    functions = {}
    for stmt in re.sub(typedef, " ", text, flags=re.S).split(";"):
        stmt = re.split(r"[{}]", stmt)[-1].strip()
        if not stmt:
            continue
        m = re.fullmatch(r"(.+?)\((.*)\)", stmt, re.S)
        if m is None:
            raise B200RLError(f"cannot parse the declaration {stmt!r}")
        name, restype = _decl(m.group(1), result=True)
        params = m.group(2).strip()
        functions[name] = (restype, [] if params in ("", "void") else [_decl(p, name)[1] for p in params.split(",")])
    return functions, structs


with open(HEADER_PATH) as _f:
    _FUNCTIONS, _STRUCTS = parse_header(_f.read())


def _bind(fn, restype, argtypes):
    fn.restype, fn.argtypes, n = restype, argtypes, len(argtypes)

    def call(*args):
        if len(args) != n:
            raise TypeError(f"{fn.__name__} takes {n} arguments ({len(args)} given)")
        return fn(*args)

    call.__name__, call.restype, call.argtypes = fn.__name__, restype, argtypes
    return call


def load_library(path: str = LIB_PATH) -> ctypes.CDLL:
    global _lib
    if _lib is None:
        if not os.path.exists(path):
            raise B200RLError(f"{path} not found: build it with `python -m sheeprl_b200.build` (nvcc, sm_90a). "
                              "The B200 engine has no CPU / PyTorch fallback.")
        lib = ctypes.CDLL(path)
        for name, (restype, argtypes) in _FUNCTIONS.items():
            setattr(lib, name, _bind(getattr(lib, name), restype, argtypes))
        _lib = lib
    return _lib


def declared_symbols() -> Sequence[str]:
    return sorted(_FUNCTIONS)


def _p(t: Optional[torch.Tensor]):
    return None if t is None else t.data_ptr()


def _ld(t: Optional[torch.Tensor]) -> int:
    if t is None:
        return 0
    if t.dim() == 1:
        assert t.numel() <= 1 or t.stride(0) == 1, "1-D views must be contiguous"
        return max(t.numel(), 1)
    assert t.dim() == 2, f"expected a 2-D view, got {tuple(t.shape)}"
    assert t.shape[1] == 1 or t.stride(1) == 1, f"inner stride must be 1, got {t.stride()}"
    return t.stride(0) if t.shape[0] > 1 else max(t.stride(0), t.shape[1])


def _f32(*ts):
    for t in ts:
        if t is not None:
            assert t.dtype == torch.float32 and t.is_cuda, (t.dtype, t.device)


def _struct(name: str, typedef: str, exclude=()):
    fields = _STRUCTS[typedef]
    pointers = tuple(n for n, t in fields if t is ctypes.c_void_p and n not in exclude)
    return type(name, (ctypes.Structure,), {"_fields_": fields, "POINTERS": pointers})


RssmScanArgs = _struct("RssmScanArgs", "b200rl_rssm_scan_args", exclude=("workspace",))
RssmScanGrads = _struct("RssmScanGrads", "b200rl_rssm_scan_grads")
GruScanArgs = _struct("GruScanArgs", "b200rl_gru_scan_args", exclude=("workspace",))
GruScanGrads = _struct("GruScanGrads", "b200rl_gru_scan_grads")


class CudaOps:
    name = "cuda"

    def __init__(self, device="cuda"):
        if not torch.cuda.is_available():
            raise B200RLError("no CUDA device visible: the B200 engine has no CPU fallback")
        self.lib = load_library()
        self.device = torch.device(device)
        if self.device.index is not None:
            torch.cuda.set_device(self.device)
        if self.lib.b200rl_device_check() != 0:
            raise B200RLError(self.lib.b200rl_last_error().decode())
        self.launches = 0
        self.use_tc = os.environ.get("B200RL_DISABLE_TC", "0") != "1"
        self._pack_bufs = {}
        self._scratch_bufs = {}

    def _st(self):
        return torch.cuda.current_stream().cuda_stream

    def _ck(self, rc: int, launches: int = 1):
        self.launches += launches
        if rc != 0:
            raise B200RLError(self.lib.b200rl_last_error().decode())

    def set_matmul_precision(self, precision: str) -> None:
        p = str(precision).lower()
        if p not in ("highest", "high", "medium"):
            raise ValueError(f"float32_matmul_precision must be highest / high / medium, got {precision}")
        self._ck(self.lib.b200rl_set_matmul_precision(3 if p == "highest" else 1), 0)

    def matmul_precision(self) -> str:
        return "highest" if self.lib.b200rl_get_matmul_precision() == 3 else "high"

    def gemm(self, A, B, C, transA: bool, transB: bool, bias=None, accumulate: bool = False):
        _f32(A, B, C, bias)
        M, N = C.shape
        K = A.shape[0] if transA else A.shape[1]
        assert (A.shape[1] if transA else A.shape[0]) == M, (A.shape, C.shape, transA)
        assert (B.shape[0] if transB else B.shape[1]) == N and (B.shape[1] if transB else B.shape[0]) == K, \
            (A.shape, B.shape, C.shape, transA, transB)
        if (not transA and M >= PRESPLIT_MIN_ROWS and self.use_tc
                and self.lib.b200rl_gemm_tc_supported(_p(A), _p(B), M, N, K, _ld(A), _ld(B), 0, int(transB))):
            hi, lo, ld = self._planes(B, transB, N, K)
            self._ck(self.lib.b200rl_gemm_tc_presplit(_p(A), _p(hi), _p(lo), _p(C), _p(bias), M, N, K, _ld(A), ld, _ld(C),
                                                      int(accumulate), self._st()))
            return
        self._ck(self.lib.b200rl_gemm_f32(_p(A), _p(B), _p(C), _p(bias), M, N, K, _ld(A), _ld(B), _ld(C), int(transA),
                                          int(transB), int(accumulate), self._st()))

    def _planes(self, B, transB: bool, N: int, K: int):
        ldb = _ld(B)
        ld = ldb if transB else (K + 3) // 4 * 4
        buf = self._scratch("b_planes", 2 * N * ld)
        hi, lo = buf[:N * ld], buf[N * ld:2 * N * ld]
        if transB:
            self._ck(self.lib.b200rl_tf32_split(_p(B), _p(hi), _p(lo), (N - 1) * ldb + K, self._st()))
        else:
            self._ck(self.lib.b200rl_tf32_split_t(_p(B), _p(hi), _p(lo), K, N, ldb, ld, self._st()))
        return hi, lo, ld

    def gemm_ln_supported(self, A, W, mode: int = 0) -> bool:
        M, K = A.shape
        return self.use_tc and bool(self.lib.b200rl_gemm_ln_supported(_p(A), _p(W), M, W.shape[0], K, _ld(A), _ld(W),
                                                                     mode))

    def gemm_ln_act(self, A, W, gamma, beta, eps: float, act: int, out, pre=None):
        _f32(A, W, gamma, beta, out, pre)
        M, K = A.shape
        N = W.shape[0]
        assert W.shape[1] == K and out.shape == (M, N)
        self._ck(self.lib.b200rl_gemm_ln(_p(A), _p(W), M, N, K, _ld(A), _ld(W), _p(gamma), _p(beta), eps, act, _p(pre),
                                         _ld(pre), _p(out), _ld(out), 0, None, 0, None, 0, None, 0, self._st()), 2)

    def gemm_ln_gru(self, A, W, gamma, beta, eps: float, h_prev, h_out, h_out2=None, g_pre=None, g_ln=None):
        _f32(A, W, gamma, beta, h_prev, h_out, h_out2, g_pre, g_ln)
        M, K = A.shape
        N = W.shape[0]
        assert W.shape[1] == K and h_prev.shape == (M, N // 3) and h_out.shape == (M, N // 3)
        self._ck(self.lib.b200rl_gemm_ln(_p(A), _p(W), M, N, K, _ld(A), _ld(W), _p(gamma), _p(beta), eps, 0, _p(g_pre),
                                         _ld(g_pre), _p(g_ln), _ld(g_ln), 1, _p(h_prev), _ld(h_prev), _p(h_out),
                                         _ld(h_out), _p(h_out2), _ld(h_out2), self._st()), 2)

    def _scratch(self, slot: str, numel: int) -> torch.Tensor:
        buf = self._scratch_bufs.get(slot)
        if buf is None or buf.numel() < numel:
            buf = torch.empty(numel, dtype=torch.float32, device=self.device)
            self._scratch_bufs[slot] = buf
        return buf

    def col_sum(self, X, out, accumulate: bool = False):
        _f32(X, out)
        self._ck(self.lib.b200rl_col_sum(_p(X), _p(out), X.shape[0], X.shape[1], _ld(X), int(accumulate), self._st()))

    def ln_act_fwd(self, X, gamma, beta, eps: float, act: int, Y):
        _f32(X, gamma, beta, Y)
        self._ck(self.lib.b200rl_ln_act_fwd(_p(X), _p(gamma), _p(beta), _p(Y), X.shape[0], X.shape[1], _ld(X), _ld(Y),
                                            eps, act, self._st()))

    def ln_act_bwd(self, X, gamma, beta, eps: float, act: int, dY, dX, dgamma, dbeta, accumulate: bool = False):
        _f32(X, gamma, beta, dY, dX, dgamma, dbeta)
        self._ck(self.lib.b200rl_ln_act_bwd(_p(X), _p(gamma), _p(beta), _p(dY), _p(dX), _p(dgamma), _p(dbeta),
                                            X.shape[0], X.shape[1], _ld(X), _ld(dY), _ld(dX), eps, act,
                                            int(accumulate), self._st()))

    def obs_prep(self, obs, out):
        assert obs.is_cuda and obs.is_contiguous() and out.is_contiguous()
        assert obs.dtype in (torch.uint8, torch.float32), obs.dtype
        NB, C, H, W = obs.shape
        self._ck(self.lib.b200rl_obs_prep(_p(obs), int(obs.dtype == torch.uint8), _p(out), NB, C, H * W, self._st()))

    def transpose_batched(self, X, Y):
        _f32(X, Y)
        assert X.is_contiguous() and Y.is_contiguous()
        NB, a, b = X.shape
        self._ck(self.lib.b200rl_transpose_batched(_p(X), _p(Y), NB, a, b, self._st()))

    def conv_down(self, big, W, small):
        _f32(big, W, small)
        assert big.is_contiguous() and small.is_contiguous() and W.is_contiguous()
        NB, h, w, Cs = small.shape
        Cb = big.shape[-1]
        assert tuple(big.shape) == (NB, 2 * h, 2 * w, Cb) and tuple(W.shape) == (Cs, Cb, 4, 4)
        if self.use_tc and self.lib.b200rl_conv_tc_supported(0, NB, h, w, Cs, Cb):
            hi, lo = self._packed(W, 0, Cs, Cb)
            self._ck(self.lib.b200rl_conv_down_tc_presplit(_p(big), _p(hi), _p(lo), _p(small), NB, h, w, Cs, Cb,
                                                           self._st()))
            return
        self._ck(self.lib.b200rl_conv_down(_p(big), _p(W), _p(small), NB, h, w, Cs, Cb, self._st()))

    def _packed(self, W, mode_up: int, Cs: int, Cb: int):
        key = (W.data_ptr(), mode_up)
        buf = self._pack_bufs.get(key)
        need = self.lib.b200rl_conv_pack_floats(mode_up, Cs, Cb)
        if buf is None or buf.shape != (2, need):
            buf = torch.empty(2, need, dtype=torch.float32, device=W.device)
            self._pack_bufs[key] = buf
        self._ck(self.lib.b200rl_conv_pack_split(_p(W), _p(buf[0]), _p(buf[1]), mode_up, Cs, Cb, self._st()))
        return buf[0], buf[1]

    def conv_up(self, small, W, big, bias=None):
        _f32(big, W, small, bias)
        assert big.is_contiguous() and small.is_contiguous() and W.is_contiguous()
        NB, h, w, Cs = small.shape
        Cb = big.shape[-1]
        assert tuple(big.shape) == (NB, 2 * h, 2 * w, Cb) and tuple(W.shape) == (Cs, Cb, 4, 4)
        if self.use_tc and self.lib.b200rl_conv_tc_supported(1, NB, h, w, Cs, Cb):
            hi, lo = self._packed(W, 1, Cs, Cb)
            self._ck(self.lib.b200rl_conv_up_tc_presplit(_p(small), _p(hi), _p(lo), _p(big), _p(bias), NB, h, w, Cs, Cb,
                                                         self._st()))
            return
        self._ck(self.lib.b200rl_conv_up(_p(small), _p(W), _p(big), _p(bias), NB, h, w, Cs, Cb, self._st()))

    def conv_wgrad(self, small, big, dW, accumulate: bool = False):
        _f32(big, dW, small)
        assert big.is_contiguous() and small.is_contiguous() and dW.is_contiguous()
        NB, h, w, Cs = small.shape
        Cb = big.shape[-1]
        assert tuple(big.shape) == (NB, 2 * h, 2 * w, Cb) and tuple(dW.shape) == (Cs, Cb, 4, 4)
        if self.use_tc and self.lib.b200rl_conv_wgrad_tc_supported(NB, h, w, Cs, Cb):
            ws = self._scratch("wgrad", self.lib.b200rl_conv_wgrad_tc_workspace(NB, h, w, Cs, Cb))
            self._ck(self.lib.b200rl_conv_wgrad_tc(_p(small), _p(big), _p(dW), _p(ws), NB, h, w, Cs, Cb,
                                                   int(accumulate), self._st()))
            return
        self._ck(self.lib.b200rl_conv_wgrad(_p(small), _p(big), _p(dW), NB, h, w, Cs, Cb, int(accumulate), self._st()))

    def gru_gate_fwd(self, G, Hin, Hout):
        _f32(G, Hin, Hout)
        M, R = Hin.shape
        self._ck(self.lib.b200rl_gru_gate_fwd(_p(G), _p(Hin), _p(Hout), M, R, _ld(G), _ld(Hin), _ld(Hout), self._st()))

    def gru_gate_bwd(self, G, Hin, dH, dG, dHin):
        _f32(G, Hin, dH, dG, dHin)
        M, R = Hin.shape
        self._ck(self.lib.b200rl_gru_gate_bwd(_p(G), _p(Hin), _p(dH), _p(dG), _p(dHin), M, R, _ld(G), _ld(Hin), _ld(dH),
                                              _ld(dG), _ld(dHin), self._st()))

    def mask_mix(self, prev, init, first, out):
        _f32(prev, init, first, out)
        M, C = out.shape
        self._ck(self.lib.b200rl_mask_mix(_p(prev), _p(init), _p(first), _p(out), M, C, _ld(prev), _ld(out), self._st()))

    def mask_rows(self, X, first, out):
        self.mask_mix(X, None, first, out)

    def mask_bwd(self, dIn, first, dPrev, dInit):
        _f32(dIn, first, dPrev, dInit)
        M, C = dIn.shape
        self._ck(self.lib.b200rl_mask_bwd(_p(dIn), _p(first), _p(dPrev), _p(dInit), M, C, _ld(dIn), _ld(dPrev),
                                          self._st()))

    def cat_sample(self, raw, noise, unimix: float, groups: int, classes: int, onehot, mix_out=None):
        _f32(raw, noise, onehot, mix_out)
        M = raw.shape[0]
        if noise is not None and noise.dim() != 2:
            noise = noise.reshape(M, -1)
        self._ck(self.lib.b200rl_cat_sample(_p(raw), _p(noise), _p(onehot), _p(mix_out), M, groups, classes, _ld(raw),
                                            _ld(noise), _ld(onehot), _ld(mix_out), unimix, self._st()))

    def head_sample_supported(self, X, W) -> bool:
        return bool(self.lib.b200rl_head_sample_supported(_p(X), _p(W), X.shape[1], W.shape[0], _ld(X), _ld(W)))

    def head_sample(self, X, W, bias, noise, unimix: float, raw, onehot):
        _f32(X, W, bias, noise, raw, onehot)
        M, Kin = X.shape
        A = W.shape[0]
        assert raw.shape == (M, A) and onehot.shape == (M, A) and W.shape[1] == Kin
        self._ck(self.lib.b200rl_head_sample(_p(X), _p(W), _p(bias), _p(noise), _p(raw), _p(onehot), M, Kin, A, _ld(X),
                                             _ld(W), _ld(raw), _ld(noise), _ld(onehot), unimix, self._st()))

    def cat_sample_bwd(self, raw, dz, dmix, unimix: float, groups: int, classes: int, draw):
        _f32(raw, dz, dmix, draw)
        self._ck(self.lib.b200rl_cat_sample_bwd(_p(raw), _p(dz), _p(dmix), _p(draw), raw.shape[0], groups, classes,
                                                _ld(raw), _ld(dz), _ld(dmix), _ld(draw), unimix, self._st()))

    def kl_loss_grad(self, post_mix, prior_mix, groups, classes, kl_dyn, kl_rep, free_nats, regularizer, scale,
                     d_post, d_prior, rows):
        _f32(post_mix, prior_mix, d_post, d_prior, rows)
        assert rows.is_contiguous() and rows.shape[1] == 4
        self._ck(self.lib.b200rl_kl_loss_grad(_p(post_mix), _p(prior_mix), _p(d_post), _p(d_prior), _p(rows),
                                              post_mix.shape[0], groups, classes, _ld(post_mix), _ld(prior_mix),
                                              _ld(d_post), _ld(d_prior), kl_dyn, kl_rep, free_nats, regularizer, scale,
                                              self._st()))

    def mse_loss_grad(self, pred, target, scale: float, loss_row, grad):
        _f32(pred, target, loss_row, grad)
        assert pred.is_contiguous() and target.is_contiguous() and grad.is_contiguous()
        M, P = pred.shape
        self._ck(self.lib.b200rl_mse_loss_grad(_p(pred), _p(target), _p(loss_row), _p(grad), M, P, scale, self._st()))

    def twohot_loss_grad(self, logits, x, weight, scale, low, high, loss_row, dlogits, accumulate: bool = False):
        _f32(logits, x, weight, loss_row, dlogits)
        M, nb = logits.shape
        assert x.numel() == M and x.is_contiguous()
        self._ck(self.lib.b200rl_twohot_loss_grad(_p(logits), _p(x), _p(weight), _p(loss_row), _p(dlogits), M, nb,
# ... 449 lines not shown
```

sheeprl_b200/params.py:

```python
from __future__ import annotations

from collections import OrderedDict
from typing import Dict, Mapping, Tuple

import torch

ALIGN = 64


class FlatGroup:
    def __init__(self, shapes: Mapping[str, Tuple[int, ...]], device, with_optimizer: bool = True):
        self.shapes = OrderedDict((k, tuple(v)) for k, v in shapes.items())
        self.offsets: Dict[str, int] = {}
        off = 0
        for k, shp in self.shapes.items():
            self.offsets[k] = off
            n = 1
            for s in shp:
                n *= s
            off += (n + ALIGN - 1) // ALIGN * ALIGN
        self.numel = off
        self.device = torch.device(device)
        self.flat = torch.zeros(off, dtype=torch.float32, device=device)
        self.views = self._views(self.flat)
        if with_optimizer:
            self.grad = torch.zeros_like(self.flat)
            self.exp_avg = torch.zeros_like(self.flat)
            self.exp_avg_sq = torch.zeros_like(self.flat)
            self.gviews = self._views(self.grad)
        self.grad_avg = None
        self.step = 0
        self.step_t = torch.zeros(1, dtype=torch.int32, device=device)

    def _views(self, flat: torch.Tensor) -> "OrderedDict[str, torch.Tensor]":
        out = OrderedDict()
        for k, shp in self.shapes.items():
            n = 1
            for s in shp:
                n *= s
            out[k] = flat[self.offsets[k]: self.offsets[k] + n].view(shp)
        return out

    def load(self, state: Mapping[str, torch.Tensor]):
        missing = set(self.shapes) - set(state)
        extra = set(state) - set(self.shapes)
        if missing or extra:
            raise KeyError(f"state dict mismatch: missing={sorted(missing)} unexpected={sorted(extra)}")
        with torch.no_grad():
            for k, v in self.views.items():
                if tuple(state[k].shape) != tuple(v.shape):
                    raise ValueError(f"shape mismatch for {k}: {tuple(state[k].shape)} vs {tuple(v.shape)}")
                v.copy_(state[k])

    def state_dict(self) -> "OrderedDict[str, torch.Tensor]":
        return OrderedDict((k, v.detach().clone()) for k, v in self.views.items())

    def optimizer_views(self):
        return self._views(self.exp_avg), self._views(self.exp_avg_sq)

    def alloc_grad_avg(self) -> torch.Tensor:
        if self.grad_avg is None:
            self.grad_avg = torch.zeros_like(self.flat)
        return self.grad_avg

    def adam_kwargs(self, weight_decay: float = 0.0) -> dict:
        opt = getattr(self, "optimizer", None)
        wd = float((opt.param_groups[0].get("weight_decay") if opt is not None else weight_decay) or 0.0)
        return {"weight_decay": wd} if wd else {}
```

Before: 60.00.

## Pre-split behaviour weights into TF32 planes once per step; fuse transition GEMM with sampling

Before imagination, the weights used by the behaviour phase (world-model GRU, transition, reward and continue heads, plus actor and critic groups) are split into TF32 hi/lo planes once per train step. The imagination-horizon GEMMs then reuse these planes through the presplit tensor-core path instead of re-splitting or using the generic path on every call. A new gemm_sample entry fuses the split-K reduction of the transition logits GEMM with bias, unimix and categorical one-hot sampling in a single kernel. This adds plane buffers sized like each parameter group and a per-step split pass, in exchange for fewer kernel launches and less redundant splitting across the horizon.

```diff
diff --git a/include/b200rl.h b/include/b200rl.h
--- a/include/b200rl.h
+++ b/include/b200rl.h
@@ -38,6 +38,10 @@
                             const float* gamma, const float* beta, float eps, int act, float* pre, long long ldpre,
                             float* out, long long ldout, int mode, const float* h_prev, long long ldh, float* h_out,
                             long long ldho, float* h_out2, long long ldho2, cudaStream_t stream);
+int b200rl_gemm_sample_supported(const float* A, const float* W, int M, int N, int K, int lda, int ldw, int classes);
+int b200rl_gemm_sample(const float* A, const float* W, const float* Wlo, const float* bias, const float* noise, float* raw,
+                       float* onehot, int M, int N, int K, int lda, int ldw, long long ldn, long long ldr, long long ldo,
+                       int classes, float unimix, cudaStream_t stream);
 int b200rl_ln_act_route(int C, long long ld0, long long ld1, long long ld2, const float* p0, const float* p1,
                         const float* p2, const float* gamma, const float* beta);
 int b200rl_ln_act_fwd(const float* X, const float* gamma, const float* beta, float* Y, long long M, int C,
diff --git a/sheeprl_b200/algos/p2e_dv3/engine.py b/sheeprl_b200/algos/p2e_dv3/engine.py
--- a/sheeprl_b200/algos/p2e_dv3/engine.py
+++ b/sheeprl_b200/algos/p2e_dv3/engine.py
@@ -129,6 +129,8 @@
             self.noise_img_action_expl.copy_(torch.cat([x for x in noise["img_action_expl"]], -1))
         self._world_model_phase(data, heads_detached=True)
         self._ensemble_learning(data)
+        self._split_behaviour_planes(self.actor_expl, *[c[k] for c in self.critics_expl.values() for k in ("group", "target")],
+                                     self.actor, self.critic, self.target)
         task_noise = (self.noise_img_state, self.noise_img_action)
         self.noise_img_state, self.noise_img_action = self.noise_img_state_expl, self.noise_img_action_expl
         try:
@@ -186,18 +188,19 @@
         a = self.cfg.algo
         M1, M0 = (H + 1) * N, H * N
         traj2 = self.traj.view(M1, L)
-        c_logit = self.cont_img.forward(traj2)
+        pl = self.use_planes
+        c_logit = self.cont_img.forward(traj2, planes=pl)
         mo = a.actor.moments
         weights_sum = sum(c["weight"] for c in self.critics_expl.values())
         v_logits, r_logits = {}, None
         for k, c in self.critics_expl.items():
-            v_logits[k] = c["mlp"].forward(traj2)
+            v_logits[k] = c["mlp"].forward(traj2, planes=pl)
             ops.twohot_mean(v_logits[k], TWOHOT_LOW, TWOHOT_HIGH, c["values"].view(-1))
             if c["reward_type"] == "intrinsic":
                 self._intrinsic_reward()
                 rew = self.intr_reward
             else:
-                r_logits = self.rew_img.forward(traj2)
+                r_logits = self.rew_img.forward(traj2, planes=pl)
                 ops.twohot_mean(r_logits, TWOHOT_LOW, TWOHOT_HIGH, self.rew_pred.view(-1))
                 rew = self.rew_pred
             ops.sum_rows(rew.view(M1, 1), c["reward_mean"], 1.0 / M1)
diff --git a/sheeprl_b200/csrc/gemm_tc.cu b/sheeprl_b200/csrc/gemm_tc.cu
--- a/sheeprl_b200/csrc/gemm_tc.cu
+++ b/sheeprl_b200/csrc/gemm_tc.cu
@@ -5,6 +5,7 @@
 #include <unordered_map>
 
 #include "common.cuh"
+#include "sample.cuh"
 
 namespace {
 
@@ -941,6 +942,31 @@
     }
   }
 }
+
+__global__ void __launch_bounds__(256)
+splitk_sample_kernel(const float* __restrict__ part, int ks, int mpad, int ldw, int M, int groups, int K,
+                     const float* __restrict__ bias, const float* __restrict__ noise, long long ldn, float* __restrict__ raw,
+                     long long ldr, float* __restrict__ onehot, long long ldo, float unimix) {
+  const int lane = threadIdx.x & 31;
+  const long long warp = ((long long)blockIdx.x * blockDim.x + threadIdx.x) >> 5;
+  if (warp >= (long long)M * groups) return;
+  const long long m = warp / groups;
+  const int g = (int)(warp - m * groups);
+  const bool on = lane < K;
+  const int col = g * K + lane;
+  float xv = -INFINITY;
+  if (on) {
+    const float* p = part + (size_t)m * ldw + col;
+    float acc = 0.f;
+#pragma unroll 4
+    for (int z = 0; z < ks; ++z) acc += __ldcg(p + (size_t)z * mpad * ldw);
+    if (bias) acc += bias[col];
+    xv = acc;
+    if (raw) raw[m * ldr + col] = xv;
+  }
+  cat_sample_lane(xv, on, K, lane, unimix, noise ? noise + m * ldn + (long long)g * K : nullptr,
+                  onehot + m * ldo + (long long)g * K, nullptr);
+}
 }
 
 extern "C" int b200rl_gemm_tc(const float* A, const float* B, float* C, const float* bias, int M, int N, int K, int lda,
@@ -1019,6 +1045,26 @@
                       h_out, ldho, h_out2, ldho2, st);
 }
 
+extern "C" int b200rl_gemm_sample_supported(const float* A, const float* W, int M, int N, int K, int lda, int ldw,
+                                            int classes) {
+  return b200rl_gemm_tc_supported(A, W, M, N, K, lda, ldw, 0, 1) && classes > 0 && classes <= 32 && N % classes == 0;
+}
+extern "C" int b200rl_gemm_sample(const float* A, const float* W, const float* Wlo, const float* bias, const float* noise,
+                                  float* raw, float* onehot, int M, int N, int K, int lda, int ldw, long long ldn,
+                                  long long ldr, long long ldo, int classes, float unimix, cudaStream_t st) {
+  RL_CHECK_ARG(A && W && onehot, "null pointer");
+  RL_CHECK_ARG(b200rl_gemm_sample_supported(A, W, M, N, K, lda, ldw, classes),
+               "gemm_sample: NT tensor-core operands, classes <= 32 dividing N");
+  FusedTail ft;
+  if (int rc = gemm_tc_impl(A, W, Wlo, nullptr, nullptr, M, N, K, lda, ldw, N, 0, 1, 0, st, &ft)) return rc;
+  const int groups = N / classes;
+  splitk_sample_kernel<<<ceil_div((long long)M * groups * 32, 256), 256, 0, st>>>(ft.part, ft.ks, ft.mpad, ft.ldw, M, groups,
+                                                                                  classes, bias, noise, ldn, raw, ldr,
+                                                                                  onehot, ldo, unimix);
+  RL_CHECK_LAUNCH();
+  return B200RL_OK;
+}
+
 extern "C" int b200rl_conv_wgrad_mn_supported(int NB, int h, int w, int Cs, int Cb) {
   if (w <= 0 || h <= 0 || (w & (w - 1)) || (h & (h - 1))) return 0;
   const long long P = (long long)NB * h * w;
diff --git a/sheeprl_b200/csrc/rssm.cu b/sheeprl_b200/csrc/rssm.cu
--- a/sheeprl_b200/csrc/rssm.cu
+++ b/sheeprl_b200/csrc/rssm.cu
@@ -1,4 +1,5 @@
 #include "common.cuh"
+#include "sample.cuh"
 
 namespace {
 
@@ -73,11 +74,6 @@
   float lse;
 };
 
-__device__ __forceinline__ float unimix_logprob(float s, float unimix, float invK, float& pm) {
-  pm = (1.f - unimix) * s + unimix * invK;
-  return logf(fminf(fmaxf(pm, kFp32Eps), 1.f - kFp32Eps));
-}
-
 __device__ __forceinline__ GroupStats group_stats(const float* x, int K, float unimix, int lane) {
   GroupStats st;
   float mx = -INFINITY;
@@ -151,38 +147,6 @@
     if (ob > best || (ob == best && oi < besti)) { best = ob; besti = oi; }
   }
   for (int c = lane; c < K; c += 32) onehot[m * ldo + (long long)g * K + c] = (c == besti) ? 1.f : 0.f;
-}
-
-__device__ __forceinline__ void cat_sample_lane(float xv, bool on, int K, int lane, float unimix,
-                                                const float* __restrict__ noise_row, float* __restrict__ onehot_row,
-                                                float* __restrict__ mix_row) {
-  const float mx = warp_max(xv);
-  const float sm = warp_sum(on ? expf(xv - mx) : 0.f);
-  const float invK = 1.f / (float)K;
-  float l = xv;
-  if (unimix > 0.f && on) { float pm; l = unimix_logprob(expf(xv - mx) / sm, unimix, invK, pm); }
-  const float lmx = warp_max(on ? l : -INFINITY);
-  const float ls = warp_sum(on ? expf(l - lmx) : 0.f);
-  const float lse = lmx + logf(ls);
-  if (mix_row && on) mix_row[lane] = l;
-  const float lgmax = warp_max(on ? l - lse : -INFINITY);
-  const float e = on ? expf(l - lse - lgmax) : 0.f;
-  const float psum = warp_sum(e);
-  if (!onehot_row) return;
-  float best = -INFINITY;
-  int besti = 0x7fffffff;
-  if (on) {
-    float p = e / psum;
-    if (noise_row) p = p / noise_row[lane];
-    if (p > best) { best = p; besti = lane; }
-  }
-#pragma unroll
-  for (int o = 16; o > 0; o >>= 1) {
-    const float ob = __shfl_xor_sync(0xffffffffu, best, o);
-    const int oi = __shfl_xor_sync(0xffffffffu, besti, o);
-    if (ob > best || (ob == best && oi < besti)) { best = ob; besti = oi; }
-  }
-  if (on) onehot_row[lane] = (lane == besti) ? 1.f : 0.f;
 }
 
 __global__ void __launch_bounds__(256)
diff --git a/sheeprl_b200/csrc/sample.cuh b/sheeprl_b200/csrc/sample.cuh
--- /dev/null
+++ b/sheeprl_b200/csrc/sample.cuh
@@ -0,0 +1,43 @@
+#pragma once
+#include "common.cuh"
+
+namespace {
+
+__device__ __forceinline__ float unimix_logprob(float s, float unimix, float invK, float& pm) {
+  pm = (1.f - unimix) * s + unimix * invK;
+  return logf(fminf(fmaxf(pm, kFp32Eps), 1.f - kFp32Eps));
+}
+
+__device__ __forceinline__ void cat_sample_lane(float xv, bool on, int K, int lane, float unimix,
+                                                const float* __restrict__ noise_row, float* __restrict__ onehot_row,
+                                                float* __restrict__ mix_row) {
+  const float mx = warp_max(xv);
+  const float sm = warp_sum(on ? expf(xv - mx) : 0.f);
+  const float invK = 1.f / (float)K;
+  float l = xv;
+  if (unimix > 0.f && on) { float pm; l = unimix_logprob(expf(xv - mx) / sm, unimix, invK, pm); }
+  const float lmx = warp_max(on ? l : -INFINITY);
+  const float ls = warp_sum(on ? expf(l - lmx) : 0.f);
+  const float lse = lmx + logf(ls);
+  if (mix_row && on) mix_row[lane] = l;
+  const float lgmax = warp_max(on ? l - lse : -INFINITY);
+  const float e = on ? expf(l - lse - lgmax) : 0.f;
+  const float psum = warp_sum(e);
+  if (!onehot_row) return;
+  float best = -INFINITY;
+  int besti = 0x7fffffff;
+  if (on) {
+    float p = e / psum;
+    if (noise_row) p = p / noise_row[lane];
+    if (p > best) { best = p; besti = lane; }
+  }
+#pragma unroll
+  for (int o = 16; o > 0; o >>= 1) {
+    const float ob = __shfl_xor_sync(0xffffffffu, best, o);
+    const int oi = __shfl_xor_sync(0xffffffffu, besti, o);
+    if (ob > best || (ob == best && oi < besti)) { best = ob; besti = oi; }
+  }
+  if (on) onehot_row[lane] = (lane == besti) ? 1.f : 0.f;
+}
+
+}
diff --git a/sheeprl_b200/engine.py b/sheeprl_b200/engine.py
--- a/sheeprl_b200/engine.py
+++ b/sheeprl_b200/engine.py
@@ -145,12 +145,16 @@
 FUSED_DENSE_MAX_ROWS = 4096
 
 
-def dense_ln_act(ops, x, W, gamma, beta, eps, act, out, pre=None, scratch=None):
+def _planes_kw(planes) -> dict:
+    return {} if planes is None else {"planes": planes}
+
+
+def dense_ln_act(ops, x, W, gamma, beta, eps, act, out, pre=None, scratch=None, planes=None):
     if x.shape[0] <= FUSED_DENSE_MAX_ROWS and ops.gemm_ln_supported(x, W):
-        ops.gemm_ln_act(x, W, gamma, beta, eps, act, out, pre)
+        ops.gemm_ln_act(x, W, gamma, beta, eps, act, out, pre, **_planes_kw(planes))
         return
     tmp = pre if pre is not None else scratch
-    ops.gemm(x, W, tmp, False, True)
+    ops.gemm(x, W, tmp, False, True, **_planes_kw(planes))
     ops.ln_act_fwd(tmp, gamma, beta, eps, act, out)
 
 
@@ -172,20 +176,23 @@
     def W(self, i):
         return self.g.views[f"{self.prefix}{3 * i}.weight"]
 
-    def forward(self, x: torch.Tensor, group: Optional[FlatGroup] = None, M: Optional[int] = None):
+    def forward(self, x: torch.Tensor, group: Optional[FlatGroup] = None, M: Optional[int] = None,
+                planes: bool = False):
         ops = self.eng.ops
         g = group or self.g
         M = x.shape[0] if M is None else M
         cur = x
         for i in range(self.n_hidden):
-            dense_ln_act(ops, cur, g.views[f"{self.prefix}{3 * i}.weight"], g.views[f"{self.prefix}{3 * i + 1}.weight"],
-                         g.views[f"{self.prefix}{3 * i + 1}.bias"], self.eps, ACT_SILU, self.act[i][:M], self.pre[i][:M])
+            w = f"{self.prefix}{3 * i}.weight"
+            dense_ln_act(ops, cur, g.views[w], g.views[f"{self.prefix}{3 * i + 1}.weight"],
+                         g.views[f"{self.prefix}{3 * i + 1}.bias"], self.eps, ACT_SILU, self.act[i][:M], self.pre[i][:M],
+                         planes=g.planes(w) if planes else None)
             cur = self.act[i][:M]
         if self.out_dim is None:
             return cur
-        j = 3 * self.n_hidden
-        ops.gemm(cur, g.views[f"{self.prefix}{j}.weight"], self.out[:M], False, True,
-                 bias=g.views[f"{self.prefix}{j}.bias"])
+        w = f"{self.prefix}{3 * self.n_hidden}.weight"
+        ops.gemm(cur, g.views[w], self.out[:M], False, True, bias=g.views[f"{self.prefix}{3 * self.n_hidden}.bias"],
+                 **_planes_kw(g.planes(w) if planes else None))
         return self.out[:M]
 
     def backward(self, x: torch.Tensor, dout: torch.Tensor, dx: Optional[torch.Tensor], accumulate_dx: bool,
@@ -255,6 +262,7 @@
 
             ops = CudaOps(device)
         self.ops = ops
+        self.use_planes = hasattr(ops, "tf32_split")
         self.cfg = cfg
         self.device = torch.device(device)
         self.actions_dim = tuple(int(x) for x in actions_dim)
@@ -500,9 +508,22 @@
     def train_step(self, data: Dict[str, torch.Tensor], noise: Optional[Dict[str, torch.Tensor]] = None):
         self._draw_noise(noise)
         self._world_model_phase(data)
+        self._split_behaviour_planes(self.actor, self.critic, self.target)
         self._imagine()
         self._behaviour_losses()
         return self.metrics
+
+    _WM_BEHAVIOUR = ("rssm.recurrent_model.rnn.linear.", "rssm.transition_model.", "reward_model.", "continue_model.")
+
+    def _split_behaviour_planes(self, *groups: FlatGroup):
+        if not self.use_planes:
+            return
+        self.wm.split_planes(self.ops, [k for k in self.wm.shapes if k.startswith(self._WM_BEHAVIOUR)])
+        for g in groups:
+            g.split_planes(self.ops)
+
+    def _wm_planes(self, name: str, planes: bool):
+        return self.wm.planes(name) if planes else None
 
     def _draw_noise(self, noise: Optional[Dict[str, torch.Tensor]]):
         ops = self.ops
@@ -730,9 +751,9 @@
         ops.gemm(self.d_dec_lin, self._w(p + "0.weight"), self.d_latent, False, False)
 
     def _recurrent_forward(self, z, act, h_prev, x_pre, x_act, g_pre, g_ln, h_out, win_t=None, hx=None, h_next=None,
-                           keep: bool = True):
+                           keep: bool = True, planes: bool = False):
         self._recurrent_input(z, act, x_pre, x_act, win_t, keep)
-        return self._gru_forward(h_prev, x_act, g_pre, g_ln, h_out, hx, h_next, keep)
+        return self._gru_forward(h_prev, x_act, g_pre, g_ln, h_out, hx, h_next, keep, planes)
 
     def _recurrent_input(self, z, act, x_pre, x_act, win_t=None, keep: bool = True):
         ops, Z = self.ops, self.Z
@@ -751,16 +772,18 @@
             ops.ln_act_fwd(x_pre, self._w(p + "mlp._model.1.weight"), self._w(p + "mlp._model.1.bias"), self.eps,
                            ACT_SILU, x_act)
 
-    def _gru_forward(self, h_prev, x_act, g_pre, g_ln, h_out, hx=None, h_next=None, keep: bool = True):
+    def _gru_forward(self, h_prev, x_act, g_pre, g_ln, h_out, hx=None, h_next=None, keep: bool = True,
+                     planes: bool = False):
         ops, R = self.ops, self.R
         p = "rssm.recurrent_model."
         Wg = self._w(p + "rnn.linear.weight")
+        pk = _planes_kw(self._wm_planes(p + "rnn.linear.weight", planes))
         if hx is not None and hx.shape[0] <= FUSED_DENSE_MAX_ROWS and ops.gemm_ln_supported(hx, Wg, 1):
             ops.gemm_ln_gru(hx, Wg, self._w(p + "rnn.layer_norm.weight"), self._w(p + "rnn.layer_norm.bias"), self.eps,
-                            h_prev, h_out, h_next, g_pre if keep else None, g_ln if keep else None)
+                            h_prev, h_out, h_next, g_pre if keep else None, g_ln if keep else None, **pk)
             return True
         if hx is not None:
-            ops.gemm(hx, Wg, g_pre, False, True)
+            ops.gemm(hx, Wg, g_pre, False, True, **pk)
         else:
             ops.gemm(h_prev, Wg[:, :R], g_pre, False, True, accumulate=x_act is None)
             if x_act is not None:
@@ -791,12 +814,18 @@
                        d_g_ln, d_g_pre, None, None)
         ops.gemm(d_g_pre, self._w(p + "linear.weight")[:, :self.R], dh_prev, False, False, accumulate=True)
 
-    def _transition_forward(self, h, tr_pre, tr_act, raw, keep: bool = True):
+    def _transition_forward(self, h, tr_pre, tr_act, raw, keep: bool = True, planes: bool = False, sample=None):
         ops = self.ops
         p = "rssm.transition_model._model."
         dense_ln_act(ops, h, self._w(p + "0.weight"), self._w(p + "1.weight"), self._w(p + "1.bias"), self.eps, ACT_SILU,
-                     tr_act, tr_pre if keep else None, scratch=tr_pre)
-        ops.gemm(tr_act, self._w(p + "3.weight"), raw, False, True, bias=self._w(p + "3.bias"))
+                     tr_act, tr_pre if keep else None, scratch=tr_pre, planes=self._wm_planes(p + "0.weight", planes))
+        W, bias, pk = self._w(p + "3.weight"), self._w(p + "3.bias"), _planes_kw(self._wm_planes(p + "3.weight", planes))
+        if sample is not None and hasattr(ops, "gemm_sample") and ops.gemm_sample_supported(tr_act, W, self.D):
+            ops.gemm_sample(tr_act, W, bias, sample[0], self.unimix, self.D, sample[1], raw if keep else None, **pk)
+            return
+        ops.gemm(tr_act, W, raw, False, True, bias=bias, **pk)
+        if sample is not None:
+            ops.cat_sample(raw, sample[0], self.unimix, self.S, self.D, sample[1])
 
     def _transition_backward(self, raw, tr_pre, dz, dmix, d_raw, d_tr_act, d_tr_pre, dh, ln_grads: bool = False):
         ops = self.ops
@@ -1047,16 +1076,14 @@
                       float(b1), float(b2), float(ocfg.eps), g.step_t, self.norms[slot: slot + 1],
                       **g.adam_kwargs(ocfg.get("weight_decay", 0.0)))
 
-    def _actor_heads(self, hidden: torch.Tensor, raw_out: torch.Tensor, actor: Optional[FlatGroup] = None):
+    def _actor_heads(self, hidden: torch.Tensor, raw_out: torch.Tensor, actor: Optional[FlatGroup] = None,
+                     planes: bool = False):
         actor = actor or self.actor
-        if self.is_continuous:
-            self.ops.gemm(hidden, actor.views["mlp_heads.0.weight"], raw_out, False, True,
-                          bias=actor.views["mlp_heads.0.bias"])
-            return
         off = 0
-        for i, ad in enumerate(self.actions_dim):
-            self.ops.gemm(hidden, actor.views[f"mlp_heads.{i}.weight"], raw_out[:, off:off + ad], False, True,
-                          bias=actor.views[f"mlp_heads.{i}.bias"])
+        for i, ad in enumerate((self.AW,) if self.is_continuous else self.actions_dim):
+            w = f"mlp_heads.{i}.weight"
+            self.ops.gemm(hidden, actor.views[w], raw_out[:, off:off + ad], False, True,
+                          bias=actor.views[f"mlp_heads.{i}.bias"], **_planes_kw(actor.planes(w) if planes else None))
             off += ad
 
     def _imagine(self, actor: Optional[FlatGroup] = None, actor_mlp: Optional["_MLP"] = None):
@@ -1070,6 +1097,7 @@
                 self._win_t = torch.empty(Win.shape[1], Win.shape[0], dtype=torch.float32, device=self.device)
             ops.transpose2d(Win, self._win_t)
         h_staged = False
+        pl = self.use_planes
         for i in range(H + 1):
             rows = slice(i * N, (i + 1) * N)
             if i > 0:
@@ -1089,15 +1117,16 @@
                     h_next = (self.c_hx[i] if self.is_continuous else hx)[:, :R]
                 h_staged = self._recurrent_forward(prev[:, :Z], self.actions[i - 1], prev[:, Z:], x_pre, hx[:, R:], g_pre,
                                                    g_ln, cur[:, Z:], win_t=self._win_t if gather else None, hx=hx,
-                                                   h_next=h_next, keep=keep) and h_next is not None
-                self._transition_forward(cur[:, Z:], tr_pre, tr_act, raw, keep=keep)
-                ops.cat_sample(raw, self.noise_img_state[i - 1], self.unimix, self.S, self.D, cur[:, :Z])
+                                                   h_next=h_next, keep=keep, planes=pl) and h_next is not None
+                self._transition_forward(cur[:, Z:], tr_pre, tr_act, raw, keep=keep, planes=pl,
+                                         sample=(self.noise_img_state[i - 1], cur[:, :Z]))
             x = self.traj[i]
             cur_in = x
             for l in range(am.n_hidden):
+                w = f"model._model.{3 * l}.weight"
                 dense_ln_act(ops, cur_in, am.W(l), actor.views[f"model._model.{3 * l + 1}.weight"],
                              actor.views[f"model._model.{3 * l + 1}.bias"], self.eps, ACT_SILU, am.act[l][rows],
-                             am.pre[l][rows])
+                             am.pre[l][rows], planes=actor.planes(w) if pl else None)
                 cur_in = am.act[l][rows]
             if not self.is_continuous:
                 off, done = 0, True
@@ -1111,7 +1140,7 @@
                                         self.actor_raw[rows, off:off + ad], self.actions[i, :, off:off + ad])
                         off += ad
                     continue
-            self._actor_heads(cur_in, self.actor_raw[rows], actor)
+            self._actor_heads(cur_in, self.actor_raw[rows], actor, planes=pl)
             if self.is_continuous:
                 ac = self.cfg.algo.actor
                 ops.cont_action_fwd(self.actor_raw[rows], self.noise_img_action[i], self.actions[i], self.act_ent[rows],
@@ -1163,11 +1192,12 @@
         a = self.cfg.algo
         M1, M0 = (H + 1) * N, H * N
         traj2 = self.traj.view(M1, L)
-        v_logits = self.critic_mlp.forward(traj2)
+        pl = self.use_planes
+        v_logits = self.critic_mlp.forward(traj2, planes=pl)
         ops.twohot_mean(v_logits, TWOHOT_LOW, TWOHOT_HIGH, self.values.view(-1))
-        r_logits = self.rew_img.forward(traj2)
+        r_logits = self.rew_img.forward(traj2, planes=pl)
         ops.twohot_mean(r_logits, TWOHOT_LOW, TWOHOT_HIGH, self.rew_pred.view(-1))
-        c_logit = self.cont_img.forward(traj2)
+        c_logit = self.cont_img.forward(traj2, planes=pl)
         ops.lambda_returns(self.rew_pred, self.values, c_logit.view(H + 1, N), self.true_cont, float(a.gamma),
                            float(a.lmbda), self.lam, self.discount)
         mo = a.actor.moments
@@ -1211,7 +1241,7 @@
         a = self.cfg.algo
         M1, M0 = (H + 1) * N, H * N
         traj2 = self.traj.view(M1, L)
-        t_logits = tm.forward(traj2[:M0])
+        t_logits = tm.forward(traj2[:M0], planes=self.use_planes)
         ops.twohot_mean(t_logits, TWOHOT_LOW, TWOHOT_HIGH, self.target_values)
         disc = self.discount.view(-1)[:M0]
         ops.twohot_loss_grad(v_logits[:M0], lam.view(-1), disc, 1.0 / M0, TWOHOT_LOW, TWOHOT_HIGH,
diff --git a/sheeprl_b200/lib.py b/sheeprl_b200/lib.py
--- a/sheeprl_b200/lib.py
+++ b/sheeprl_b200/lib.py
@@ -160,15 +160,21 @@
     def matmul_precision(self) -> str:
         return "highest" if self.lib.b200rl_get_matmul_precision() == 3 else "high"
 
-    def gemm(self, A, B, C, transA: bool, transB: bool, bias=None, accumulate: bool = False):
+    def gemm(self, A, B, C, transA: bool, transB: bool, bias=None, accumulate: bool = False, planes=None):
         _f32(A, B, C, bias)
         M, N = C.shape
         K = A.shape[0] if transA else A.shape[1]
         assert (A.shape[1] if transA else A.shape[0]) == M, (A.shape, C.shape, transA)
         assert (B.shape[0] if transB else B.shape[1]) == N and (B.shape[1] if transB else B.shape[0]) == K, \
             (A.shape, B.shape, C.shape, transA, transB)
-        if (not transA and M >= PRESPLIT_MIN_ROWS and self.use_tc
-                and self.lib.b200rl_gemm_tc_supported(_p(A), _p(B), M, N, K, _ld(A), _ld(B), 0, int(transB))):
+        tc = (not transA and self.use_tc
+              and self.lib.b200rl_gemm_tc_supported(_p(A), _p(B), M, N, K, _ld(A), _ld(B), 0, int(transB)))
+        if tc and planes is not None:
+            assert transB and planes[0].shape == B.shape and planes[0].stride() == B.stride()
+            self._ck(self.lib.b200rl_gemm_tc_presplit(_p(A), _p(planes[0]), _p(planes[1]), _p(C), _p(bias), M, N, K,
+                                                      _ld(A), _ld(B), _ld(C), int(accumulate), self._st()))
+            return
+        if tc and M >= PRESPLIT_MIN_ROWS:
             hi, lo, ld = self._planes(B, transB, N, K)
             self._ck(self.lib.b200rl_gemm_tc_presplit(_p(A), _p(hi), _p(lo), _p(C), _p(bias), M, N, K, _ld(A), ld, _ld(C),
                                                       int(accumulate), self._st()))
@@ -192,22 +198,55 @@
         return self.use_tc and bool(self.lib.b200rl_gemm_ln_supported(_p(A), _p(W), M, W.shape[0], K, _ld(A), _ld(W),
                                                                      mode))
 
-    def gemm_ln_act(self, A, W, gamma, beta, eps: float, act: int, out, pre=None):
+    def _gemm_ln(self, A, W, planes, *args):
+        M, K = A.shape
+        N = W.shape[0]
+        if planes is None:
+            self._ck(self.lib.b200rl_gemm_ln(_p(A), _p(W), M, N, K, _ld(A), _ld(W), *args, self._st()), 2)
+            return
+        assert planes[0].shape == W.shape and planes[0].stride() == W.stride()
+        self._ck(self.lib.b200rl_gemm_ln_presplit(_p(A), _p(planes[0]), _p(planes[1]), M, N, K, _ld(A), _ld(W), *args,
+                                                  self._st()), 2)
+
+    def gemm_ln_act(self, A, W, gamma, beta, eps: float, act: int, out, pre=None, planes=None):
         _f32(A, W, gamma, beta, out, pre)
         M, K = A.shape
         N = W.shape[0]
         assert W.shape[1] == K and out.shape == (M, N)
-        self._ck(self.lib.b200rl_gemm_ln(_p(A), _p(W), M, N, K, _ld(A), _ld(W), _p(gamma), _p(beta), eps, act, _p(pre),
-                                         _ld(pre), _p(out), _ld(out), 0, None, 0, None, 0, None, 0, self._st()), 2)
-
-    def gemm_ln_gru(self, A, W, gamma, beta, eps: float, h_prev, h_out, h_out2=None, g_pre=None, g_ln=None):
+        self._gemm_ln(A, W, planes, _p(gamma), _p(beta), eps, act, _p(pre), _ld(pre), _p(out), _ld(out), 0, None, 0, None,
+                      0, None, 0)
+
+    def gemm_ln_gru(self, A, W, gamma, beta, eps: float, h_prev, h_out, h_out2=None, g_pre=None, g_ln=None, planes=None):
         _f32(A, W, gamma, beta, h_prev, h_out, h_out2, g_pre, g_ln)
         M, K = A.shape
         N = W.shape[0]
         assert W.shape[1] == K and h_prev.shape == (M, N // 3) and h_out.shape == (M, N // 3)
-        self._ck(self.lib.b200rl_gemm_ln(_p(A), _p(W), M, N, K, _ld(A), _ld(W), _p(gamma), _p(beta), eps, 0, _p(g_pre),
-                                         _ld(g_pre), _p(g_ln), _ld(g_ln), 1, _p(h_prev), _ld(h_prev), _p(h_out),
-                                         _ld(h_out), _p(h_out2), _ld(h_out2), self._st()), 2)
+        self._gemm_ln(A, W, planes, _p(gamma), _p(beta), eps, 0, _p(g_pre), _ld(g_pre), _p(g_ln), _ld(g_ln), 1,
+                      _p(h_prev), _ld(h_prev), _p(h_out), _ld(h_out), _p(h_out2), _ld(h_out2))
+
+    def tf32_split(self, X, hi, lo):
+        _f32(X, hi, lo)
+        assert X.is_contiguous() and hi.is_contiguous() and lo.is_contiguous() and hi.shape == X.shape == lo.shape
+        self._ck(self.lib.b200rl_tf32_split(_p(X), _p(hi), _p(lo), X.numel(), self._st()))
+
+    def gemm_sample_supported(self, A, W, classes: int) -> bool:
+        M, K = A.shape
+        return self.use_tc and bool(self.lib.b200rl_gemm_sample_supported(_p(A), _p(W), M, W.shape[0], K, _ld(A), _ld(W),
+                                                                         classes))
+
+    def gemm_sample(self, A, W, bias, noise, unimix: float, classes: int, onehot, raw=None, planes=None):
+        _f32(A, W, bias, noise, onehot, raw)
+        M, K = A.shape
+        N = W.shape[0]
+        assert W.shape[1] == K and onehot.shape == (M, N) and (raw is None or raw.shape == (M, N))
+        if noise is not None and noise.dim() != 2:
+            noise = noise.reshape(M, -1)
+        hi, lo = (W, None) if planes is None else planes
+        if planes is not None:
+            assert hi.shape == W.shape and hi.stride() == W.stride()
+        self._ck(self.lib.b200rl_gemm_sample(_p(A), _p(hi), _p(lo), _p(bias), _p(noise), _p(raw), _p(onehot), M, N, K,
+                                             _ld(A), _ld(W), _ld(noise), _ld(raw), _ld(onehot), classes, unimix,
+                                             self._st()), 2)
 
     def _scratch(self, slot: str, numel: int) -> torch.Tensor:
         buf = self._scratch_bufs.get(slot)
diff --git a/sheeprl_b200/params.py b/sheeprl_b200/params.py
--- a/sheeprl_b200/params.py
+++ b/sheeprl_b200/params.py
@@ -29,6 +29,7 @@
             self.exp_avg_sq = torch.zeros_like(self.flat)
             self.gviews = self._views(self.grad)
         self.grad_avg = None
+        self.hi = self.lo = None
         self.step = 0
         self.step_t = torch.zeros(1, dtype=torch.int32, device=device)
 
@@ -63,6 +64,26 @@
             self.grad_avg = torch.zeros_like(self.flat)
         return self.grad_avg
 
+    def split_planes(self, ops, names=None) -> None:
+        if self.hi is None:
+            self.hi, self.lo = torch.zeros_like(self.flat), torch.zeros_like(self.flat)
+            self.hviews, self.lviews = self._views(self.hi), self._views(self.lo)
+        wanted = set(self.shapes if names is None else names)
+        runs, keys = [], list(self.shapes)
+        for i, k in enumerate(keys):
+            if k not in wanted:
+                continue
+            end = self.offsets[keys[i + 1]] if i + 1 < len(keys) else self.numel
+            if runs and runs[-1][1] == self.offsets[k]:
+                runs[-1][1] = end
+            else:
+                runs.append([self.offsets[k], end])
+        for a, b in runs:
+            ops.tf32_split(self.flat[a:b], self.hi[a:b], self.lo[a:b])
+
+    def planes(self, name: str):
+        return self.hviews[name], self.lviews[name]
+
     def adam_kwargs(self, weight_decay: float = 0.0) -> dict:
         opt = getattr(self, "optimizer", None)
         wd = float((opt.param_groups[0].get("weight_decay") if opt is not None else weight_decay) or 0.0)
```

New measurement: 60.99 (median of 6 runs). 1.02x the previous value.
